# yisol/IDM-VTON

Hardware: AMD Instinct MI355X
Metric: try-on images/sec at 768x1024, 30 DDIM steps, guidance 2.0 (higher is better)
Workload: dtype bf16; 1 GPU; BASELINE.json configs[1]: 768x1024, 30 steps, batch 2/GPU, guidance 2.0, bf16 storage / fp32 accumulate, scheduler ddim, hipGraph on, GarmentNet batched over 6 timesteps, GarmentNet(block b+1)||TryonNet(block b) two-stream overlap on; images_per_call=2, parallelism=dp1 (image shards, one start-up RCCL weight broadcast), rccl_ranks=1

## Files before the change

### idm-vton_amd/csrc/gemm_body.cuh

```cuda
#pragma once
#include <type_traits>
#if !defined(__gfx950__) && !defined(__gfx942__) && defined(__HIP_DEVICE_COMPILE__)
#error "gemm_body.cuh: the counted vmcnt pipeline is written for gfx94x/gfx950 (stores counted in vmcnt)"
#endif
#include "common.cuh"
#include "gemm_common.cuh"

template <typename T, int BN, int BM, int WN, int WM, int ST, bool V1, bool LIN, bool PF, bool TR, bool XA = false>
__device__ __forceinline__ void gemm_body(const GemmParams& p, char* smem, const int m0, const int n0) {
    typedef typename VT<T>::v8 v8;
    typedef typename VT<T>::v4 v4;
    constexpr int NW = WN * WM;
    constexpr int SN = BN / WN, SM = BM / WM;
    constexpr int NI = SN / 32, MI = SM / 32;
    constexpr int WBYTES = BN * 128, XBYTES = BM * 128;
    constexpr int PW_ = BN / 8, PX_ = BM / 8;
    constexpr bool UNEVEN = (PW_ % NW != 0) || (PX_ % NW != 0);
    constexpr int WI = (PW_ + NW - 1) / NW, XI = (PX_ + NW - 1) / NW;
    static_assert(BN % 8 == 0 && BM % 8 == 0 && WN * SN == BN && WM * SM == BM && NI * 32 == SN && MI * 32 == SM, "tile / wave-count mismatch");
    static_assert(!UNEVEN || (V1 && ST == 2), "round-robin piece assignment needs the two-stage ring");
    char* sW = smem;
    char* sX = smem + ST * WBYTES;

    const int lane = threadIdx.x & 63;
    const int wave = uniform(threadIdx.x >> 6);
    const int wn = wave / WM, wm = wave % WM;
    const int u = lane >> 5, l31 = lane & 31;

    const int lrow = lane >> 3, lslot = lane & 7;
    auto wj = [&](int i) { return UNEVEN ? wave + i * NW : wave * WI + i; };
    auto xj = [&](int i) { return UNEVEN ? wave + i * NW : wave * XI + i; };
    uint32_t w_off[WI];
#pragma unroll
    for (int i = 0; i < WI; ++i) {
        const int R = wj(i) * 8 + lrow;
        const int c = lslot ^ ((R >> 1) & 7);
        w_off[i] = ((uint32_t)(n0 + R) * (uint32_t)p.Ktot + c * 8) * 2u;
    }
    int x_pix[XI], x_oy[XI], x_ox[XI], x_c8[XI];
    uint32_t x_off[XI];
    const int HoWo = p.Ho * p.Wo;
    auto kbyte = [&](int t) -> uint32_t { return (uint32_t)t * 128u; };
#pragma unroll
    for (int i = 0; i < XI; ++i) {
        const int R = xj(i) * 8 + lrow;
        const int m = m0 + R;
        x_c8[i] = (lslot ^ ((R >> 1) & 7)) * 8;
        if constexpr (LIN) {
            x_off[i] = m < p.M ? ((uint32_t)m * (uint32_t)p.seg[0].pitch + p.seg[0].coff + x_c8[i]) * 2u : OOB_SENTINEL;
        } else if (m < p.M) {
            const int b = m / HoWo, rem = m - b * HoWo;
            const int oy = rem / p.Wo, ox = rem - oy * p.Wo;
            x_pix[i] = b * p.Hi * p.Wi; x_oy[i] = oy * p.stride; x_ox[i] = ox * p.stride;
        } else {
            x_pix[i] = 0; x_oy[i] = -(1 << 28); x_ox[i] = 0;
        }
    }
    const __amdgpu_buffer_rsrc_t rs_w = make_rsrc(p.w, p.w_bytes);
    const __amdgpu_buffer_rsrc_t rs_x0 = make_rsrc(p.seg[0].ptr, p.seg[0].bytes);
    const int hin = p.ups ? p.Ho : p.Hi, win = p.ups ? p.Wo : p.Wi;

    int si = 0, kseg = 0;
    auto issue = [&](int t, int buf) {
        char* dW = sW + buf * WBYTES;
        char* dX = sX + buf * XBYTES;
#pragma unroll
        for (int i = 0; i < WI; ++i) {
            if (UNEVEN && wj(i) >= PW_) continue;
            dma16(rs_w, dW + wj(i) * 1024, w_off[i] + kbyte(t));
        }
        if constexpr (LIN) {
#pragma unroll
            for (int i = 0; i < XI; ++i) {
                if (UNEVEN && xj(i) >= PX_) continue;
                dma16(rs_x0, dX + xj(i) * 1024, x_off[i] + kbyte(t));
            }
        } else {
            const idmvton_seg sg = p.seg[si];
            const __amdgpu_buffer_rsrc_t rs_x = make_rsrc(sg.ptr, sg.bytes);
#pragma unroll
            for (int i = 0; i < XI; ++i) {
                if (UNEVEN && xj(i) >= PX_) continue;
                int iy = x_oy[i] + sg.dy, ix = x_ox[i] + sg.dx;
                const bool ok = (unsigned)iy < (unsigned)hin && (unsigned)ix < (unsigned)win;
                if (p.ups) { iy >>= 1; ix >>= 1; }
                const uint32_t off = ((uint32_t)(x_pix[i] + iy * p.Wi + ix) * (uint32_t)sg.pitch + sg.coff + kseg + x_c8[i]) * 2u;
                dma16(rs_x, dX + xj(i) * 1024, ok ? off : OOB_SENTINEL);
            }
            kseg += 64;
            if (kseg >= sg.len) { kseg = 0; ++si; }
        }
    };

    idmvton_seg sgc = p.seg[0];
    __amdgpu_buffer_rsrc_t rs_xc = rs_x0;
    auto issue_part = [&](int t, int buf, int s) {
        constexpr int LPT_ = WI + XI;
        char* dW = sW + buf * WBYTES;
        char* dX = sX + buf * XBYTES;
        if constexpr (!LIN) {
            if (s == 0) { sgc = p.seg[si]; rs_xc = make_rsrc(sgc.ptr, sgc.bytes); }
        }
#pragma unroll
        for (int j = 0; j < LPT_; ++j) {
            if ((j & 3) != s) continue;
            if (j < WI) {
                if (UNEVEN && wj(j) >= PW_) continue;
                dma16(rs_w, dW + wj(j) * 1024, w_off[j] + kbyte(t));
            } else {
                const int i = j - WI;
                if (UNEVEN && xj(i) >= PX_) continue;
                if constexpr (LIN) dma16(rs_x0, dX + xj(i) * 1024, x_off[i] + kbyte(t));
                else {
                    int iy = x_oy[i] + sgc.dy, ix = x_ox[i] + sgc.dx;
                    const bool ok = (unsigned)iy < (unsigned)hin && (unsigned)ix < (unsigned)win;
                    if (p.ups) { iy >>= 1; ix >>= 1; }
                    const uint32_t off = ((uint32_t)(x_pix[i] + iy * p.Wi + ix) * (uint32_t)sgc.pitch + sgc.coff + kseg + x_c8[i]) * 2u;
                    dma16(rs_xc, dX + xj(i) * 1024, ok ? off : OOB_SENTINEL);
                }
            }
        }
        if constexpr (!LIN) {
            if (s == 3) { kseg += 64; if (kseg >= sgc.len) { kseg = 0; ++si; } }
        }
    };

    int a_row[NI], a_swz[NI], b_row[MI], b_swz[MI];
#pragma unroll
    for (int ni = 0; ni < NI; ++ni) { const int r = wn * SN + ni * 32 + l31; a_row[ni] = r * 128; a_swz[ni] = (r >> 1) & 7; }
#pragma unroll
    for (int mi = 0; mi < MI; ++mi) { const int r = wm * SM + mi * 32 + l31; b_row[mi] = r * 128; b_swz[mi] = (r >> 1) & 7; }

    f32x16 acc[NI][MI];
#pragma unroll
    for (int ni = 0; ni < NI; ++ni)
#pragma unroll
        for (int mi = 0; mi < MI; ++mi)
#pragma unroll
            for (int r = 0; r < 16; ++r) acc[ni][mi][r] = 0.f;

    auto frag_a = [&](const char* bW, int s, int ni) { return *(const v8*)(bW + a_row[ni] + (((2 * s + u) ^ a_swz[ni]) << 4)); };
    auto frag_b = [&](const char* bX, int s, int mi) { return *(const v8*)(bX + b_row[mi] + (((2 * s + u) ^ b_swz[mi]) << 4)); };
    auto compute = [&](int buf, bool spread = false, int t_next = 0, int buf_next = 0) {
        const char* bW = sW + buf * WBYTES;
        const char* bX = sX + buf * XBYTES;
        if constexpr (!PF) {
#pragma unroll
            for (int s = 0; s < 4; ++s) {
                v8 a[NI], b[MI];
#pragma unroll
                for (int ni = 0; ni < NI; ++ni) a[ni] = frag_a(bW, s, ni);
#pragma unroll
                for (int mi = 0; mi < MI; ++mi) b[mi] = frag_b(bX, s, mi);
                if constexpr (V1) {
                    if (spread) issue_part(t_next, buf_next, s);
                    __builtin_amdgcn_sched_barrier(0);
                }
#pragma unroll
                for (int ni = 0; ni < NI; ++ni)
#pragma unroll
                    for (int mi = 0; mi < MI; ++mi)
                        acc[ni][mi] = TR ? VT<T>::mfma(b[mi], a[ni], acc[ni][mi]) : VT<T>::mfma(a[ni], b[mi], acc[ni][mi]);
            }
        } else {
            v8 a[2][NI], b[2][MI];
#pragma unroll
            for (int ni = 0; ni < NI; ++ni) a[0][ni] = frag_a(bW, 0, ni);
#pragma unroll
            for (int mi = 0; mi < MI; ++mi) b[0][mi] = frag_b(bX, 0, mi);
#pragma unroll
            for (int s = 0; s < 4; ++s) {
                if (s < 3) {
#pragma unroll
                    for (int ni = 0; ni < NI; ++ni) a[(s + 1) & 1][ni] = frag_a(bW, s + 1, ni);
#pragma unroll
                    for (int mi = 0; mi < MI; ++mi) b[(s + 1) & 1][mi] = frag_b(bX, s + 1, mi);
                }
                if (spread) issue_part(t_next, buf_next, s);
                __builtin_amdgcn_sched_barrier(0);
#pragma unroll
                for (int ni = 0; ni < NI; ++ni)
#pragma unroll
                    for (int mi = 0; mi < MI; ++mi)
                        acc[ni][mi] = TR ? VT<T>::mfma(b[s & 1][mi], a[s & 1][ni], acc[ni][mi])
                                         : VT<T>::mfma(a[s & 1][ni], b[s & 1][mi], acc[ni][mi]);
                __builtin_amdgcn_sched_barrier(0);
            }
        }
    };

    v8 xkf[XA ? XA_NK : 1];
    int xa_b = 0, xa_h = 0;
    if constexpr (XA) {
        static_assert(NI == 2 && !TR, "fused cross-attention: one 64-channel head per wave");
        const int mw = m0 + wm * SM;
        xa_b = (mw < p.M ? mw : p.M - 1) / p.xa.tokens;
        xa_h = (n0 + wn * SN) >> 6;
        xattn_load_k<T>(p.xa, xa_b, xa_h, lane, xkf);
    }
    const int nt = p.Ktot >> 6;
    if constexpr (!V1) {
        issue(0, 0);
        for (int t = 0; t < nt; ++t) {
            asm volatile("s_waitcnt vmcnt(0)" ::: "memory");
            __syncthreads();
            if (t + 1 < nt) issue(t + 1, (t + 1) & 1);
            compute(t & 1);
        }
    } else {
        constexpr int LPT = WI + XI;
        static_assert((ST - 2) * LPT < 64, "vmcnt immediate is 6 bits");
#pragma unroll
        for (int s = 0; s < ST - 1; ++s)
            if (s < nt) issue(s, s);
        int cbuf = 0, ibuf = ST - 1;
        for (int t = 0; t < nt; ++t) {
            if (t + ST - 2 < nt) wait_vmcnt<(ST - 2) * LPT>(); else wait_vmcnt<0>();
            __builtin_amdgcn_s_barrier();
            asm volatile("" ::: "memory");
            compute(cbuf, t + ST - 1 < nt, t + ST - 1, ibuf);
            cbuf = cbuf + 1 == ST ? 0 : cbuf + 1;
            ibuf = ibuf + 1 == ST ? 0 : ibuf + 1;
        }
    }

    if constexpr (XA) {
        v8 xvf[XA_NV];
        xattn_load_v<T>(p.xa, xa_b, xa_h, lane, xvf);
        xattn_compute<T, MI>(p.xa, p.M, acc, m0 + wm * SM, lane, xkf, xvf);
    }
    gemm_epilogue<T, NI, MI, SN, SM, TR>(p, acc, m0, n0, wn, wm, lane);
}

template <typename T, int BN, int BM, int WN, int WM, int ST, bool V1, bool LIN, int OCC, bool PFX = false>
__global__ __launch_bounds__(WN * WM * 64, OCC) void gemm_conv_kernel(const GemmParams p) {
    __shared__ __attribute__((aligned(1024))) char smem[ST * (BN + BM) * 128];
    const int wg = xcd_remap(blockIdx.x, p.tiles_m * p.tiles_n);
    int tm, tn;
    if constexpr (!V1) { tm = wg / p.tiles_n; tn = wg - tm * p.tiles_n; }
    else {
        const int GM = p.gm > 0 ? p.gm : 1024 / BM;
        const int width = GM * p.tiles_n;
        const int grp = wg / width, rem = wg - grp * width;
        const int first = grp * GM;
        const int gsz = p.tiles_m - first < GM ? p.tiles_m - first : GM;
        tn = rem / gsz; tm = first + (rem - tn * gsz);
    }
    const int m0 = tm * BM, n0 = tn * BN;
    if constexpr (BN == 320) {
        gemm_body<T, BN, BM, WN, WM, ST, V1, LIN, OCC == 1 || PFX, false>(p, smem, m0, n0);
    } else {
        if (p.vt != nullptr && n0 >= p.vt_n0) gemm_body<T, BN, BM, WN, WM, ST, V1, LIN, OCC == 1 || PFX, true>(p, smem, m0, n0);
        else gemm_body<T, BN, BM, WN, WM, ST, V1, LIN, OCC == 1 || PFX, false>(p, smem, m0, n0);
    }
}

template <typename T, int BN, int BM, int WN, int WM, int ST, int OCC>
__global__ __launch_bounds__(WN * WM * 64, OCC) void gemm_xattn_kernel(const GemmParams p) {
    __shared__ __attribute__((aligned(1024))) char smem[ST * (BN + BM) * 128];
    const int wg = xcd_remap(blockIdx.x, p.tiles_m * p.tiles_n);
    const int GM = p.gm > 0 ? p.gm : 1024 / BM;
    const int width = GM * p.tiles_n;
    const int grp = wg / width, rem = wg - grp * width;
    const int first = grp * GM;
    const int gsz = p.tiles_m - first < GM ? p.tiles_m - first : GM;
    const int tn = rem / gsz, tm = first + (rem - tn * gsz);
    gemm_body<T, BN, BM, WN, WM, ST, true, true, OCC == 1, false, true>(p, smem, tm * BM, tn * BN);
}

template <typename T, int BN, int BM, int WN, int WM, int ST, bool V1, int OCC, bool PFX = false>
static void launch_cfg(const GemmParams& p0, bool lin, hipStream_t st) {
    GemmParams p = p0;
    p.gm = V1 ? idmvton_choose_gm(p.tiles_m, p.tiles_n, BM, BN, p.Ktot) : 0;
    const dim3 grid(p.tiles_n * p.tiles_m), block(WN * WM * 64);
    if constexpr (V1) {
        if (lin) { hipLaunchKernelGGL((gemm_conv_kernel<T, BN, BM, WN, WM, ST, true, true, OCC, PFX>), grid, block, 0, st, p); return; }
    }
    hipLaunchKernelGGL((gemm_conv_kernel<T, BN, BM, WN, WM, ST, V1, false, OCC, PFX>), grid, block, 0, st, p);
}


int gemm_tiles_v0(const GemmParams& p, bool bf16, int bn, int bm, bool lin, hipStream_t st);
int gemm_tiles_v1(const GemmParams& p, bool bf16, int bn, int bm, bool lin, hipStream_t st);
int gemm_tiles_v2(const GemmParams& p, bool bf16, int bn, int bm, bool lin, hipStream_t st);
int gemm_tiles_w8(const GemmParams& p, bool bf16, int bn, int bm, int form, bool lin, hipStream_t st);
int gemm_tiles_xattn(const GemmParams& p, bool bf16, int bn, int bm, int w8, hipStream_t st);
int launch_gemm_lin(const GemmParams& p, bool bf16, int bm, int form, int grid_cap, hipStream_t st);
```

### idm-vton_amd/csrc/gemm_common.cuh

```cuda
#pragma once
#include "common.cuh"
#include "xattn.cuh"

struct GemmParams {
    const void* w; uint32_t w_bytes; int N; int Ktot;
    int nseg; idmvton_seg seg[IDMVTON_MAX_SEG];
    int M, Ho, Wo, Hi, Wi, stride, ups;
    void* out; int ldo;
    const void* bias; const void* rowbias; int rowbias_ld; int rows_per_group;
    const void* res; int ldr;
    int mode;
    void* vt; int vt_n0; int vt_tokens; int vt_perm;
    int colscale_n; float colscale;
    int tiles_m, tiles_n;
    int gm;
    int wide;
    int res32, out32;
    int bias32;
    int out8; float o8_scale, vt8_scale;
    XAttnParams xa;
};

int idmvton_choose_gm(int tiles_m, int tiles_n, int bm, int bn, int K);

template <int N> __device__ __forceinline__ void wait_vmcnt() { asm volatile("s_waitcnt vmcnt(%0)" ::"n"(N) : "memory"); }

__device__ __forceinline__ void swap_cols8(const f32x16& c, const int gp, float (&v)[8]) {
#pragma unroll
    for (int j = 0; j < 4; ++j) {
        const auto r = __builtin_amdgcn_permlane32_swap(__float_as_uint(c[8 * gp + j]), __float_as_uint(c[8 * gp + 4 + j]), false, false);
        v[j] = __uint_as_float(r[0]);
        v[4 + j] = __uint_as_float(r[1]);
    }
}

template <typename T, int NI, int MI, int SN, int SM, bool TR>
__device__ __forceinline__ void gemm_epilogue(const GemmParams& p, f32x16 (&acc)[NI][MI], const int m0, const int n0, const int wn, const int wm,
                                              const int lane) {
    typedef typename VT<T>::v4 v4;
    typedef typename VT<T>::v8 v8;
    const int u = lane >> 5, l31 = lane & 31;
    const T* bias = (const T*)p.bias;
    if constexpr (TR) {
        if (p.out8) {
            uint8_t* vt = (uint8_t*)p.vt;
            const int Cv = p.N - p.vt_n0;
#pragma unroll
            for (int ni = 0; ni < NI; ++ni) {
                const int n = n0 + wn * SN + ni * 32 + l31;
                if (n >= p.N) continue;
                const float bv = bias ? (float)bias[n] : 0.f;
#pragma unroll
                for (int mi = 0; mi < MI; ++mi) {
                    const int m = m0 + wm * SM + mi * 32;
                    if (m >= p.M) continue;
                    const int b = m / p.vt_tokens;
                    const int tok = m - b * p.vt_tokens;
                    int4 o;
                    int w[4];
#pragma unroll
                    for (int g = 0; g < 4; ++g)
                        w[g] = pack4_fp8(clamp448((acc[ni][mi][4 * g] + bv) * p.vt8_scale), clamp448((acc[ni][mi][4 * g + 1] + bv) * p.vt8_scale),
                                         clamp448((acc[ni][mi][4 * g + 2] + bv) * p.vt8_scale), clamp448((acc[ni][mi][4 * g + 3] + bv) * p.vt8_scale));
                    o.x = w[0]; o.y = w[1]; o.z = w[2]; o.w = w[3];
                    *(int4*)(vt + ((size_t)(b * Cv + n - p.vt_n0) * p.vt_tokens + (tok & ~63) + 32 * u + ((tok >> 1) & 16))) = o;
                }
            }
            return;
        }
        if (p.vt_perm) {
            T* vt = (T*)p.vt;
            const int Cv = p.N - p.vt_n0;
#pragma unroll
            for (int ni = 0; ni < NI; ++ni) {
                const int n = n0 + wn * SN + ni * 32 + l31;
                if (n >= p.N) continue;
                const float bv = bias ? (float)bias[n] : 0.f;
#pragma unroll
                for (int mi = 0; mi < MI; ++mi)
#pragma unroll
                    for (int gp = 0; gp < 2; ++gp) {
                        const int m = m0 + wm * SM + mi * 32 + 16 * gp;
                        if (m >= p.M) continue;
                        const int b = m / p.vt_tokens;
                        const int tok = m - b * p.vt_tokens + 8 * u;
                        v8 o;
#pragma unroll
                        for (int j = 0; j < 8; ++j) o[j] = (T)(acc[ni][mi][8 * gp + j] + bv);
                        *(v8*)(vt + ((size_t)(b * Cv + n - p.vt_n0) * p.vt_tokens + tok)) = o;
                    }
            }
            return;
        }
        T* vt = (T*)p.vt;
        const int Cv = p.N - p.vt_n0;
#pragma unroll
        for (int ni = 0; ni < NI; ++ni) {
            const int n = n0 + wn * SN + ni * 32 + l31;
            if (n >= p.N) continue;
            const float bv = bias ? (float)bias[n] : 0.f;
#pragma unroll
            for (int mi = 0; mi < MI; ++mi)
#pragma unroll
                for (int g = 0; g < 4; ++g) {
                    const int m = m0 + wm * SM + mi * 32 + 8 * g + 4 * u;
                    if (m >= p.M) continue;
                    const int b = m / p.vt_tokens;
                    int tok = m - b * p.vt_tokens;
                    if (p.vt_perm) tok = (tok & ~12) | ((tok & 4) << 1) | ((tok & 8) >> 1);
                    v4 o;
#pragma unroll
                    for (int j = 0; j < 4; ++j) o[j] = (T)(acc[ni][mi][4 * g + j] + bv);
                    *(v4*)(vt + ((size_t)(b * Cv + n - p.vt_n0) * p.vt_tokens + tok)) = o;
                }
        }
        return;
    }
    T* out = (T*)p.out;
    const T* res = (const T*)p.res;
    const T* rowbias = (const T*)p.rowbias;
    if (p.wide) {
#pragma unroll
        for (int mi = 0; mi < MI; ++mi) {
            const int m = m0 + wm * SM + mi * 32 + l31;
            if (m >= p.M) continue;
            const T* rb = rowbias ? rowbias + (size_t)(m / p.rows_per_group) * p.rowbias_ld : nullptr;
            if (p.mode == IDMVTON_EPI_GEGLU) {
                if constexpr (NI % 2 == 0) {
#pragma unroll
                    for (int pr = 0; pr < NI / 2; ++pr)
#pragma unroll
                        for (int gp = 0; gp < 2; ++gp) {
                            float h[8], gt[8];
                            swap_cols8(acc[2 * pr][mi], gp, h);
                            swap_cols8(acc[2 * pr + 1][mi], gp, gt);
                            const int nh = n0 + wn * SN + pr * 64 + 16 * gp + 8 * u;
                            if (nh + 32 >= p.N) continue;
                            const int jo = ((n0 + wn * SN + pr * 64) >> 1) + 16 * gp + 8 * u;
                            if (bias) {
                                const v8 bh = *(const v8*)(bias + nh), bg = *(const v8*)(bias + nh + 32);
#pragma unroll
                                for (int j = 0; j < 8; ++j) { h[j] += (float)bh[j]; gt[j] += (float)bg[j]; }
                            }
                            v8 o;
#pragma unroll
                            for (int j = 0; j < 8; ++j) o[j] = (T)(h[j] * gelu_erf(gt[j]));
                            *(v8*)(out + (size_t)m * p.ldo + jo) = o;
                        }
                }
                continue;
            }
#pragma unroll
            for (int ni = 0; ni < NI; ++ni) {
#pragma unroll
                for (int gp = 0; gp < 2; ++gp) {
                    float v[8];
                    swap_cols8(acc[ni][mi], gp, v);
                    const int n = n0 + wn * SN + ni * 32 + 16 * gp + 8 * u;
                    if (n >= p.N) continue;
                    if (bias) {
                        if (p.bias32) {
                            const float4* bp = (const float4*)((const float*)p.bias + n);
                            const float4 b0 = bp[0], b1 = bp[1];
                            v[0] += b0.x; v[1] += b0.y; v[2] += b0.z; v[3] += b0.w;
                            v[4] += b1.x; v[5] += b1.y; v[6] += b1.z; v[7] += b1.w;
                        } else {
                            const v8 bb = *(const v8*)(bias + n);
#pragma unroll
                            for (int j = 0; j < 8; ++j) v[j] += (float)bb[j];
                        }
                    }
                    if (rb) {
                        const v8 bb = *(const v8*)(rb + n);
#pragma unroll
                        for (int j = 0; j < 8; ++j) v[j] += (float)bb[j];
                    }
                    if (n < p.colscale_n) {
#pragma unroll
                        for (int j = 0; j < 8; ++j) v[j] *= p.colscale;
                    }
                    if constexpr (NI * MI <= 8)
                    if (p.out8) {
                        int2 o;
                        o.x = pack4_fp8(clamp448(v[0] * p.o8_scale), clamp448(v[1] * p.o8_scale), clamp448(v[2] * p.o8_scale), clamp448(v[3] * p.o8_scale));
                        o.y = pack4_fp8(clamp448(v[4] * p.o8_scale), clamp448(v[5] * p.o8_scale), clamp448(v[6] * p.o8_scale), clamp448(v[7] * p.o8_scale));
                        *(int2*)((uint8_t*)p.out + (size_t)m * p.ldo + n) = o;
                        continue;
                    }
                    if (p.mode == IDMVTON_EPI_GELU) {
#pragma unroll
                        for (int j = 0; j < 8; ++j) v[j] = gelu_erf(v[j]);
                    } else if (p.mode == IDMVTON_EPI_QUICKGELU) {
#pragma unroll
                        for (int j = 0; j < 8; ++j) v[j] = v[j] / (1.0f + __expf(-1.702f * v[j]));
                    }
                    if (res) {
                        if (p.res32) {
                            const float4* rp = (const float4*)((const float*)p.res + (size_t)m * p.ldr + n);
                            const float4 r0 = rp[0], r1 = rp[1];
                            v[0] += r0.x; v[1] += r0.y; v[2] += r0.z; v[3] += r0.w;
                            v[4] += r1.x; v[5] += r1.y; v[6] += r1.z; v[7] += r1.w;
                        } else {
                            const v8 rr = *(const v8*)(res + (size_t)m * p.ldr + n);
#pragma unroll
                            for (int j = 0; j < 8; ++j) v[j] += (float)rr[j];
                        }
                    }
                    if (p.out32) {
                        float4* op = (float4*)((float*)p.out + (size_t)m * p.ldo + n);
                        op[0] = make_float4(v[0], v[1], v[2], v[3]);
                        op[1] = make_float4(v[4], v[5], v[6], v[7]);
                    } else {
                        v8 o;
#pragma unroll
                        for (int j = 0; j < 8; ++j) o[j] = (T)v[j];
                        *(v8*)(out + (size_t)m * p.ldo + n) = o;
                    }
                }
            }
        }
        return;
    }
    if constexpr (NI * MI <= 8)
#pragma unroll
    for (int mi = 0; mi < MI; ++mi) {
        const int m = m0 + wm * SM + mi * 32 + l31;
        if (m >= p.M) continue;
        const T* rb = rowbias ? rowbias + (size_t)(m / p.rows_per_group) * p.rowbias_ld : nullptr;
        if (p.mode == IDMVTON_EPI_GEGLU) {
            if constexpr (NI % 2 == 0) {
#pragma unroll
                for (int pr = 0; pr < NI / 2; ++pr)
#pragma unroll
                    for (int g = 0; g < 4; ++g) {
                        const int nh = n0 + wn * SN + pr * 64 + 8 * g + 4 * u;
                        if (nh + 32 >= p.N) continue;
                        const int jo = ((n0 + wn * SN + pr * 64) >> 1) + 8 * g + 4 * u;
                        v4 o;
#pragma unroll
                        for (int j = 0; j < 4; ++j) {
                            float h = acc[2 * pr][mi][4 * g + j], gt = acc[2 * pr + 1][mi][4 * g + j];
                            if (bias) { h += (float)bias[nh + j]; gt += (float)bias[nh + 32 + j]; }
                            o[j] = (T)(h * gelu_erf(gt));
                        }
                        *(v4*)(out + (size_t)m * p.ldo + jo) = o;
                    }
            }
            continue;
        }
#pragma unroll
        for (int ni = 0; ni < NI; ++ni)
#pragma unroll
            for (int g = 0; g < 4; ++g) {
                const int n = n0 + wn * SN + ni * 32 + 8 * g + 4 * u;
                if (n >= p.N) continue;
                float v[4];
#pragma unroll
                for (int j = 0; j < 4; ++j) v[j] = acc[ni][mi][4 * g + j];
                if (bias) {
                    const v4 bb = *(const v4*)(bias + n);
#pragma unroll
                    for (int j = 0; j < 4; ++j) v[j] += (float)bb[j];
                }
                if (rb) {
                    const v4 bb = *(const v4*)(rb + n);
#pragma unroll
                    for (int j = 0; j < 4; ++j) v[j] += (float)bb[j];
                }
                if (n < p.colscale_n) {
#pragma unroll
                    for (int j = 0; j < 4; ++j) v[j] *= p.colscale;
                }
                if (p.mode == IDMVTON_EPI_GELU) {
#pragma unroll
                    for (int j = 0; j < 4; ++j) v[j] = gelu_erf(v[j]);
                } else if (p.mode == IDMVTON_EPI_QUICKGELU) {
#pragma unroll
                    for (int j = 0; j < 4; ++j) v[j] = v[j] / (1.0f + __expf(-1.702f * v[j]));
                }
                if (res) {
                    const v4 rr = *(const v4*)(res + (size_t)m * p.ldr + n);
#pragma unroll
                    for (int j = 0; j < 4; ++j) v[j] += (float)rr[j];
                }
                v4 o;
#pragma unroll
                for (int j = 0; j < 4; ++j) o[j] = (T)v[j];
                *(v4*)(out + (size_t)m * p.ldo + n) = o;
            }
    }
}
```

### idm-vton_amd/csrc/gemm_conv.hip

```cpp
#include <cstdlib>
#include <cstring>
#include <vector>
#include "gemm_body.cuh"

int launch_gemm_lin(const GemmParams& p, bool bf16, int bm, int form, int grid_cap, hipStream_t st);

#include <map>
#include <mutex>
#include <tuple>
int idmvton_choose_gm(int tiles_m, int tiles_n, int bm, int bn, int K) {
    static const char* env = getenv("IDMVTON_GM");
    if (env) return atoi(env);
    static const bool model = getenv("IDMVTON_GM_MODEL") && atoi(getenv("IDMVTON_GM_MODEL")) != 0;
    if (!model) return 0;
    static std::mutex mu;
    static std::map<std::tuple<int, int, int, int, int>, int> cache;
    const auto key = std::make_tuple(tiles_m, tiles_n, bm, bn, K);
    std::lock_guard<std::mutex> lk(mu);
    auto it = cache.find(key);
    if (it != cache.end()) return it->second;
    const int T = tiles_m * tiles_n, q = T / 8, r = T % 8;
    static const long cap = getenv("IDMVTON_GM_CAP_KB") ? atol(getenv("IDMVTON_GM_CAP_KB")) << 10 : (2l << 20);
    long best = -1; int best_gm = 0;
    for (int gm = 1; gm <= tiles_m; ++gm) {
        if (gm > 1 && (long)gm * bm * K * 2 > cap) break;
        long cost = 0;
        for (int x = 0; x < 8; ++x) {
            const int lo = x < r ? x * (q + 1) : r * (q + 1) + (x - r) * q, n = x < r ? q + 1 : q;
            int m_lo = tiles_m, m_hi = -1;
            std::vector<char> ms(tiles_m, 0), ns(tiles_n, 0);
            int cm = 0, cn = 0;
            for (int wg = lo; wg < lo + n; ++wg) {
                const int width = gm * tiles_n, grp = wg / width, rem = wg - grp * width, first = grp * gm;
                const int gsz = tiles_m - first < gm ? tiles_m - first : gm;
                const int tn = rem / gsz, tm = first + (rem - tn * gsz);
                if (!ms[tm]) { ms[tm] = 1; ++cm; }
                if (!ns[tn]) { ns[tn] = 1; ++cn; }
            }
            (void)m_lo; (void)m_hi;
            cost += (long)cm * bm + (long)cn * bn;
        }
        if (best < 0 || cost < best) { best = cost; best_gm = gm; }
    }
    cache[key] = best_gm;
    return best_gm;
}

static int launch_gemm(const GemmParams& p0, bool bf16, int variant, int bn, int bm, bool lin, hipStream_t st) {
    GemmParams p = p0;
    int form = 0;
    int grid_cap = 0;
    if (variant == 5) { form = bm & 15; grid_cap = (bm & 0x4000) ? 5 : 0; bm &= ~(15 | 0x4000); }
    p.tiles_n = (p.N + bn - 1) / bn;
    p.tiles_m = (p.M + bm - 1) / bm;
    int rc = 1;
    if (p.mode == IDMVTON_EPI_XATTN) {
        if (bm != 64 && p.xa.tokens % 64 != 0) {
            bm = 64;
            p.tiles_m = (p.M + bm - 1) / bm;
        }
        if (gemm_tiles_xattn(p, bf16, bn, bm, variant == 6 && bn == 128 && bm == 128, st))
            return idmvton_set_error(IDMVTON_E_ARG, "gemm_conv: IDMVTON_EPI_XATTN runs on the 128x64, 128x128 and 128x256 tiles (got %dx%d)", bn, bm);
        CHECK_LAUNCH("gemm_conv");
        return IDMVTON_OK;
    }
    if (variant == 0) rc = gemm_tiles_v0(p, bf16, bn, bm, lin, st);
    else if (variant == 1) rc = gemm_tiles_v1(p, bf16, bn, bm, lin, st);
    else if (variant == 2) rc = gemm_tiles_v2(p, bf16, bn, bm, lin, st);
    else if (variant == 5) {
        if (!(bn == 256 && (bm == 256 || bm == 192))) return idmvton_set_error(IDMVTON_E_ARG, "gemm_conv: variant 5 is the 256x256 / 256x192 tile");
        if (lin) rc = launch_gemm_lin(p, bf16, bm, form, grid_cap, st);
        else if (bm == 256) rc = gemm_tiles_v1(p, bf16, 256, 256, lin, st);
        else {
            p.tiles_n = (p.N + 127) / 128; p.tiles_m = (p.M + 255) / 256;
            rc = gemm_tiles_v1(p, bf16, 128, 256, lin, st);
        }
    } else if (variant == 6) {
        const int form6 = bm & 15;
        bm &= ~15;
        p.tiles_m = (p.M + bm - 1) / bm;
        if (bn == 320 && (p.vt || !p.wide || p.out8 || p.mode == IDMVTON_EPI_GEGLU)) {
            const int fbn = bn == 320 ? 128 : bn, fbm = bn == 320 ? 256 : bm;
            p.tiles_n = (p.N + fbn - 1) / fbn;
            p.tiles_m = (p.M + fbm - 1) / fbm;
            rc = gemm_tiles_v1(p, bf16, fbn, fbm, lin, st);
        } else rc = gemm_tiles_w8(p, bf16, bn, bm, form6, lin, st);
    } else return idmvton_set_error(IDMVTON_E_ARG, "gemm_conv: unknown variant %d", variant);
    if (rc) return idmvton_set_error(IDMVTON_E_ARG, "gemm_conv: variant %d has no %dx%d tile", variant, bn, bm);
    CHECK_LAUNCH("gemm_conv");
    return IDMVTON_OK;
}

extern "C" int idmvton_gemm_conv(const idmvton_gemm_conv_args* a, void* stream) {
    CHECK_ARG(a != nullptr, IDMVTON_E_ARG, "gemm_conv: null args");
    CHECK_ARG(a->dtype == IDMVTON_F16 || a->dtype == IDMVTON_BF16, IDMVTON_E_DTYPE, "gemm_conv: dtype %d", a->dtype);
    CHECK_ARG(a->M > 0 && a->N > 0 && a->Ktot > 0, IDMVTON_E_SHAPE, "gemm_conv: M=%d N=%d K=%d", a->M, a->N, a->Ktot);
    CHECK_ARG(a->Ktot % 64 == 0, IDMVTON_E_SHAPE, "gemm_conv: Ktot=%d must be a multiple of 64", a->Ktot);
    CHECK_ARG(a->N % 4 == 0, IDMVTON_E_SHAPE, "gemm_conv: N=%d must be a multiple of 4", a->N);
    CHECK_ARG(a->nseg >= 1 && a->nseg <= IDMVTON_MAX_SEG, IDMVTON_E_SHAPE, "gemm_conv: nseg=%d", a->nseg);
    int ksum = 0;
    for (int s = 0; s < a->nseg; ++s) {
        const idmvton_seg& g = a->seg[s];
        CHECK_ARG(g.ptr && g.len > 0 && g.len % 64 == 0, IDMVTON_E_SHAPE, "gemm_conv: seg %d len=%d", s, g.len);
        CHECK_ARG(g.pitch % 8 == 0 && g.coff % 8 == 0, IDMVTON_E_ALIGN, "gemm_conv: seg %d pitch=%d coff=%d", s, g.pitch, g.coff);
        CHECK_ARG(g.bytes < 0x80000000u, IDMVTON_E_SHAPE, "gemm_conv: seg %d tensor >= 2 GiB", s);
        CHECK_ARG(((uintptr_t)g.ptr & 15) == 0, IDMVTON_E_ALIGN, "gemm_conv: seg %d pointer not 16-byte aligned", s);
        ksum += g.len;
    }
    CHECK_ARG(ksum == a->Ktot, IDMVTON_E_SHAPE, "gemm_conv: segment lengths sum to %d, Ktot=%d", ksum, a->Ktot);
    CHECK_ARG(a->Ho > 0 && a->Wo > 0 && a->Hi > 0 && a->Wi > 0 && a->stride > 0 && a->M % (a->Ho * a->Wo) == 0,
              IDMVTON_E_SHAPE, "gemm_conv: geometry M=%d Ho=%d Wo=%d", a->M, a->Ho, a->Wo);
    if (a->ups) CHECK_ARG(a->stride == 1 && a->Ho <= 2 * a->Hi && a->Ho >= 2 * a->Hi - 1 && a->Wo <= 2 * a->Wi && a->Wo >= 2 * a->Wi - 1, IDMVTON_E_SHAPE,
                          "gemm_conv: ups=1 needs stride 1 and an output grid of 2Hi x 2Wi or one short of it (Ho=%d Hi=%d Wo=%d Wi=%d)", a->Ho, a->Hi, a->Wo, a->Wi);
    CHECK_ARG(a->w && ((uintptr_t)a->w & 15) == 0, IDMVTON_E_ALIGN, "gemm_conv: weight pointer");
    const uint64_t wbytes = (uint64_t)a->N * a->Ktot * 2;
    CHECK_ARG(wbytes + (uint64_t)128 * a->Ktot * 2 < 0xFFFFFFFFull, IDMVTON_E_SHAPE, "gemm_conv: weight too large");
    const bool geglu = a->mode == IDMVTON_EPI_GEGLU, xattn = a->mode == IDMVTON_EPI_XATTN;
    CHECK_ARG(a->mode == IDMVTON_EPI_NONE || a->mode == IDMVTON_EPI_GELU || a->mode == IDMVTON_EPI_QUICKGELU || geglu || xattn, IDMVTON_E_ARG, "gemm_conv: mode %d", a->mode);
    CHECK_ARG(a->colscale_n >= 0 && a->colscale_n % 4 == 0 && !(geglu && a->colscale_n), IDMVTON_E_ARG, "gemm_conv: colscale_n=%d", a->colscale_n);
    if (geglu) CHECK_ARG(a->N % 64 == 0 && !a->res && !a->rowbias && !a->vt, IDMVTON_E_ARG, "gemm_conv: GEGLU needs N%%64==0, no res/rowbias/vt");
    CHECK_ARG(a->out || (a->vt && a->vt_n0 == 0), IDMVTON_E_ARG, "gemm_conv: null out");
    if (a->out) CHECK_ARG(a->ldo % 4 == 0 && ((uintptr_t)a->out & 7) == 0, IDMVTON_E_ALIGN, "gemm_conv: out alignment");
    if (a->res) CHECK_ARG(a->ldr % 4 == 0 && ((uintptr_t)a->res & 7) == 0, IDMVTON_E_ALIGN, "gemm_conv: res alignment");
    if (a->bias) CHECK_ARG(((uintptr_t)a->bias & 7) == 0, IDMVTON_E_ALIGN, "gemm_conv: bias alignment");
    if (a->rowbias) CHECK_ARG(a->rowbias_ld % 4 == 0 && a->rows_per_group > 0 && ((uintptr_t)a->rowbias & 7) == 0,
                              IDMVTON_E_ALIGN, "gemm_conv: rowbias");
    if (a->vt && a->vt_perm) CHECK_ARG(((uintptr_t)a->vt & 15) == 0, IDMVTON_E_ALIGN, "gemm_conv: vt pointer not 16-byte aligned");
    if (a->vt && a->vt_perm) CHECK_ARG(a->vt_tokens % 16 == 0, IDMVTON_E_ARG, "gemm_conv: vt_perm needs vt_tokens %% 16 == 0 (got %d)", a->vt_tokens);
    if (a->vt) CHECK_ARG(a->vt_tokens > 0 && a->vt_tokens % 4 == 0 && a->M % a->vt_tokens == 0 && a->vt_n0 % 64 == 0 &&
                         a->vt_n0 >= 0 && a->vt_n0 < a->N && ((uintptr_t)a->vt & 7) == 0,
                         IDMVTON_E_ARG, "gemm_conv: vt_tokens=%d vt_n0=%d", a->vt_tokens, a->vt_n0);

    GemmParams p;
    memset(&p.xa, 0, sizeof(p.xa));
    if (xattn) {
        const idmvton_xattn* x = a->xattn;
        CHECK_ARG(x != nullptr && (x->nseg == 1 || x->nseg == 2), IDMVTON_E_ARG, "gemm_conv: IDMVTON_EPI_XATTN needs `xattn` with 1 or 2 key segments");
        CHECK_ARG(a->N % 64 == 0 && !a->bias && !a->res && !a->rowbias && !a->vt && !a->colscale_n && !a->io_flags &&
                  a->nseg == 1 && a->Ho == 1 && a->Hi == 1 && a->Wo == a->M && a->Wi == a->M && a->out && a->ldo % 8 == 0 && ((uintptr_t)a->out & 15) == 0,
                  IDMVTON_E_ARG, "gemm_conv: IDMVTON_EPI_XATTN is a plain Linear with N %% 64 == 0 and nothing else in its epilogue");
        CHECK_ARG(x->tokens > 0 && x->tokens % 32 == 0 && a->M % x->tokens == 0, IDMVTON_E_SHAPE, "gemm_conv: xattn.tokens=%d (rows per batch element, a multiple of 32 dividing M=%d)", x->tokens, a->M);
        for (int s = 0; s < x->nseg; ++s) {
            const int nk_max = s == 0 ? 96 : 32;
            CHECK_ARG(x->k[s] && x->vt[s] && x->nk[s] > 0 && x->nk[s] <= nk_max && x->k_rows[s] >= ((x->nk[s] + 31) & ~31) && x->ldk[s] >= a->N && x->ldk[s] % 8 == 0 &&
                      x->ldvt[s] >= ((x->nk[s] + 15) & ~15) && x->ldvt[s] % 8 == 0 && (((uintptr_t)x->k[s] | (uintptr_t)x->vt[s]) & 15) == 0, IDMVTON_E_SHAPE,
                      "gemm_conv: xattn segment %d: nk=%d (<= %d) k_rows=%d (>= round32(nk)) ldk=%d ldvt=%d (>= round16(nk))", s, x->nk[s], nk_max, x->k_rows[s], x->ldk[s], x->ldvt[s]);
            p.xa.k[s] = x->k[s]; p.xa.vt[s] = x->vt[s]; p.xa.ldk[s] = x->ldk[s]; p.xa.ldvt[s] = x->ldvt[s]; p.xa.nk[s] = x->nk[s]; p.xa.krows[s] = x->k_rows[s];
        }
        p.xa.nseg = x->nseg; p.xa.tokens = x->tokens; p.xa.vchan = a->N; p.xa.ip_scale = x->ip_scale;
    } else CHECK_ARG(a->xattn == nullptr, IDMVTON_E_ARG, "gemm_conv: `xattn` without mode IDMVTON_EPI_XATTN");
    p.w = a->w; p.w_bytes = (uint32_t)wbytes; p.N = a->N; p.Ktot = a->Ktot;
    p.nseg = a->nseg;
    for (int s = 0; s < IDMVTON_MAX_SEG; ++s) p.seg[s] = a->seg[s < a->nseg ? s : a->nseg - 1];
    p.M = a->M; p.Ho = a->Ho; p.Wo = a->Wo; p.Hi = a->Hi; p.Wi = a->Wi; p.stride = a->stride; p.ups = a->ups ? 1 : 0;
    p.out = a->out; p.ldo = a->ldo; p.bias = a->bias; p.rowbias = a->rowbias; p.rowbias_ld = a->rowbias_ld;
    p.rows_per_group = a->rows_per_group > 0 ? a->rows_per_group : 1; p.res = a->res; p.ldr = a->ldr; p.mode = a->mode;
    p.vt = a->vt; p.vt_n0 = a->vt_n0; p.vt_tokens = a->vt_tokens > 0 ? a->vt_tokens : 4; p.vt_perm = a->vt_perm ? 1 : 0;
    p.colscale_n = a->colscale_n; p.colscale = a->colscale;
    p.tiles_m = p.tiles_n = 0; p.gm = 0;
    {
        auto a16 = [](const void* q) { return ((uintptr_t)q & 15) == 0; };
        const int n_out = geglu ? a->N / 2 : a->N;
        p.wide = n_out % 8 == 0 && a->N % 8 == 0 && a->colscale_n % 8 == 0 && (!a->out || (a->ldo % 8 == 0 && a16(a->out))) &&
                 (!a->res || (a->ldr % 8 == 0 && a16(a->res))) && (!a->bias || a16(a->bias)) &&
                 (!a->rowbias || (a->rowbias_ld % 8 == 0 && a16(a->rowbias))) && (!a->vt || a->vt_n0 % 8 == 0);
    }

    int variant = 1, bn = 64, bm = 64;
    static const bool env_narrow = getenv("IDMVTON_EPILOGUE_8B") != nullptr;
    if ((a->tile_hint & 0x8000) || env_narrow) p.wide = 0;
    p.res32 = (a->io_flags & IDMVTON_IO_RES_F32) ? 1 : 0;
    p.out32 = (a->io_flags & IDMVTON_IO_OUT_F32) ? 1 : 0;
    p.bias32 = (a->io_flags & IDMVTON_IO_BIAS_F32) ? 1 : 0;
    if (p.bias32) CHECK_ARG(a->bias && p.wide && !geglu && !a->vt && ((uintptr_t)a->bias & 15) == 0, IDMVTON_E_ARG,
                            "gemm_conv: IDMVTON_IO_BIAS_F32 needs a 16-byte aligned bias and the plain 16-byte epilogue (no GEGLU, no vt)");
    CHECK_ARG((a->io_flags & ~15) == 0, IDMVTON_E_ARG, "gemm_conv: io_flags=%d", a->io_flags);
    p.out8 = (a->io_flags & IDMVTON_IO_OUT_F8) ? 1 : 0;
    p.o8_scale = a->f8_out_scale; p.vt8_scale = a->f8_vt_scale;
    if (p.out8) {
        CHECK_ARG(a->io_flags == IDMVTON_IO_OUT_F8 && a->mode == IDMVTON_EPI_NONE && !a->res && !a->rowbias && p.wide,
                  IDMVTON_E_ARG, "gemm_conv: IDMVTON_IO_OUT_F8 needs the plain 16-byte epilogue (no activation / residual / rowbias / fp32 IO)");
        CHECK_ARG((!a->out || a->f8_out_scale > 0.f) && (!a->vt || (a->f8_vt_scale > 0.f && a->vt_tokens % 64 == 0 && ((uintptr_t)a->vt & 15) == 0)),
                  IDMVTON_E_ARG, "gemm_conv: IDMVTON_IO_OUT_F8: scales > 0, vt_tokens %% 64 == 0 (got %d), 16-byte aligned vt", a->vt_tokens);
    }
    if (p.res32 || p.out32) {
        CHECK_ARG((a->io_flags & ~7) == 0 && !geglu && !a->vt, IDMVTON_E_ARG, "gemm_conv: io_flags=%d (fp32 res / out: no GEGLU, no vt)", a->io_flags);
        CHECK_ARG(!p.res32 || a->res, IDMVTON_E_ARG, "gemm_conv: IDMVTON_IO_RES_F32 without res");
        CHECK_ARG(p.wide, IDMVTON_E_ALIGN, "gemm_conv: the fp32 residual stream needs the 16-byte epilogue (N, ldo, ldr multiples of 8, 16-byte aligned pointers)");
    }
    if (a->tile_hint) { variant = (a->tile_hint >> 28) & 0xf; bn = (a->tile_hint >> 16) & 0xfff; bm = a->tile_hint & 0x7fff; }
    else {
        static const int cand[5][2] = {{256, 256}, {128, 256}, {128, 128}, {128, 64}, {64, 64}};
        for (int i = 0; i < 5; ++i) {
            const int n_ = cand[i][0], m_ = cand[i][1];
            if (geglu && n_ < 128) continue;
            if (xattn && (n_ != 128)) continue;
            if (a->vt && a->vt_n0 % n_ != 0) continue;
            if (i < 4 && (n_ > ((a->N + 63) & ~63) || m_ > ((a->M + 63) & ~63))) continue;
            bn = n_; bm = m_;
            if ((long)((a->N + n_ - 1) / n_) * ((a->M + m_ - 1) / m_) >= 200) break;
        }
    }
    if (geglu) CHECK_ARG(bn >= 128, IDMVTON_E_ARG, "gemm_conv: GEGLU needs BN >= 128 (64-row wave tiles)");
    if (a->vt) CHECK_ARG(a->vt_n0 % bn == 0, IDMVTON_E_ARG, "gemm_conv: vt_n0 %% BN != 0");
    const idmvton_seg& s0 = a->seg[0];
    const bool lin = a->nseg == 1 && a->Ho == 1 && a->Hi == 1 && a->Wo == a->M && a->Wi == a->M && a->stride == 1 &&
                     !a->ups && s0.dy == 0 && s0.dx == 0 && (uint64_t)a->M * s0.pitch * 2 < 0x80000000ull;
    if (!a->tile_hint && bn == 256 && bm == 256 && lin) { variant = 5; bm = 257; }
    else if (!a->tile_hint && !xattn) {
        if (bn == 256 && bm == 256) variant = 6;
        else if (bn == 128 && bm == 128) variant = 6;
        if (a->N > 256 && a->N <= 320 && p.wide && !a->vt && !geglu && !p.out8 && (a->M + 191) / 192 >= 200) { variant = 6; bn = 320; bm = 192; }
    }
    hipStream_t st = (hipStream_t)stream;
    return launch_gemm(p, a->dtype == IDMVTON_BF16, variant, bn, bm, lin, st);
}
```

### idm-vton_amd/csrc/gemm_lin.hip

```cpp
#include "gemm_common.cuh"
#include <type_traits>

template <typename T, int BM, int WN, int WM, int DMA_SPLIT, int WAIT_AT>
__device__ __forceinline__ void gemm_lin_persistent(const GemmParams& p, char* smem) {
    typedef typename VT<T>::v8 v8;
    constexpr int BN = 256, NW = WN * WM;
    constexpr int SN = BN / WN, SM = BM / WM, NI = SN / 32, MI = SM / 32;
    constexpr int PWW = BN / (8 * NW), PWX = BM / (8 * NW);
    static_assert(PWW * 8 * NW == BN && PWX * 8 * NW == BM && NI * 32 * WN == BN && MI * 32 * WM == BM, "tile / wave-count mismatch");
    constexpr int OPW = BN * 128;
    constexpr int BUF = (BN + BM) * 128;

    const int lane = threadIdx.x & 63;
    const int wave = uniform(threadIdx.x >> 6);
    const int wn = wave / WM, wm = wave % WM;
    const int u = lane >> 5, l31 = lane & 31;

    const int ntiles = p.tiles_m * p.tiles_n, G = gridDim.x;
    auto coords = [&](int idx, int& m0, int& n0) {
        const int wg = xcd_remap(idx, ntiles);
        const int GM = p.gm > 0 ? p.gm : 1024 / BM;
        const int width = GM * p.tiles_n;
        const int grp = wg / width, rem = wg - grp * width;
        const int first = grp * GM;
        const int gsz = p.tiles_m - first < GM ? p.tiles_m - first : GM;
        const int tn = rem / gsz;
        m0 = (first + (rem - tn * gsz)) * BM;
        n0 = tn * BN;
    };

    const int lrow = lane >> 3, lslot = lane & 7;
    uint32_t w_off[PWW], x_off[PWX];
    auto set_offsets = [&](int m0, int n0) {
#pragma unroll
        for (int i = 0; i < PWW; ++i) {
            const int R = (wave * PWW + i) * 8 + lrow;
            w_off[i] = ((uint32_t)(n0 + R) * (uint32_t)p.Ktot + (lslot ^ ((R >> 1) & 7)) * 8) * 2u;
        }
#pragma unroll
        for (int i = 0; i < PWX; ++i) {
            const int R = (wave * PWX + i) * 8 + lrow;
            const int m = m0 + R;
            x_off[i] = m < p.M ? ((uint32_t)m * (uint32_t)p.seg[0].pitch + p.seg[0].coff + (lslot ^ ((R >> 1) & 7)) * 8) * 2u : OOB_SENTINEL;
        }
    };
    const __amdgpu_buffer_rsrc_t rs_w = make_rsrc(p.w, p.w_bytes);
    const __amdgpu_buffer_rsrc_t rs_x = make_rsrc(p.seg[0].ptr, p.seg[0].bytes);
    char* const dW = smem + wave * (PWW * 1024);
    char* const dX = smem + OPW + wave * (PWX * 1024);
    auto dma_w = [&](int i, int buf_off, uint32_t koff) {
        __builtin_amdgcn_raw_ptr_buffer_load_lds(rs_w, LDS_PTR(dW + buf_off + i * 1024), 16, w_off[i], koff, 0, 0);
    };
    auto dma_x = [&](int i, int buf_off, uint32_t koff) {
        __builtin_amdgcn_raw_ptr_buffer_load_lds(rs_x, LDS_PTR(dX + buf_off + i * 1024), 16, x_off[i], koff, 0, 0);
    };
    auto dma_first = [&](int buf_off) {
#pragma unroll
        for (int i = 0; i < PWW; ++i) dma_w(i, buf_off, 0u);
#pragma unroll
        for (int i = 0; i < PWX; ++i) dma_x(i, buf_off, 0u);
    };

    const int swz = (l31 >> 1) & 7;
    int fa_off[4], fb_off[4];
#pragma unroll
    for (int s = 0; s < 4; ++s) {
        const int ch = ((2 * s + u) ^ swz) << 4;
        fa_off[s] = (wn * SN + l31) * 128 + ch;
        fb_off[s] = OPW + (wm * SM + l31) * 128 + ch;
    }
    v8 fa[2][NI], fb[2][MI];
    f32x16 acc[NI][MI];

    auto read_all = [&](int set, int s, int buf_off) {
#pragma unroll
        for (int ni = 0; ni < NI; ++ni) fa[set][ni] = *(const v8*)(smem + buf_off + fa_off[s] + ni * 4096);
#pragma unroll
        for (int mi = 0; mi < MI; ++mi) fb[set][mi] = *(const v8*)(smem + buf_off + fb_off[s] + mi * 4096);
    };
    constexpr int NMF = NI * MI;
    constexpr int NRD = NI + MI;
    auto pin = [&](int nrd, int nv) {
#pragma unroll
        for (int i = 0; i < NMF; ++i) {
            __builtin_amdgcn_sched_group_barrier(0x008, 1, 0);
            if (i < nrd) __builtin_amdgcn_sched_group_barrier(0x100, 1, 0);
            if (i >= NMF - nv) __builtin_amdgcn_sched_group_barrier(0x010, 1, 0);
            if (i < nv - NMF) __builtin_amdgcn_sched_group_barrier(0x010, 1, 0);
        }
    };

    const int nt = p.Ktot >> 6;
    int idx = blockIdx.x, m0, n0, nm0 = 0, nn0 = 0;
    bool has_next = false;
    int cur = 0;

    auto run_tile = [&](auto trc) {
        constexpr bool TR = decltype(trc)::value;
        auto mfma_range = [&](int set, int i0, int i1) {
#pragma unroll
            for (int k = i0; k < i1; ++k) {
                const int ni = k / MI, mi = k % MI;
                acc[ni][mi] = TR ? VT<T>::mfma(fb[set][mi], fa[set][ni], acc[ni][mi]) : VT<T>::mfma(fa[set][ni], fb[set][mi], acc[ni][mi]);
            }
        };
#pragma unroll
        for (int ni = 0; ni < NI; ++ni)
#pragma unroll
            for (int mi = 0; mi < MI; ++mi)
#pragma unroll
                for (int r = 0; r < 16; ++r) acc[ni][mi][r] = 0.f;
        __builtin_amdgcn_s_barrier();
        asm volatile("" ::: "memory");
        read_all(0, 0, cur);
        for (int t = 0; t + 1 < nt; ++t) {
            const int nxt = cur ^ BUF;
            const uint32_t koff = (uint32_t)(t + 1) * 128u;
            read_all(1, 1, cur);
#pragma unroll
            for (int i = 0; i < PWW; ++i) dma_w(i, nxt, koff);
            if constexpr (DMA_SPLIT == 1) {
#pragma unroll
                for (int i = 0; i < PWX; ++i) dma_x(i, nxt, koff);
            }
            mfma_range(0, 0, NMF);
            pin(NRD, DMA_SPLIT == 0 ? PWW : PWW + PWX);
            __builtin_amdgcn_sched_barrier(0);
            read_all(0, 2, cur);
            if constexpr (DMA_SPLIT == 0) {
#pragma unroll
                for (int i = 0; i < PWX; ++i) dma_x(i, nxt, koff);
            }
            mfma_range(1, 0, NMF);
            pin(NRD, DMA_SPLIT == 0 ? PWX : 0);
            __builtin_amdgcn_sched_barrier(0);
            read_all(1, 3, cur);
            mfma_range(0, 0, NMF);
            pin(NRD, 0);
            __builtin_amdgcn_sched_barrier(0);
            mfma_range(1, 0, WAIT_AT);
            __builtin_amdgcn_sched_barrier(0);
            asm volatile("s_waitcnt vmcnt(0) lgkmcnt(0)" ::: "memory");
            __builtin_amdgcn_s_barrier();
            asm volatile("" ::: "memory");
            __builtin_amdgcn_sched_barrier(0);
            read_all(0, 0, nxt);
            mfma_range(1, WAIT_AT, NMF);
#pragma unroll
            for (int i = 0; i < NMF - WAIT_AT; ++i) {
                __builtin_amdgcn_sched_group_barrier(0x008, 1, 0);
                if (i < NRD) __builtin_amdgcn_sched_group_barrier(0x100, 1, 0);
                if (i == NMF - WAIT_AT - 1 && NRD > NMF - WAIT_AT) __builtin_amdgcn_sched_group_barrier(0x100, NRD - (NMF - WAIT_AT), 0);
            }
            __builtin_amdgcn_sched_barrier(0);
            cur = nxt;
        }
        if (has_next) {
            set_offsets(nm0, nn0);
            dma_first(cur ^ BUF);
        }
        read_all(1, 1, cur);
        mfma_range(0, 0, NMF);
        pin(NRD, 0);
        __builtin_amdgcn_sched_barrier(0);
        read_all(0, 2, cur);
        mfma_range(1, 0, NMF);
        pin(NRD, 0);
        __builtin_amdgcn_sched_barrier(0);
        read_all(1, 3, cur);
        mfma_range(0, 0, NMF);
        pin(NRD, 0);
        __builtin_amdgcn_sched_barrier(0);
        mfma_range(1, 0, NMF);
        if (has_next) asm volatile("s_waitcnt vmcnt(0)" ::: "memory");
        gemm_epilogue<T, NI, MI, SN, SM, TR>(p, acc, m0, n0, wn, wm, lane);
    };

    coords(idx, m0, n0);
    set_offsets(m0, n0);
    dma_first(0);
    asm volatile("s_waitcnt vmcnt(0)" ::: "memory");
    for (;;) {
        const int nidx = idx + G;
        has_next = nidx < ntiles;
        if (has_next) coords(nidx, nm0, nn0);
        if (p.vt != nullptr && n0 >= p.vt_n0) run_tile(std::true_type{});
        else run_tile(std::false_type{});
        if (!has_next) break;
        cur ^= BUF; idx = nidx; m0 = nm0; n0 = nn0;
    }
}

template <typename T, int BM, int WN, int WM, int DMA_SPLIT, int WAIT_AT>
__global__ __launch_bounds__(512, 2) void gemm_lin_kernel(const GemmParams p) {
    __shared__ __attribute__((aligned(1024))) char smem[2 * (256 + BM) * 128];
    gemm_lin_persistent<T, BM, WN, WM, DMA_SPLIT, WAIT_AT>(p, smem);
}

static int persistent_grid(int ntiles, int grid_cap) {
    static int cus = 0;
    if (!cus) {
        int dev = 0, n = 0;
        if (hipGetDevice(&dev) != hipSuccess || hipDeviceGetAttribute(&n, hipDeviceAttributeMultiprocessorCount, dev) != hipSuccess || n < 8) n = 256;
        cus = n & ~7;
    }
    const int cap = grid_cap > 0 ? grid_cap : cus;
    return ntiles < cap ? ntiles : cap;
}
template <typename T>
static int launch_lin(const GemmParams& p0, int bm, int form, int grid_cap, hipStream_t st) {
    GemmParams p = p0;
    p.gm = idmvton_choose_gm(p.tiles_m, p.tiles_n, bm, 256, p.Ktot);
    const dim3 grid(persistent_grid(p.tiles_n * p.tiles_m, grid_cap)), block(512);
    if (bm == 192) hipLaunchKernelGGL((gemm_lin_kernel<T, 192, 4, 2, 0, 2>), grid, block, 0, st, p);
    else if (form == 0) hipLaunchKernelGGL((gemm_lin_kernel<T, 256, 2, 4, 0, 2>), grid, block, 0, st, p);
    else hipLaunchKernelGGL((gemm_lin_kernel<T, 256, 2, 4, 1, 2>), grid, block, 0, st, p);
    return 0;
}
int launch_gemm_lin(const GemmParams& p, bool bf16, int bm, int form, int grid_cap, hipStream_t st) {
    return bf16 ? launch_lin<bf16_t>(p, bm, form, grid_cap, st) : launch_lin<f16_t>(p, bm, form, grid_cap, st);
}
```

### idm-vton_amd/csrc/gemm_tiles_v1.hip

```cpp
#include "gemm_body.cuh"

template <typename T>
static int run(const GemmParams& p, int bn, int bm, bool lin, hipStream_t st) {
    if (bn == 256 && bm == 256) launch_cfg<T, 256, 256, 2, 4, 2, true, 2>(p, lin, st);
    else if (bn == 128 && bm == 256) launch_cfg<T, 128, 256, 2, 4, 3, true, 2>(p, lin, st);
    else if (bn == 128 && bm == 128) launch_cfg<T, 128, 128, 2, 2, 3, true, 1>(p, lin, st);
    else if (bn == 128 && bm == 64) launch_cfg<T, 128, 64, 2, 2, 3, true, 2>(p, lin, st);
    else if (bn == 64 && bm == 64) launch_cfg<T, 64, 64, 2, 2, 4, true, 2>(p, lin, st);
    else return 1;
    return 0;
}
int gemm_tiles_v1(const GemmParams& p, bool bf16, int bn, int bm, bool lin, hipStream_t st) {
    return bf16 ? run<bf16_t>(p, bn, bm, lin, st) : run<f16_t>(p, bn, bm, lin, st);
}
```

### idm-vton_amd/ffi.py

```python
import ctypes as C
import os

_HERE = os.path.dirname(os.path.abspath(__file__))
LIB_PATH = os.environ.get("IDMVTON_HIP_LIB") or os.path.join(_HERE, "libidmvton_hip.so")

F16, BF16, F32, F8E4M3 = 0, 1, 2, 3
EPI_NONE, EPI_GEGLU, EPI_GELU, EPI_QUICKGELU, EPI_XATTN = 0, 1, 2, 3, 4
ATTN_SELF, ATTN_CROSS = 0, 1
IO_RES_F32, IO_OUT_F32, IO_BIAS_F32, IO_OUT_F8 = 1, 2, 4, 8
GN_X_F32, GN_Y_SPLIT, GN_AFFINE_F32 = 1, 2, 4
LAYOUT_SPLIT, LAYOUT_NHWC_F32 = 1, 2
SPLIT_ACT, SPLIT_W3, SPLIT_W3T = 0, 1, 2
KVS_WIDEN_E4M3, KVS_COPY = 0, 1
MAX_SEG = 24
ABI_VERSION = 9

i32, u32, f32, vp = C.c_int32, C.c_uint32, C.c_float, C.c_void_p


class Seg(C.Structure):
    _fields_ = [("ptr", vp), ("bytes", u32), ("pitch", i32), ("coff", i32), ("len", i32), ("dy", i32), ("dx", i32)]


class XAttn(C.Structure):
    _fields_ = [("nseg", i32), ("k", vp * 2), ("ldk", i32 * 2), ("k_rows", i32 * 2), ("vt", vp * 2), ("ldvt", i32 * 2), ("nk", i32 * 2),
                ("tokens", i32), ("ip_scale", f32)]


class GemmConvArgs(C.Structure):
    _fields_ = [("dtype", i32), ("w", vp), ("N", i32), ("Ktot", i32), ("nseg", i32), ("seg", Seg * MAX_SEG),
                ("M", i32), ("Ho", i32), ("Wo", i32), ("Hi", i32), ("Wi", i32), ("stride", i32), ("ups", i32),
                ("out", vp), ("ldo", i32), ("bias", vp), ("rowbias", vp), ("rowbias_ld", i32),
                ("rows_per_group", i32), ("res", vp), ("ldr", i32), ("mode", i32), ("vt", vp), ("vt_n0", i32),
                ("vt_tokens", i32), ("tile_hint", i32), ("vt_perm", i32), ("io_flags", i32), ("xattn", C.POINTER(XAttn)),
                ("colscale_n", i32), ("colscale", f32), ("f8_out_scale", f32), ("f8_vt_scale", f32)]


class AttnArgs(C.Structure):
    _fields_ = [("dtype", i32), ("mode", i32), ("B", i32), ("heads", i32), ("Nq", i32), ("q", vp), ("ldq", i32),
                ("out", vp), ("ldo", i32), ("nseg", i32), ("k", vp * 2), ("ldk", i32 * 2), ("vt", vp * 2),
                ("ldvt", i32 * 2), ("nk", i32 * 2), ("k_rows", i32 * 2), ("seg_b0", i32 * 2), ("ip_scale", f32), ("tune", i32), ("q_prescaled", i32)]


class LayerNormArgs(C.Structure):
    _fields_ = [("dtype", i32), ("rows", i32), ("C", i32), ("x", vp), ("ldx", i32), ("gamma", vp), ("beta", vp),
                ("eps", f32), ("y", vp), ("ldy", i32), ("y2", vp), ("ldy2", i32), ("x_f32", i32)]


class GroupNormArgs(C.Structure):
    _fields_ = [("dtype", i32), ("B", i32), ("HW", i32), ("C", i32), ("groups", i32), ("x", vp), ("C1", i32),
                ("x2", vp), ("gamma", vp), ("beta", vp), ("eps", f32), ("silu", i32), ("y", vp), ("stats", vp), ("stats_doubles", i32),
                ("flags", i32)]


class PackInputArgs(C.Structure):
    _fields_ = [("dtype", i32), ("B", i32), ("hw", i32), ("cpad", i32), ("latents", vp), ("cond", vp), ("out", vp)]


class CfgStepArgs(C.Structure):
    _fields_ = [("dtype", i32), ("B", i32), ("hw", i32), ("ldc", i32), ("eps_nhwc", vp), ("latents", vp),
                ("noise", vp), ("coef", vp)]


class LayoutArgs(C.Structure):
    _fields_ = [("dtype", i32), ("B", i32), ("C", i32), ("HW", i32), ("cpad", i32), ("to_nhwc", i32), ("src", vp),
                ("dst", vp), ("scale", f32), ("shift", f32), ("flags", i32)]


class VaeSampleArgs(C.Structure):
    _fields_ = [("dtype", i32), ("B", i32), ("hw", i32), ("ldm", i32), ("moments", vp), ("noise", vp), ("z", vp),
                ("scale", f32)]


class AttnSmallArgs(C.Structure):
    _fields_ = [("dtype", i32), ("B", i32), ("heads", i32), ("Lq", i32), ("Lk", i32), ("d", i32), ("q", vp), ("ldq", i32),
                ("k", vp), ("ldk", i32), ("v", vp), ("ldv", i32), ("out", vp), ("ldo", i32), ("scale", f32), ("causal", i32)]


class AttnF8Args(C.Structure):
    _fields_ = [("out_dtype", i32), ("B", i32), ("heads", i32), ("Nq", i32), ("q8", vp), ("ldq", i32), ("out", vp), ("ldo", i32),
                ("nseg", i32), ("k8", vp * 2), ("ldk", i32 * 2), ("vt8", vp * 2), ("ldvt", i32 * 2), ("nk", i32 * 2), ("k_rows", i32 * 2),
                ("seg_b0", i32 * 2), ("qk_scale_exp", i32), ("v_scale_exp", i32)]


class QuantF8Args(C.Structure):
    _fields_ = [("dtype", i32), ("mode", i32), ("rows", i32), ("cols", i32), ("src", vp), ("lds", i32), ("dst", vp), ("ldd", i32), ("scale", f32)]


class SoftmaxArgs(C.Structure):
    _fields_ = [("dtype", i32), ("rows", i32), ("n", i32), ("ld", i32), ("x", vp), ("scale", f32), ("y_split", vp), ("ldy", i32), ("n_valid", i32)]


class SplitArgs(C.Structure):
    _fields_ = [("dtype", i32), ("mode", i32), ("rows", i32), ("cols", i32), ("src", vp), ("lds", i32), ("dst", vp), ("ldd", i32)]


class KvUnpackDesc(C.Structure):
    _fields_ = [("src", vp), ("dst", vp), ("exp", vp), ("rows", i32), ("cols", i32), ("lds", i32), ("ldd", i32)]


class KvUnpackArgs(C.Structure):
    _fields_ = [("dtype", i32), ("n", i32), ("desc", vp), ("max_chunks", i32)]


class KvStreamDesc(KvUnpackDesc):
    pass


class KvStreamArgs(C.Structure):
    _fields_ = [("dtype", i32), ("mode", i32), ("n", i32), ("workgroups", i32), ("desc", vp), ("first", vp)]


STRUCTS = {"idmvton_seg": Seg, "idmvton_gemm_conv_args": GemmConvArgs, "idmvton_attn_args": AttnArgs,
           "idmvton_layernorm_args": LayerNormArgs, "idmvton_groupnorm_args": GroupNormArgs,
           "idmvton_pack_input_args": PackInputArgs, "idmvton_cfg_step_args": CfgStepArgs,
           "idmvton_layout_args": LayoutArgs, "idmvton_vae_sample_args": VaeSampleArgs, "idmvton_softmax_args": SoftmaxArgs,
           "idmvton_attn_small_args": AttnSmallArgs, "idmvton_attn_f8_args": AttnF8Args, "idmvton_quant_f8_args": QuantF8Args,
           "idmvton_split_args": SplitArgs, "idmvton_xattn": XAttn, "idmvton_kv_unpack_desc": KvUnpackDesc,
           "idmvton_kv_unpack_args": KvUnpackArgs, "idmvton_kv_stream_desc": KvStreamDesc, "idmvton_kv_stream_args": KvStreamArgs}

SYMBOLS = ["idmvton_last_error", "idmvton_abi_version", "idmvton_sizeof", "idmvton_gemm_conv", "idmvton_attn_fwd",
           "idmvton_layernorm", "idmvton_groupnorm", "idmvton_pack_input", "idmvton_cfg_step", "idmvton_layout",
           "idmvton_vae_sample", "idmvton_softmax_rows", "idmvton_probe_mfma", "idmvton_groupnorm_stats_doubles",
           "idmvton_attn_small", "idmvton_rccl_unique_id", "idmvton_rccl_comm_init", "idmvton_rccl_bcast_arena",
           "idmvton_rccl_comm_destroy", "idmvton_attn_f8", "idmvton_quant_f8", "idmvton_split", "idmvton_attn_fwd_shared",
           "idmvton_attn_f8_shared", "idmvton_attn_fwd_indexed", "idmvton_attn_f8_indexed",
           "idmvton_attn_fwd_ragged", "idmvton_attn_f8_ragged", "idmvton_kv_unpack", "idmvton_kv_stream",
           "idmvton_host_device_ptr", "idmvton_kv_fill"]

_lib = None


class HipLibraryMissing(RuntimeError):
    pass


def lib():
    global _lib
    if _lib is not None:
        return _lib
    if not os.path.exists(LIB_PATH):
        raise HipLibraryMissing(f"{LIB_PATH} not built: run `make -C {os.path.join(_HERE, 'csrc')}` "
                                "(or __graft_entry__.build()); there is no CPU fallback")
    L = C.CDLL(LIB_PATH)
    for s in SYMBOLS:
        if not hasattr(L, s):
            raise HipLibraryMissing(f"{LIB_PATH} does not export {s}")
    L.idmvton_last_error.restype = C.c_char_p
    L.idmvton_sizeof.argtypes = [C.c_char_p]
    L.idmvton_abi_version.restype = C.c_int
    v = L.idmvton_abi_version()
    if v != ABI_VERSION:
        raise HipLibraryMissing(f"{LIB_PATH} implements C ABI version {v}, this binding needs {ABI_VERSION}: rebuild it "
                                f"(`make -C {os.path.join(_HERE, 'csrc')}`)")
    for name, st in STRUCTS.items():
        n = L.idmvton_sizeof(name.encode())
        if n != C.sizeof(st):
            raise HipLibraryMissing(f"ABI drift: sizeof({name}) is {n} in the library, {C.sizeof(st)} in ffi.py")
    for s in ("idmvton_gemm_conv", "idmvton_attn_fwd", "idmvton_layernorm", "idmvton_groupnorm",
              "idmvton_pack_input", "idmvton_cfg_step", "idmvton_layout", "idmvton_vae_sample", "idmvton_softmax_rows",
              "idmvton_attn_small", "idmvton_attn_f8", "idmvton_quant_f8", "idmvton_split"):
        getattr(L, s).argtypes = [vp, vp]
        getattr(L, s).restype = C.c_int
    for s in ("idmvton_attn_fwd_shared", "idmvton_attn_f8_shared"):
        getattr(L, s).argtypes = [vp, C.POINTER(i32), vp]
        getattr(L, s).restype = C.c_int
    for s in ("idmvton_attn_fwd_indexed", "idmvton_attn_f8_indexed"):
        getattr(L, s).argtypes = [vp, C.POINTER(i32), C.POINTER(vp), vp]
        getattr(L, s).restype = C.c_int
    for s in ("idmvton_attn_fwd_ragged", "idmvton_attn_f8_ragged"):
        getattr(L, s).argtypes = [vp, C.POINTER(i32), C.POINTER(vp), C.POINTER(vp), vp]
        getattr(L, s).restype = C.c_int
    L.idmvton_kv_unpack.argtypes = [vp, vp, vp]
    L.idmvton_kv_unpack.restype = C.c_int
    L.idmvton_kv_stream.argtypes = [vp, vp, vp, vp]
    L.idmvton_kv_stream.restype = C.c_int
    L.idmvton_kv_fill.argtypes = [vp, vp, vp, vp]
    L.idmvton_kv_fill.restype = C.c_int
    L.idmvton_host_device_ptr.argtypes = [vp, C.POINTER(vp)]
    L.idmvton_host_device_ptr.restype = C.c_int
    L.idmvton_probe_mfma.argtypes = [C.c_int, vp, vp, vp, vp]
    L.idmvton_groupnorm_stats_doubles.argtypes = [C.c_int] * 4
    L.idmvton_groupnorm_stats_doubles.restype = C.c_int
    L.idmvton_rccl_unique_id.argtypes = [vp]
    L.idmvton_rccl_comm_init.argtypes = [vp, C.c_int, C.c_int, C.POINTER(vp)]
    L.idmvton_rccl_bcast_arena.argtypes = [vp, vp, C.c_uint64, C.c_int, C.c_uint64, vp]
    L.idmvton_rccl_comm_destroy.argtypes = [vp]
    for s in ("idmvton_rccl_unique_id", "idmvton_rccl_comm_init", "idmvton_rccl_bcast_arena", "idmvton_rccl_comm_destroy"):
        getattr(L, s).restype = C.c_int
    _lib = L
    return L


def call(fn_name, args, stream):
    L = lib()
    rc = getattr(L, fn_name)(C.byref(args), C.c_void_p(stream))
    if rc != 0:
        raise RuntimeError(f"{fn_name} failed ({rc}): {L.idmvton_last_error().decode()}")


def call_shared(fn_name, args, seg_nb, stream):
    L = lib()
    nb = (i32 * 2)(*seg_nb)
    rc = getattr(L, fn_name)(C.byref(args), nb, C.c_void_p(stream))
    if rc != 0:
        raise RuntimeError(f"{fn_name} failed ({rc}): {L.idmvton_last_error().decode()}")


def call_indexed(fn_name, args, seg_nb, seg_index, stream):
    L = lib()
    nb = (i32 * 2)(*seg_nb)
    ix = (vp * 2)(*[int(x) if x else None for x in seg_index])
    rc = getattr(L, fn_name)(C.byref(args), nb, ix, C.c_void_p(stream))
    if rc != 0:
        raise RuntimeError(f"{fn_name} failed ({rc}): {L.idmvton_last_error().decode()}")


def call_ragged(fn_name, args, seg_nb, seg_index, seg_nk, stream):
    L = lib()
    nb = (i32 * 2)(*seg_nb)
    ix = (vp * 2)(*[int(x) if x else None for x in (seg_index or (0, 0))])
    nk = (vp * 2)(*[int(x) if x else None for x in seg_nk])
    rc = getattr(L, fn_name)(C.byref(args), nb, ix, nk, C.c_void_p(stream))
    if rc != 0:
        raise RuntimeError(f"{fn_name} failed ({rc}): {L.idmvton_last_error().decode()}")


def call_kv_unpack(args, host_desc, stream):
    L = lib()
    rc = L.idmvton_kv_unpack(C.byref(args), host_desc if isinstance(host_desc, int) else C.cast(host_desc, vp), C.c_void_p(stream))
    if rc != 0:
        raise RuntimeError(f"idmvton_kv_unpack failed ({rc}): {L.idmvton_last_error().decode()}")


def call_kv_stream(args, host_desc, host_first, stream):
    L = lib()
    p = lambda x: x if isinstance(x, int) else C.cast(x, vp)
    rc = L.idmvton_kv_stream(C.byref(args), p(host_desc), p(host_first), C.c_void_p(stream))
    if rc != 0:
        raise RuntimeError(f"idmvton_kv_stream failed ({rc}): {L.idmvton_last_error().decode()}")


def call_kv_fill(args, host_desc, host_first, stream):
    L = lib()
    p = lambda x: x if isinstance(x, int) else C.cast(x, vp)
    rc = L.idmvton_kv_fill(C.byref(args), p(host_desc), p(host_first), C.c_void_p(stream))
    if rc != 0:
        raise RuntimeError(f"idmvton_kv_fill failed ({rc}): {L.idmvton_last_error().decode()}")


def host_device_ptr(host):
    L = lib()
    dev = vp()
    rc = L.idmvton_host_device_ptr(C.c_void_p(host), C.byref(dev))
    if rc != 0:
        raise RuntimeError(f"idmvton_host_device_ptr failed ({rc}): {L.idmvton_last_error().decode()}")
    return int(dev.value)
```

### idm-vton_amd/ops.py

```python
import ctypes as C
import json
import os

import torch

from . import ffi

_DT = {torch.float16: ffi.F16, torch.bfloat16: ffi.BF16}


def _dt(t):
    try:
        return _DT[t.dtype]
    except KeyError:
        raise TypeError(f"idm_vton_amd ops take float16/bfloat16 tensors, got {t.dtype}") from None


def _stream():
    return torch.cuda.current_stream().cuda_stream


PROFILE = None


def _call(fn_name, args, flops=0.0, bytes_=0.0, seg_nb=None, seg_index=None, seg_nk=None):
    if seg_nk is not None:
        launch = lambda: ffi.call_ragged(fn_name, args, seg_nb, seg_index, seg_nk, _stream())
    elif seg_index is not None:
        launch = lambda: ffi.call_indexed(fn_name, args, seg_nb, seg_index, _stream())
    elif seg_nb is not None:
        launch = lambda: ffi.call_shared(fn_name, args, seg_nb, _stream())
    else:
        launch = lambda: ffi.call(fn_name, args, _stream())
    if PROFILE is None:
        launch()
        return
    e0, e1 = torch.cuda.Event(enable_timing=True), torch.cuda.Event(enable_timing=True)
    e0.record()
    launch()
    e1.record()
    PROFILE.append((fn_name, e0, e1, flops, bytes_))


TUNE_PATH = os.environ.get("IDMVTON_TUNE_TABLE") or os.path.join(os.path.dirname(os.path.abspath(__file__)), "tune_gfx950.json")
_TUNE = {"gemm": {}, "attn": {}}
RECORD = None


def load_tune(path=TUNE_PATH):
    global _TUNE
    _TUNE = {"gemm": {}, "attn": {}}
    if path and os.path.exists(path):
        with open(path) as f:
            t = json.load(f)
        _TUNE = {"gemm": dict(t.get("gemm", {})), "attn": dict(t.get("attn", {}))}
        for kind in ("gemm", "attn") if os.environ.get("IDMVTON_TUNE_NO_MIRROR") != "1" else ():
            for k, v in list(_TUNE[kind].items()):
                d, rest = k.split(",", 1)
                if d in ("0", "1"):
                    _TUNE[kind].setdefault(("1" if d == "0" else "0") + "," + rest, v)
    return _TUNE


def gemm_key(a):
    return "%d,%d,%d,%d,%d,%d,%d,%d,%d,%d" % (a.dtype, a.M, a.N, a.Ktot, a.nseg, a.Wo, a.stride, a.ups, a.mode, 1 if a.vt else 0)


def attn_key(a):
    return "%d,%d,%d,%d,%d,%d,%d,%d,%d" % (a.dtype, a.mode, a.B, a.heads, a.Nq, a.nseg, a.nk[0], a.nk[1] if a.nseg > 1 else 0,
                                          a.seg_b0[1] if a.nseg > 1 else 0)


def _dev(t):
    if not t.is_cuda:
        raise RuntimeError("idm_vton_amd ops run on the GPU only (tensor is on %s); there is no CPU fallback" % t.device)
    return t


def _ptr(t):
    return None if t is None else _dev(t).data_ptr()


class SegSpec:
    __slots__ = ("t", "coff", "len", "dy", "dx")

    def __init__(self, t, coff, length, dy=0, dx=0):
        self.t, self.coff, self.len, self.dy, self.dx = t, coff, length, dy, dx


def gemm_conv(segs, w, M, *, Ho=1, Wo=None, Hi=1, Wi=None, stride=1, ups=False, out=None, ldo=None, bias=None,
              rowbias=None, rowbias_ld=0, rows_per_group=1, res=None, ldr=None, geglu=False, gelu=False, quick_gelu=False, vt=None,
              vt_n0=0, vt_tokens=0, vt_perm=True, colscale_n=0, colscale=1.0, tile_hint=0, out_f32=False, xattn=None, f8=None):
    if f8 is not None:
        if res is not None or rowbias is not None or geglu or gelu or quick_gelu or (bias is not None and bias.dtype == torch.float32):
            raise ValueError("gemm_conv(f8=...): no residual / rowbias / activation, and the bias in the storage dtype (not fp32)")
        if vt is not None and vt_tokens % 64 != 0:
            raise ValueError(f"gemm_conv(f8=...): vt_tokens must be a multiple of 64 (got {vt_tokens})")
    a = ffi.GemmConvArgs()
    a.dtype = _dt(w)
    N, Ktot = w.shape
    a.w, a.N, a.Ktot = _ptr(w), N, Ktot
    a.nseg = len(segs)
    for i, s in enumerate(segs):
        t = _dev(s.t)
        g = a.seg[i]
        pitch = t.shape[-1]
        for d in range(t.dim() - 2, -1, -1):
            if t.shape[d] > 1:
                pitch = t.stride(d)
                break
        extent = 1 + sum((n - 1) * st for n, st in zip(t.shape, t.stride()))
        g.ptr, g.bytes, g.pitch = t.data_ptr(), extent * t.element_size(), pitch
        g.coff, g.len, g.dy, g.dx = s.coff, s.len, s.dy, s.dx
    Wo = M if Wo is None else Wo
    Wi = M if Wi is None else Wi
    a.M, a.Ho, a.Wo, a.Hi, a.Wi, a.stride, a.ups = M, Ho, Wo, Hi, Wi, stride, int(bool(ups))
    n_out = N // 2 if geglu else (vt_n0 if vt is not None else N)
    if out is None and n_out > 0:
        out = torch.empty((M, n_out), dtype=torch.uint8 if f8 is not None else (torch.float32 if out_f32 else w.dtype), device=w.device)
    if f8 is not None:
        if (out is not None and out.dtype != torch.uint8) or (vt is not None and vt.dtype != torch.uint8):
            raise TypeError("gemm_conv(f8=...): out / vt must be uint8 (e4m3 bytes)")
        a.f8_out_scale, a.f8_vt_scale = float(f8[0]), float(f8[1])
    a.io_flags = ffi.IO_OUT_F8 if f8 is not None else (
        (ffi.IO_RES_F32 if res is not None and res.dtype == torch.float32 else 0) |
        (ffi.IO_OUT_F32 if out is not None and out.dtype == torch.float32 else 0) |
        (ffi.IO_BIAS_F32 if bias is not None and bias.dtype == torch.float32 else 0))
    a.out = _ptr(out)
    a.ldo = (ldo if ldo is not None else (out.stride(-2) if out is not None else 0))
    a.bias = _ptr(bias)
    a.rowbias, a.rowbias_ld, a.rows_per_group = _ptr(rowbias), rowbias_ld, rows_per_group
    a.res = _ptr(res)
    a.ldr = (ldr if ldr is not None else (res.stride(-2) if res is not None else 0))
    a.mode = ffi.EPI_GEGLU if geglu else (ffi.EPI_GELU if gelu else (ffi.EPI_QUICKGELU if quick_gelu else ffi.EPI_NONE))
    xa, xflops = None, 0.0
    if xattn is not None:
        xa = ffi.XAttn()
        xa.nseg, xa.tokens, xa.ip_scale = len(xattn["segs"]), xattn["tokens"], xattn.get("ip_scale", 1.0)
        for i, sg in enumerate(xattn["segs"]):
            xa.k[i], xa.vt[i], xa.ldk[i], xa.ldvt[i], xa.nk[i], xa.k_rows[i] = _ptr(sg["k"]), _ptr(sg["vt"]), sg["ldk"], sg["ldvt"], sg["nk"], sg["k_rows"]
            xflops += 4.0 * M * N * sg["nk"]
        a.mode, a.xattn = ffi.EPI_XATTN, C.pointer(xa)
    a.vt, a.vt_n0, a.vt_tokens = _ptr(vt), vt_n0, vt_tokens
    a.vt_perm = int(bool(vt_perm)) if vt is not None else 0
    a.colscale_n, a.colscale = colscale_n, colscale
    a.tile_hint = tile_hint if tile_hint else _TUNE["gemm"].get(gemm_key(a), 0)
    if RECORD is not None:
        RECORD.append(("gemm", gemm_key(a), type(a).from_buffer_copy(a), (segs, w, out, bias, rowbias, res, vt, xa, xattn)))
    seen, xbytes = set(), 0
    for sg in segs:
        if sg.t.data_ptr() not in seen:
            seen.add(sg.t.data_ptr())
            xbytes += sg.t.numel() * sg.t.element_size()
    esz = w.element_size()
    obytes = (M * (N // 2 if geglu else N)) * (out.element_size() if out is not None else esz) + (M * N * res.element_size() if res is not None else 0)
    _call("idmvton_gemm_conv", a, flops=2.0 * M * N * Ktot + xflops, bytes_=float(xbytes + N * Ktot * esz + obytes))
    return out


def xattn_q_weight(w):
    return w.index_select(0, key_order_index(w.shape[0], w.device)).contiguous()


def key_order_index(n, device=None):
    if n % 16:
        raise ValueError("key order needs a multiple of 16 keys, got %d" % n)
    i = torch.arange(n, device=device)
    return (i & ~12) | ((i & 4) << 1) | ((i & 8) >> 1)


def key_order(vt):
    return vt.index_select(-1, key_order_index(vt.shape[-1], vt.device)).contiguous()


def round16(n):
    return (n + 15) // 16 * 16


def linear(x, w, **kw):
    M, K = x.shape
    return gemm_conv([SegSpec(x, 0, K)], w, M, **kw)


def conv_segs(x, k, pad, coff=0, length=None):
    length = x.shape[-1] if length is None else length
    return [SegSpec(x, coff, length, ky - pad, kx - pad) for ky in range(k) for kx in range(k)]


QSCALE = 0.125 * 1.4426950408889634


def attention(q, out, segs, heads, *, mode=ffi.ATTN_SELF, ip_scale=1.0, B=None, Nq=None, ldq=None, ldo=None, tune=0, q_prescaled=False):
    a = ffi.AttnArgs()
    a.dtype, a.mode = _dt(q), mode
    a.B = q.shape[0] if B is None else B
    a.Nq = q.shape[1] if Nq is None else Nq
    a.heads = heads
    a.q, a.ldq = _ptr(q), (q.stride(-2) if ldq is None else ldq)
    a.out, a.ldo = _ptr(out), (out.stride(-2) if ldo is None else ldo)
    a.nseg = len(segs)
    for i, s in enumerate(segs):
        a.k[i], a.vt[i] = _ptr(s["k"]), _ptr(s["vt"])
        a.ldk[i], a.ldvt[i] = s["ldk"], s["ldvt"]
        a.nk[i], a.k_rows[i], a.seg_b0[i] = s["nk"], s.get("k_rows", 0), s.get("b0", 0)
    a.ip_scale = ip_scale
    a.q_prescaled = int(bool(q_prescaled))
    a.tune = tune
    if not tune:
        t = _TUNE["attn"].get(attn_key(a), 0)
        a.tune = t if (q_prescaled or ((t >> 16) & 0xff) not in (7, 8, 16)) else 0
    if RECORD is not None:
        RECORD.append(("attn", attn_key(a), type(a).from_buffer_copy(a), (q, out, segs)))
    fl = 0.0
    for s in segs:
        fl += 4.0 * (a.B - s.get("b0", 0)) * heads * a.Nq * s["nk"] * 64
    nb, ix, nkt = _seg_nb(segs), _seg_index(segs, a.B), _seg_nk(segs, a.B)
    _call("idmvton_attn_fwd_ragged" if nkt else "idmvton_attn_fwd_indexed" if ix else "idmvton_attn_fwd_shared" if nb else "idmvton_attn_fwd", a, flops=fl,
          bytes_=2.0 * a.B * a.Nq * heads * 64 * q.element_size(), seg_nb=nb or ([0, 0] if ix or nkt else None), seg_index=ix, seg_nk=nkt)
    return out


def _seg_nb(segs):
    nb = [int(s.get("nb", 0) or 0) for s in segs] + [0] * (2 - len(segs))
    return nb if any(nb) else None


def _seg_index(segs, B):
    ix = []
    for s in segs:
        t = s.get("index")
        if t is not None:
            if not (isinstance(t, torch.Tensor) and t.dtype == torch.int32 and t.is_cuda and t.is_contiguous() and t.numel() == B - s.get("b0", 0)):
                raise ValueError(f"attention: a segment's index must be a contiguous int32 device tensor of B - b0 = {B - s.get('b0', 0)} entries")
            if int(s.get("nb", 0) or 0) < 1:
                raise ValueError("attention: a segment with index= needs nb= (the number of elements it holds)")
        ix.append(0 if t is None else t.data_ptr())
    ix += [0] * (2 - len(ix))
    return ix if any(ix) else None


def _seg_nk(segs, B):
    nk = []
    for s in segs:
        t = s.get("nk_table")
        if t is not None and not (isinstance(t, torch.Tensor) and t.dtype == torch.int32 and t.is_cuda and t.is_contiguous() and t.numel() == B):
            raise ValueError(f"attention: a segment's nk_table must be a contiguous int32 device tensor of B = {B} entries")
        nk.append(0 if t is None else t.data_ptr())
    nk += [0] * (2 - len(nk))
    return nk if any(nk) else None


def quant_f8(src, scale, mode=0, out=None):
    rows, cols = src.shape
    ldd = cols if mode == 0 else (cols + 63) // 64 * 64
    if out is None:
        out = torch.empty((rows, ldd), dtype=torch.uint8, device=src.device)
    a = ffi.QuantF8Args()
    a.dtype, a.mode, a.rows, a.cols = _dt(src), mode, rows, cols
    a.src, a.lds, a.dst, a.ldd, a.scale = _ptr(src), src.stride(0), _ptr(out), out.stride(0), scale
    _call("idmvton_quant_f8", a, bytes_=float(rows * cols * (src.element_size() + 1)))
    return out


KV_UNPACK_CHUNK = 1024
KV_UNPACK_MAX_N = 65534


class KvUnpackTable:

    def __init__(self, host, device):
        self.host = host.contiguous()
        self.n = self.host.shape[0]
        lo = lambda c: self.host[:, c] & 0xffffffff
        self.items = lo(3) * ((self.host[:, 3] >> 32) >> 4)
        self.dev = self.host.to(device)

    def launch(self, dtype, first=0, count=None):
        count = self.n - first if count is None else count
        if first % 2 or first < 0 or count < 1 or first + count > self.n:
            raise ValueError(f"kv_unpack: descriptors [{first}, {first + count}) of {self.n} (an even first index, at least one descriptor)")
        for f0 in range(first, first + count, KV_UNPACK_MAX_N):
            c = min(KV_UNPACK_MAX_N, first + count - f0)
            a = ffi.KvUnpackArgs()
            a.dtype, a.n, a.desc = _DT[dtype], c, self.dev.data_ptr() + 40 * f0
            a.max_chunks = (int(self.items[f0:f0 + c].max()) + KV_UNPACK_CHUNK - 1) // KV_UNPACK_CHUNK
            launch = lambda: ffi.call_kv_unpack(a, self.host.data_ptr() + 40 * f0, _stream())
            if PROFILE is None:
                launch()
                continue
            e0, e1 = torch.cuda.Event(enable_timing=True), torch.cuda.Event(enable_timing=True)
            e0.record()
            launch()
            e1.record()
            PROFILE.append(("idmvton_kv_unpack", e0, e1, 0.0, 48.0 * float(self.items[f0:f0 + c].sum())))


def kv_unpack_rows(src, dst, exp, rows, cols, lds, ldd):
    t = lambda v: v if isinstance(v, torch.Tensor) else torch.tensor(v, dtype=torch.int64)
    src, dst, exp, rows, cols, lds, ldd = torch.broadcast_tensors(*[t(v) for v in (src, dst, exp, rows, cols, lds, ldd)])
    return torch.stack([src, dst, exp, rows | (cols << 32), lds | (ldd << 32)], dim=-1)


def kv_unpack(descs, dtype, device=None):
    if not isinstance(descs, KvUnpackTable):
        rec = []
        for src, dst, exp in descs:
            if src.dtype != torch.uint8 or dst.dtype != dtype or exp.dtype != torch.int32 or exp.numel() != 1 or src.dim() != 2 or src.shape != dst.shape or \
                    src.stride(1) != 1 or dst.stride(1) != 1:
                raise ValueError("kv_unpack: a run is (uint8 [rows][cols], %s [rows][cols], one int32), rows contiguous" % dtype)
            rows, cols = src.shape
            rec.append((_ptr(src), _ptr(dst), _ptr(exp), rows | (cols << 32), src.stride(0) | (dst.stride(0) << 32)))
        device = descs[0][0].device if device is None else device
        descs = KvUnpackTable(torch.tensor(rec, dtype=torch.int64).reshape(-1, 5), device)
    descs.launch(dtype)
    return descs


KV_STREAM_CHUNK = 1024
KV_STREAM_MAX_N = 1 << 20
KV_STREAM_WORKGROUPS = 16


def stream_address(t):
    if t.is_cuda:
        return t.data_ptr()
    if not t.is_pinned():
        raise ValueError("kv_stream: a host tensor that a kernel reads must be page-locked (pin_memory=True); this one is pageable")
    return ffi.host_device_ptr(t.data_ptr())


def kv_stream_first(items):
    chunks = (items + KV_STREAM_CHUNK - 1) // KV_STREAM_CHUNK
    return torch.cat([torch.zeros(1, dtype=torch.int64), torch.cumsum(chunks, 0)]).to(torch.int32)


class KvStreamTable:
    ENTRY = "kv_stream"

    def __init__(self, host, device, mode=ffi.KVS_WIDEN_E4M3, slices=None):
        self.host, self.mode = host.contiguous(), mode
        self.n = self.host.shape[0]
        self.slices = [(0, self.n)] if slices is None else [(int(f), int(c)) for f, c in slices]
        for f, c in self.slices:
            if f % 2 or f < 0 or c < 1 or c > KV_STREAM_MAX_N or f + c > self.n:
                raise ValueError(f"kv_stream: descriptors [{f}, {f + c}) of {self.n} (an even first index, 1 to {KV_STREAM_MAX_N} descriptors)")
        self.items = (self.host[:, 3] & 0xffffffff) * ((self.host[:, 3] >> 32) >> 4)
        firsts = [kv_stream_first(self.items[f:f + c]) for f, c in self.slices]
        self.first_at, at = [], 0
        for t in firsts:
            self.first_at.append(at)
            at += t.numel()
        self.first_host = torch.cat(firsts).contiguous()
        self.dev, self.first_dev = self.host.to(device), self.first_host.to(device)

    def launch(self, dtype, which=0, workgroups=None):
        f0, c = self.slices[which]
        a = ffi.KvStreamArgs()
        a.dtype, a.mode, a.n, a.workgroups = _DT[dtype], self.mode, c, KV_STREAM_WORKGROUPS if workgroups is None else workgroups
        a.desc, a.first = self.dev.data_ptr() + 40 * f0, self.first_dev.data_ptr() + 4 * self.first_at[which]
        call = getattr(ffi, "call_" + self.ENTRY)
        launch = lambda: call(a, self.host.data_ptr() + 40 * f0, self.first_host.data_ptr() + 4 * self.first_at[which], _stream())
        if PROFILE is None:
            return launch()
        e0, e1 = torch.cuda.Event(enable_timing=True), torch.cuda.Event(enable_timing=True)
        e0.record()
        launch()
        e1.record()
        PROFILE.append(("idmvton_" + self.ENTRY, e0, e1, 0.0, self.bytes_moved(f0, c)))

    def bytes_moved(self, f0, c):
        return (48.0 if self.mode == ffi.KVS_WIDEN_E4M3 else 32.0) * float(self.items[f0:f0 + c].sum())


class KvFillTable(KvStreamTable):
    ENTRY = "kv_fill"

    def link_bytes(self, f0=0, c=None):
        c = self.n - f0 if c is None else c
        return 16.0 * float(self.items[f0:f0 + c][self.host[f0:f0 + c, 0] != 0].sum())

    def bytes_moved(self, f0, c):
        return self.link_bytes(f0, c) + (32.0 if self.mode == ffi.KVS_WIDEN_E4M3 else 16.0) * float(self.items[f0:f0 + c].sum())


def kv_pad_even(rec):
    if rec.shape[0] % 2 == 0:
        return rec
    items = (rec[:, 3] & 0xffffffff) * ((rec[:, 3] >> 32) >> 4)
    return torch.cat([rec, rec[int(items.argmin())].view(1, 5)])


def kv_stream(descs, dtype, mode=ffi.KVS_WIDEN_E4M3, workgroups=None, device=None):
    if not isinstance(descs, KvStreamTable):
        widen = mode == ffi.KVS_WIDEN_E4M3
        rec = []
        for src, dst, exp in descs:
            ok = src.dim() == 2 and src.shape == dst.shape and src.stride(1) == 1 and dst.stride(1) == 1 and dst.is_cuda
            if widen:
                ok = ok and src.dtype == torch.uint8 and dst.dtype == dtype and exp is not None and exp.dtype == torch.int32 and exp.numel() == 1
            else:
                ok = ok and src.dtype == dst.dtype
            if not ok:
                raise ValueError("kv_stream: a run is (uint8 [rows][cols], %s [rows][cols], one int32) when widening, (x [rows][cols], x [rows][cols], None) "
                                 "when copying; rows contiguous, the destination on the device" % dtype)
            rows, cols = src.shape
            sz = 1 if widen else src.element_size()
            rec.append((stream_address(src), _ptr(dst), stream_address(exp) if widen else 0, rows | ((cols * sz) << 32),
                        (src.stride(0) * sz) | ((dst.stride(0) * sz) << 32)))
        device = descs[0][1].device if device is None else device
        descs = KvStreamTable(torch.tensor(rec, dtype=torch.int64).reshape(-1, 5), device, mode)
    descs.launch(dtype, 0, workgroups)
    return descs


def kv_fill(descs, dtype, mode=ffi.KVS_WIDEN_E4M3, workgroups=None, device=None):
    if not isinstance(descs, KvStreamTable):
        widen = mode == ffi.KVS_WIDEN_E4M3
        rec = []
        for src, dst, exp in descs:
            ok = dst.dim() == 2 and dst.stride(1) == 1 and dst.is_cuda and (not widen or dst.dtype == dtype)
            if src is not None:
                ok = ok and src.dim() == 2 and src.shape == dst.shape and src.stride(1) == 1
                if widen:
                    ok = ok and src.dtype == torch.uint8 and exp is not None and exp.dtype == torch.int32 and exp.numel() == 1
                else:
                    ok = ok and src.dtype == dst.dtype
            if not ok:
                raise ValueError("kv_fill: a run is (uint8 [rows][cols], %s [rows][cols], one int32) when widening, (x [rows][cols], x [rows][cols], None) "
                                 "when copying, (None, dst [rows][cols], None) for a zero run; rows contiguous, the destination on the device" % dtype)
            rows, cols = dst.shape
            sz = 1 if widen else dst.element_size()
            if src is None:
                rec.append((0, _ptr(dst), 0, rows | ((cols * sz) << 32), (cols * sz) | ((dst.stride(0) * sz) << 32)))
            else:
                rec.append((stream_address(src), _ptr(dst), stream_address(exp) if widen else 0, rows | ((cols * sz) << 32),
                            (src.stride(0) * sz) | ((dst.stride(0) * sz) << 32)))
        device = descs[0][1].device if device is None else device
        descs = KvFillTable(torch.tensor(rec, dtype=torch.int64).reshape(-1, 5), device, mode)
    descs.launch(dtype, 0, workgroups)
    return descs


def attention_f8(q8, out, segs, heads, *, qk_scale_exp, v_scale_exp, B, Nq, ldq=None, ldo=None):
    a = ffi.AttnF8Args()
    a.out_dtype, a.B, a.heads, a.Nq = _dt(out), B, heads, Nq
    a.q8, a.ldq = _ptr(q8), (q8.stride(-2) if ldq is None else ldq)
    a.out, a.ldo = _ptr(out), (out.stride(-2) if ldo is None else ldo)
    a.nseg = len(segs)
    fl = 0.0
    for i, s in enumerate(segs):
        a.k8[i], a.vt8[i] = _ptr(s["k8"]), _ptr(s["vt8"])
        a.ldk[i], a.ldvt[i] = s["ldk"], s["ldvt"]
        a.nk[i], a.k_rows[i], a.seg_b0[i] = s["nk"], s.get("k_rows", 0), s.get("b0", 0)
        fl += 4.0 * (B - s.get("b0", 0)) * heads * Nq * s["nk"] * 64
    a.qk_scale_exp, a.v_scale_exp = qk_scale_exp, v_scale_exp
    nb, ix, nkt = _seg_nb(segs), _seg_index(segs, B), _seg_nk(segs, B)
    _call("idmvton_attn_f8_ragged" if nkt else "idmvton_attn_f8_indexed" if ix else "idmvton_attn_f8_shared" if nb else "idmvton_attn_f8", a, flops=fl,
          bytes_=float(B * Nq * heads * 64 * (1 + out.element_size())), seg_nb=nb or ([0, 0] if ix or nkt else None), seg_index=ix, seg_nk=nkt)
    return out


def attention_small(q, k, v, out, heads, d, *, scale, causal=False, B=None, Lq=None, Lk=None, ldq=None, ldk=None, ldv=None, ldo=None):
    a = ffi.AttnSmallArgs()
    a.dtype = _dt(q)
    a.B = q.shape[0] if B is None else B
    a.heads, a.d = heads, d
    a.Lq = q.shape[1] if Lq is None else Lq
    a.Lk = k.shape[1] if Lk is None else Lk
    a.q, a.ldq = _ptr(q), (q.stride(-2) if ldq is None else ldq)
    a.k, a.ldk = _ptr(k), (k.stride(-2) if ldk is None else ldk)
    a.v, a.ldv = _ptr(v), (v.stride(-2) if ldv is None else ldv)
    a.out, a.ldo = _ptr(out), (out.stride(-2) if ldo is None else ldo)
    a.scale, a.causal = scale, int(bool(causal))
    _call("idmvton_attn_small", a, flops=4.0 * a.B * heads * a.Lq * a.Lk * d)
    return out


def layernorm(x, gamma, beta, eps=1e-5, out=None, out2=None):
    rows, Cc = x.shape
    if out is None:
        out = torch.empty((rows, Cc), dtype=gamma.dtype, device=x.device)
    a = ffi.LayerNormArgs()
    a.dtype, a.rows, a.C = _dt(gamma), rows, Cc
    a.x_f32 = int(x.dtype == torch.float32)
    a.x, a.ldx = _ptr(x), x.stride(0)
    a.gamma, a.beta, a.eps = _ptr(gamma), _ptr(beta), eps
    a.y, a.ldy = _ptr(out), out.stride(0)
    a.y2, a.ldy2 = _ptr(out2), (out2.stride(0) if out2 is not None else 0)
    _call("idmvton_layernorm", a, bytes_=(x.element_size() + (1.0 + (out2 is not None)) * out.element_size()) * rows * Cc)
    return out


def groupnorm(x, gamma, beta, groups, eps, silu, stats, x2=None, out=None, split_dtype=None):
    B, HW, C1 = x.shape
    Cc = C1 + (x2.shape[-1] if x2 is not None else 0)
    prec = split_dtype is not None
    if prec and not (x.dtype == gamma.dtype == beta.dtype == torch.float32 and (x2 is None or x2.dtype == torch.float32)):
        raise TypeError("groupnorm(split_dtype=...): x, gamma and beta must be float32")
    if out is None:
        out = torch.empty((B, HW, 2 * Cc if prec else Cc), dtype=split_dtype if prec else x.dtype, device=x.device)
    a = ffi.GroupNormArgs()
    a.dtype, a.B, a.HW, a.C, a.groups = _dt(out), B, HW, Cc, groups
    a.flags = (ffi.GN_X_F32 | ffi.GN_Y_SPLIT | ffi.GN_AFFINE_F32) if prec else 0
    a.x, a.C1, a.x2 = _ptr(x), C1, _ptr(x2)
    a.gamma, a.beta, a.eps, a.silu = _ptr(gamma), _ptr(beta), eps, int(bool(silu))
    a.y, a.stats, a.stats_doubles = _ptr(out), _ptr(stats), stats.numel()
    _call("idmvton_groupnorm", a, bytes_=(2.0 * x.element_size() + (2 if prec else 1) * out.element_size()) * B * HW * Cc)
    return out


GN_STATS_DOUBLES = 2 * 32 * (2048 + 2 * 64 + 64)


def gn_stats_doubles(B, HW, C, groups):
    return ffi.lib().idmvton_groupnorm_stats_doubles(B, HW, C, groups)


def pack_input(latents, cond, out):
    a = ffi.PackInputArgs()
    B, hw = latents.shape[0], latents.shape[2] * latents.shape[3] if latents.dim() == 4 else latents.shape[2]
    a.dtype, a.B, a.hw, a.cpad = _dt(out), B, hw, out.shape[-1]
    a.latents, a.cond, a.out = _ptr(latents), _ptr(cond), _ptr(out)
    _call("idmvton_pack_input", a)
    return out


def cfg_step(eps_nhwc, latents, noise, coef):
    a = ffi.CfgStepArgs()
    B = latents.shape[0]
    hw = latents.numel() // (B * 4)
    a.dtype, a.B, a.hw, a.ldc = _dt(eps_nhwc), B, hw, eps_nhwc.shape[-1]
    a.eps_nhwc, a.latents, a.noise, a.coef = _ptr(eps_nhwc), _ptr(latents), _ptr(noise), _ptr(coef)
    _call("idmvton_cfg_step", a)
    return latents


def to_nhwc(src_nchw_f32, dtype, cpad=None, scale=1.0, shift=0.0, out=None, split=False):
    B, Cc = src_nchw_f32.shape[:2]
    HW = src_nchw_f32.numel() // (B * Cc)
    cpad = Cc if cpad is None else cpad
    if out is None:
        out = torch.empty((B, HW, 2 * cpad if split else cpad), dtype=dtype, device=src_nchw_f32.device)
    a = ffi.LayoutArgs()
    a.flags = ffi.LAYOUT_SPLIT if split else 0
    a.dtype, a.B, a.C, a.HW, a.cpad, a.to_nhwc = _dt(out), B, Cc, HW, cpad, 1
    a.src, a.dst, a.scale, a.shift = _ptr(src_nchw_f32), _ptr(out), scale, shift
    _call("idmvton_layout", a)
    return out


def to_nchw(src_nhwc, Cc, shape_hw, scale=1.0, shift=0.0, out=None):
    B, HW, cpad = src_nhwc.shape
    if out is None:
        out = torch.empty((B, Cc) + tuple(shape_hw), dtype=torch.float32, device=src_nhwc.device)
    a = ffi.LayoutArgs()
    f32 = src_nhwc.dtype == torch.float32
    a.flags = ffi.LAYOUT_NHWC_F32 if f32 else 0
    a.dtype, a.B, a.C, a.HW, a.cpad, a.to_nhwc = (ffi.BF16 if f32 else _dt(src_nhwc)), B, Cc, HW, cpad, 0
    a.src, a.dst, a.scale, a.shift = _ptr(src_nhwc), _ptr(out), scale, shift
    _call("idmvton_layout", a)
    return out


def vae_sample(moments_nhwc, noise, scale, out=None):
    B, hw, ldm = moments_nhwc.shape
    if out is None:
        out = torch.empty_like(noise)
    a = ffi.VaeSampleArgs()
    a.dtype, a.B, a.hw, a.ldm = _dt(moments_nhwc), B, hw, ldm
    a.moments, a.noise, a.z, a.scale = _ptr(moments_nhwc), _ptr(noise), _ptr(out), scale
    _call("idmvton_vae_sample", a)
    return out


def softmax_rows(x, scale, n_valid=0):
    a = ffi.SoftmaxArgs()
    a.dtype, a.rows, a.n, a.ld = _dt(x), x.shape[0], x.shape[1], x.stride(0)
    a.x, a.scale, a.n_valid = _ptr(x), scale, n_valid
    _call("idmvton_softmax_rows", a)
    return x


def softmax_rows_split(x, scale, dtype, n_valid=0, out=None):
    rows, n = x.shape
    if out is None:
        out = torch.empty((rows, 2 * n), dtype=dtype, device=x.device)
    elif tuple(out.shape) != (rows, 2 * n) or out.dtype != dtype:
        raise ValueError(f"softmax_rows_split(out=...): needs shape {(rows, 2 * n)} of {dtype}, got {tuple(out.shape)} of {out.dtype}")
    a = ffi.SoftmaxArgs()
    a.n_valid = n_valid
    a.dtype, a.rows, a.n, a.ld = _dt(out), rows, n, x.stride(0)
    a.x, a.scale, a.y_split, a.ldy = _ptr(x), scale, _ptr(out), out.stride(0)
    _call("idmvton_softmax_rows", a, bytes_=float(rows * n * (3 * 4 + 2 * out.element_size())))
    return out


def split(x, dtype, mode=ffi.SPLIT_ACT, out=None):
    rows, cols = x.shape
    shape = {ffi.SPLIT_ACT: (rows, 2 * cols), ffi.SPLIT_W3: (rows, 3 * cols), ffi.SPLIT_W3T: (cols, 3 * rows)}[mode]
    if out is None:
        out = torch.empty(shape, dtype=dtype, device=x.device)
    elif tuple(out.shape) != shape or out.dtype != dtype:
        raise ValueError(f"split(out=...): needs shape {shape} of {dtype}, got {tuple(out.shape)} of {out.dtype}")
    a = ffi.SplitArgs()
    a.dtype, a.mode, a.rows, a.cols = _dt(out), mode, rows, cols
    a.src, a.lds, a.dst, a.ldd = _ptr(x), x.stride(0), _ptr(out), out.stride(0)
    _call("idmvton_split", a, bytes_=float(rows * cols * 4 + out.numel() * out.element_size()))
    return out


def probe_mfma(which, a, b):
    c = torch.empty((64, 16), dtype=torch.float32, device=a.device)
    rc = ffi.lib().idmvton_probe_mfma(which, C.c_void_p(a.data_ptr()), C.c_void_p(b.data_ptr()),
                                      C.c_void_p(c.data_ptr()), C.c_void_p(_stream()))
    if rc != 0:
        raise RuntimeError(ffi.lib().idmvton_last_error().decode())
    return c


load_tune()
```

### idm-vton_amd/pipeline.py

```python
import torch

from . import ops
from .garment_cache import (GarmentCache, PackedGarmentCache, ShelvedGarmentCache, alloc_kv, fill_records, index_runs, kv_shapes, shelf_records,
                            slot_run, timestep_run)
from .scheduler import StepScheduler


def drive_blocks(blocks, garment, tryon, main=None, side=None, ready=None, free=None):
    if side is None:
        for bi in range(len(blocks)):
            garment(bi, 0)
            if tryon(bi, 0):
                return
        return
    garment(0, 0)
    side.wait_stream(main)
    for bi in range(len(blocks)):
        cur, nxt = bi & 1, (bi + 1) & 1
        if bi + 1 < len(blocks):
            with torch.cuda.stream(side):
                if bi >= 1:
                    side.wait_event(free[nxt])
                garment(bi + 1, nxt)
                ready[nxt].record(side)
        if bi >= 1:
            main.wait_event(ready[cur])
        tryon(bi, cur)
        free[cur].record(main)
    main.wait_stream(side)


def _copy_state(G, st):
    for name in ("latents", "cond", "cloth_k", "gix", "gnk"):
        if G.get(name) is not None:
            G[name].copy_(st[name])
    for name in ("ctx_t", "ctx_gk"):
        if name in G:
            for p, ent in st[name]["kv"].items():
                for kind, t in ent.items():
                    G[name]["kv"][p][kind].copy_(t)


def _is_attn1_kv(key):
    return ".attn1.to_k." in key or ".attn1.to_v." in key


class TryonEngine:
    def __init__(self, unet, unet_encoder, vae, resampler=None, dtype=torch.bfloat16, device="cuda"):
        self.unet, self.unet_encoder, self.vae, self.resampler = unet, unet_encoder, vae, resampler
        self.dtype, self.device = dtype, torch.device(device)
        self._graphs = {}
        self._set_shapes = {}
        self._side = None
        self.garment_steps = 6
        self.ramp = True
        self.stats = dict(garment_batches=0, garment_set_copies=0, garment_stream_launches=0)
        self._streaming = []
        self._weights_id = None

    @staticmethod
    def _timesteps(scheduler, num_inference_steps, strength):
        sched = StepScheduler(scheduler)
        timesteps = sched.set_timesteps(num_inference_steps)
        init_t = min(int(num_inference_steps * strength), num_inference_steps)
        timesteps = timesteps[max(num_inference_steps - init_t, 0):]
        if len(timesteps) < 1:
            raise ValueError(f"After adjusting the num_inference_steps by strength parameter: {strength}, the number of pipeline"
                             f"steps is {len(timesteps)} which is < 1 and not appropriate for this pipeline.")
        return sched, timesteps

    def _block_schedule(self, n):
        k = max(1, min(self.garment_steps, n))
        sizes, s0 = [], 0
        for c in (1, 2, 4):
            if c < k and s0 + c <= n and self.ramp:
                sizes.append(c); s0 += c
        while s0 < n:
            sizes.append(min(k, n - s0)); s0 += sizes[-1]
        blocks, s0 = [], 0
        for c in sizes:
            blocks.append((s0, c)); s0 += c
        return k, blocks

    def _garment_inputs(self, cloth_lat, text_embeds_cloth, timesteps, B):
        dev, dt = self.device, self.dtype
        cloth_nhwc = ops.to_nhwc(cloth_lat, dt, cpad=self.unet_encoder.cin_pad)
        ctx_g = self.unet_encoder.encode_context(text_embeds_cloth.to(dev))
        temb_g = self.unet_encoder.time_embeddings(timesteps, B)
        n = len(timesteps)
        k, blocks = self._block_schedule(n)
        tidx = torch.tensor([[min(s0 + j, n - 1) for j in range(k)] for s0, _ in blocks], device=dev)
        temb_gk = temb_g[tidx].reshape(len(blocks), k * B, -1).contiguous()
        cloth_k = cloth_nhwc.repeat(k, 1, 1).contiguous()
        ctx_gk = ctx_g if k == 1 else self.unet_encoder.encode_context(text_embeds_cloth.to(dev).repeat(k, 1, 1))
        return dict(cloth=cloth_nhwc, ctx_g=ctx_g, temb_g=temb_g, k=k, blocks=blocks, temb_gk=temb_gk, cloth_k=cloth_k, ctx_gk=ctx_gk)

    @staticmethod
    def _garment_latent_size(cloth):
        Hg, Wg = cloth.shape[-2:]
        if Hg % 8 or Wg % 8:
            raise ValueError(f"`cloth` height and width have to be divisible by 8 but are {Hg} and {Wg}.")
        return Hg // 8, Wg // 8

    @staticmethod
    def _set_key(st):
        return (st["B"], st["gh"], st["gw"], st["k"])

    @staticmethod
    def _graph_key(st, live):
        if live:
            return (st["B"], st["h"], st["w"], st["gh"], st["gw"], st["k"], st["steps_noise"] is not None)
        return (st["B"], st["h"], st["w"], st["gh"], st["gw"], st["k"], st["steps_noise"] is not None, "cached",
                "indexed" if st.get("gindex") is not None else st["gcache"].G) + (("ragged",) if st.get("gnk") is not None else ())

    def weights_identity(self):
        if self._weights_id is None:
            self._weights_id = self.unet_encoder.weights_id() + ":" + self.unet.weights_id(_is_attn1_kv)
        return self._weights_id

    @torch.no_grad()
    def encode_garment(self, *, cloth, text_embeds_cloth, noise_cloth, num_inference_steps, scheduler="ddpm", strength=1.0,
                       height=None, width=None, storage="native"):
        dev = self.device
        f32 = lambda t: t.to(dev, torch.float32).contiguous()
        cloth, nz = f32(cloth), f32(noise_cloth)
        G = cloth.shape[0]
        Hg, Wg = cloth.shape[-2:]
        H = height or Hg
        W = width or Wg
        if H % 8 or W % 8:
            raise ValueError(f"`height` and `width` have to be divisible by 8 but are {H} and {W}.")
        gh, gw = self._garment_latent_size(cloth)
        h, w = H // 8, W // 8
        _, timesteps = self._timesteps(scheduler, num_inference_steps, strength)
        if (Hg, Wg) == (H, W):
            cloth_lat = self.vae.encode_sample(torch.cat([cloth, cloth, cloth]), torch.cat([nz, nz, nz]))[2 * G:]
        else:
            cloth_lat = self.vae.encode_sample(cloth, nz)
        gs = dict(B=G, gh=gh, gw=gw, **self._garment_inputs(cloth_lat, text_embeds_cloth, timesteps, G))
        n, k = len(timesteps), gs["k"]
        fs, ks = self._discover_set_shapes(gs)
        feats = [torch.empty(sh, dtype=self.dtype, device=dev) for sh in fs]
        if storage == "e4m3":
            return self._encode_packed(gs, feats, ks, timesteps, h, w)
        if storage != "native":
            raise ValueError(f"encode_garment: storage={storage!r} (\"native\" or \"e4m3\")")
        kv = alloc_kv(ks, k, n, dev)
        for bi, (s0, c) in enumerate(gs["blocks"]):
            self._garment_side(gs, gs["temb_gk"][bi], dict(feats=feats, kv=timestep_run(kv, n, G, s0, c)), c)
        return GarmentCache(G=G, timesteps=timesteps, h=h, w=w, gh=gh, gw=gw, dtype=self.dtype, attn_fp8=self.unet.attn_fp8, f8_exp=self.unet.f8_exp,
                            weights_id=self.weights_identity(), kv=kv)

    def _encode_packed(self, gs, feats, ks, timesteps, h, w):
        if self.unet.attn_fp8:
            raise ValueError("encode_garment(storage=\"e4m3\"): an attn_fp8 engine's cache cannot be packed (its features already are e4m3 operands)")
        G, n, k, dev = gs["B"], len(timesteps), gs["k"], self.device
        blk = alloc_kv(ks, k, k, dev)
        meta = dict(G=G, timesteps=timesteps, h=h, w=w, gh=gs["gh"], gw=gs["gw"], dtype=self.dtype, attn_fp8=False, f8_exp=self.unet.f8_exp,
                    weights_id=self.weights_identity())
        amax = None
        for bi, (s0, c) in enumerate(gs["blocks"]):
            self._garment_side(gs, gs["temb_gk"][bi], dict(feats=feats, kv=timestep_run(blk, k, G, 0, c)), c)
            m = torch.stack([torch.stack([t.reshape(c, G, -1).abs().amax(dim=(0, 2)).float() for t in kvf], dim=-1)
                             for kvf in timestep_run(blk, k, G, 0, c)], dim=1)
            amax = m if amax is None else torch.maximum(amax, m)
        from .garment_cache import pack_exponent
        exps = pack_exponent(amax)
        kv = alloc_kv([(a, b, torch.uint8) for a, b, _ in ks], k, n, dev)
        for bi, (s0, c) in enumerate(gs["blocks"]):
            views = timestep_run(blk, k, G, 0, c)
            self._garment_side(gs, gs["temb_gk"][bi], dict(feats=feats, kv=views), c)
            part = GarmentCache(**{**meta, "timesteps": timesteps[s0:s0 + c], "kv": views}).pack(exps)
            for (dk, dv), (sk, sv) in zip(timestep_run(kv, n, G, s0, c), part.kv):
                dk.copy_(sk)
                dv.copy_(sv)
        self.stats["garment_batches"] -= len(gs["blocks"])
        return PackedGarmentCache(exps=exps, kv=kv, **meta)

    def empty_garment_cache(self, G, garment_height, garment_width, num_inference_steps, scheduler="ddpm", strength=1.0, height=None, width=None):
        if garment_height % 8 or garment_width % 8:
            raise ValueError(f"`garment_height` and `garment_width` have to be divisible by 8 but are {garment_height} and {garment_width}.")
        H, W = height or garment_height, width or garment_width
        if H % 8 or W % 8:
            raise ValueError(f"`height` and `width` have to be divisible by 8 but are {H} and {W}.")
        if G < 1:
            raise ValueError(f"empty_garment_cache: G = {G} < 1")
        gh, gw = garment_height // 8, garment_width // 8
        _, timesteps = self._timesteps(scheduler, num_inference_steps, strength)
        n = len(timesteps)
        kv = []
        for blk, tokens in zip(self.unet.block_order, self.unet.feature_tokens(gh, gw)):
            C, N = blk["qkv"].shape[1], ops.round16(tokens)
            kv.append((torch.empty(n * G * N, C, dtype=self.dtype, device=self.device), torch.empty(n * G, C, N, dtype=self.dtype, device=self.device)))
        return GarmentCache(G=G, timesteps=timesteps, h=H // 8, w=W // 8, gh=gh, gw=gw, dtype=self.dtype, attn_fp8=self.unet.attn_fp8,
                            f8_exp=self.unet.f8_exp, weights_id=self.weights_identity(), kv=kv, sizes=[(gh, gw)] * G)

    @torch.no_grad()
    def prepare(self, *, image, mask_image, pose_img, cloth, prompt_embeds, negative_prompt_embeds, pooled_prompt_embeds,
                negative_pooled_prompt_embeds, text_embeds_cloth, noise, num_inference_steps, guidance_scale,
                ip_hidden_states=None, image_embeds=None, scheduler="ddpm", height=None, width=None, strength=1.0,
                image_dtype=None, garment_index=None):
        dev, dt = self.device, self.dtype
        self._release_streamed()
        f32 = lambda t: t.to(dev, torch.float32).contiguous()
        gcache = cloth if isinstance(cloth, GarmentCache) else None
        if garment_index is not None and gcache is None:
            raise ValueError("garment_index names garments of a GarmentCache: pass one as `cloth=` (a live call encodes one garment per person)")
        gindex = None
        if gcache is not None and gcache.sizes is not None and garment_index is None:
            raise ValueError("a GarmentCache with `sizes` holds garments of several sizes: pass garment_index (person i wears garment "
                             "garment_index[i]; the i % G rule of a plain cache does not apply)")
        if gcache is not None:
            gidx = gcache.check(timesteps=self._timesteps(scheduler, num_inference_steps, strength)[1],
                                h=(height or image.shape[-2]) // 8, w=(width or image.shape[-1]) // 8, dtype=dt, attn_fp8=self.unet.attn_fp8,
                                f8_exp=self.unet.f8_exp, weights_id=self.weights_identity(), persons=image.shape[0], garment_index=garment_index)
            if garment_index is not None:
                gidx, gindex = gidx
            if gcache.host_resident:
                self._check_host_cache(gcache)
        image, mask_image, pose_img = f32(image), f32(mask_image), f32(pose_img)
        cloth = f32(cloth) if gcache is None else None
        B = image.shape[0]
        H = height or image.shape[-2]
        W = width or image.shape[-1]
        h, w = H // 8, W // 8
        gh, gw = self._garment_latent_size(cloth) if gcache is None else (gcache.gh, gcache.gw)
        if H % 8 or W % 8:
            raise ValueError(f"`height` and `width` have to be divisible by 8 but are {H} and {W}.")
        start_is_given = bool(noise.get("latents_given"))
        if strength < 1.0 and noise.get("image") is None and not start_is_given:
            raise ValueError("strength < 1 starts from add_noise(encode(image)): pass the posterior draw of the init-image encode as "
                             "noise['image'] (the reference's first random draw, tryon_pipeline.py:883-889), or set noise['latents_given'] "
                             "when noise['latents'] already is the start (the reference's `latents=` argument)")
        sched, timesteps = self._timesteps(scheduler, num_inference_steps, strength)
        if guidance_scale <= 1:
            guidance_scale = 1.0
            if negative_prompt_embeds is None:
                negative_prompt_embeds = torch.zeros_like(prompt_embeds)
            if negative_pooled_prompt_embeds is None:
                negative_pooled_prompt_embeds = torch.zeros_like(pooled_prompt_embeds)
            if ip_hidden_states is not None and ip_hidden_states.shape[0] == B:
                ip_hidden_states = torch.cat([torch.zeros_like(ip_hidden_states), ip_hidden_states])
            if image_embeds is not None and image_embeds.shape[0] == B:
                image_embeds = torch.cat([torch.zeros_like(image_embeds), image_embeds])

        init_image = 2.0 * image - 1.0
        mask = (mask_image >= 0.5).float()
        masked_image = init_image * (mask < 0.5)
        if strength == 1.0 or start_is_given:
            latents = f32(noise["latents"]) * sched.init_noise_sigma
        else:
            src = init_image if image_dtype is None else init_image.to(image_dtype).float()
            ab = float(sched.alphas_cumprod[int(timesteps[0])])
            latents = ab ** 0.5 * self.vae.encode_sample(src, f32(noise["image"])) + (1.0 - ab) ** 0.5 * f32(noise["latents"])
        mask_l = torch.nn.functional.interpolate(mask, size=(h, w))
        if gcache is None and tuple(cloth.shape[-2:]) == (H, W):
            enc = self.vae.encode_sample(torch.cat([masked_image, pose_img, cloth]),
                                         torch.cat([f32(noise["masked"]), f32(noise["pose"]), f32(noise["cloth"])]))
            masked_lat, pose_lat, cloth_lat = enc[:B], enc[B:2 * B], enc[2 * B:]
        else:
            enc = self.vae.encode_sample(torch.cat([masked_image, pose_img]), torch.cat([f32(noise["masked"]), f32(noise["pose"])]))
            masked_lat, pose_lat, cloth_lat = enc[:B], enc[B:], None
            if gcache is None:
                cloth_lat = self.vae.encode_sample(cloth, f32(noise["cloth"]))
        cond = torch.cat([mask_l, masked_lat, pose_lat], dim=1).permute(0, 2, 3, 1).reshape(B, h * w, 9)
        cond = torch.cat([cond, cond], dim=0).to(dt).contiguous()

        pe = torch.cat([negative_prompt_embeds, prompt_embeds], dim=0).to(dev)
        add_text = torch.cat([negative_pooled_prompt_embeds, pooled_prompt_embeds], dim=0).to(dev)
        time_ids = torch.tensor([[H, W, 0, 0, H, W]], dtype=torch.float32, device=dev).repeat(2 * B, 1)
        if image_embeds is None:
            image_embeds = self.resampler(ip_hidden_states.to(dev))
        ctx_t = self.unet.encode_context(pe, image_embeds)
        temb_t = self.unet.time_embeddings(timesteps, 2 * B, dict(text_embeds=add_text, time_ids=time_ids))
        if gcache is None:
            garm = dict(self._garment_inputs(cloth_lat, text_embeds_cloth, timesteps, B), gcache=None, gidx=None, garment_persons=None,
                        gindex=None, gix=None, gnk=None)
        else:
            k, blocks = self._block_schedule(len(timesteps))
            if gcache.sizes is not None:
                per = [self.unet.feature_tokens(*sz) for sz in gcache.garment_sizes(gindex)]
                gnk = torch.tensor([[p[f] for p in per] * 2 for f in range(len(per[0]))], dtype=torch.int32, device=dev)
            garm = dict(cloth=None, ctx_g=None, temb_g=None, k=k, blocks=blocks, temb_gk=None, cloth_k=None, ctx_gk=None,
                        gcache=gcache, gidx=gidx, garment_persons=B, gindex=gindex,
                        gix=torch.tensor(gindex, dtype=torch.int32, device=dev) if gindex is not None else None,
                        gnk=gnk if gcache.sizes is not None else None)
        coef = torch.tensor([list(sched.coeffs(t)) + [guidance_scale] for t in timesteps], dtype=torch.float32, device=dev)
        steps_noise = f32(noise["steps"]) if noise.get("steps") is not None and scheduler == "ddpm" else None
        return dict(B=B, h=h, w=w, gh=gh, gw=gw, timesteps=timesteps, latents=latents.contiguous(), cond=cond,
                    ctx_t=ctx_t, temb_t=temb_t, coef=coef, steps_noise=steps_noise, **garm,
                    x_in=torch.empty(2 * B, h * w, self.unet.cin_pad, dtype=dt, device=dev),
                    trace=dict(masked_lat=masked_lat, pose_lat=pose_lat, cloth_lat=cloth_lat, image_embeds=image_embeds))

    def _garment_side(self, st, temb_gk, fset, c=None):
        B, h, w = st["B"], st["gh"], st["gw"]
        c = st["k"] if c is None else c
        self.stats["garment_batches"] += 1
        _, feats = self.unet_encoder.forward(st["cloth_k"][:c * B], temb_gk[:c * B], st["ctx_gk"], c * B, h, w, feats_buf=fset["feats"])
        self.unet.project_garment_kv(feats, out=fset["kv"])

    def _tryon_main(self, st, temb_t, coef, noise, kv_j):
        B, h, w = st["B"], st["h"], st["w"]
        ops.pack_input(st["latents"], st["cond"], st["x_in"])
        eps, _ = self.unet.forward(st["x_in"], temb_t, st["ctx_t"], 2 * B, h, w, garment_kv=kv_j, garment_persons=st["garment_persons"],
                                   garment_hw=(st["gh"], st["gw"]), garment_index=st.get("gix"), garment_nk=st.get("gnk"))
        ops.cfg_step(eps, st["latents"], noise, coef)
        return eps

    def _discover_set_shapes(self, st):
        B, h, w, k = st["B"], st["gh"], st["gw"], st["k"]
        key = self._set_key(st)
        if key not in self._set_shapes:
            _, feats = self.unet_encoder.forward(st["cloth_k"], st["temb_gk"][0], st["ctx_gk"], k * B, h, w)
            kv = self.unet.project_garment_kv(feats)
            self._set_shapes[key] = ([tuple(f.shape) for f in feats], kv_shapes(kv))
        return self._set_shapes[key]

    def _alloc_set(self, feat_shapes, shapes, n, k, G):
        kv = alloc_kv(shapes, n, k, self.device)
        return dict(feats=[torch.empty(sh, dtype=self.dtype, device=self.device) for sh in feat_shapes], kv=kv,
                    step=[timestep_run(kv, k, G, j) for j in range(k)])

    def _new_set(self, st):
        fs, ks = self._discover_set_shapes(st)
        return self._alloc_set(fs, ks, st["k"], st["k"], st["B"])

    def _fill_set(self, st, fset, s0, c):
        gc, idx = st["gcache"], st["gidx"][s0:s0 + c]
        self.stats["garment_set_copies"] += 1
        if st["gindex"] is not None:
            n, P = len(gc.timesteps), st["B"]
            runs = index_runs(list(dict.fromkeys(st["gindex"])))
            for j, i in enumerate(idx):
                for d0, g0, cc in runs:
                    for (dk, dv), (sk, sv) in zip(slot_run(fset["kv"], st["k"], P, j, d0, cc), slot_run(gc.kv, n, gc.G, i, g0, cc)):
                        dk.copy_(sk)
                        dv.copy_(sv)
            return
        runs = [(0, idx[0], c)] if idx == list(range(idx[0], idx[0] + c)) else [(j, i, 1) for j, i in enumerate(idx)]
        for j0, i0, cc in runs:
            for (dk, dv), (sk, sv) in zip(timestep_run(fset["kv"], st["k"], gc.G, j0, cc), gc.run(i0, cc)):
                dk.copy_(sk)
                dv.copy_(sv)

    @staticmethod
    def _cache_set_shapes(st):
        gc = st["gcache"]
        slots = gc.G if st["gindex"] is None else st["B"]
        if isinstance(gc, ShelvedGarmentCache):
            n = len(gc.timesteps)
            return slots, [((n * slots * a[0], a[1]), (n * slots, b[0], b[1]), gc.dtype) for a, b in gc.slot_shapes]
        dt = lambda d: gc.dtype if gc.packed else d
        return slots, [((a[0] // gc.G * slots,) + a[1:], (b[0] // gc.G * slots,) + b[1:], dt(d)) for a, b, d in kv_shapes(gc.kv)]

    def _check_host_cache(self, gc):
        if self.unet.attn_fp8:
            raise ValueError("host-resident GarmentCache attn_fp8 mismatch: an attn_fp8 engine does not stream a cache from host memory "
                             "(move it with .to(device))")
        if isinstance(gc, ShelvedGarmentCache):
            for part in gc.parts:
                self._check_host_cache(part)
            return
        if gc.sizes is not None:
            raise ValueError("host-resident GarmentCache sizes mismatch: a cache with `sizes` (slotted / mixed_sizes) is not streamed from host "
                             "memory (move it with .to(device))")
        if not all(k.is_pinned() and vt.is_pinned() for k, vt in gc.kv):
            raise ValueError("host-resident GarmentCache kv mismatch: the tensors are pageable host memory; the device reads page-locked memory "
                             "only -- make the cache with .to(\"cpu\", pin_memory=True) or GarmentPool(resident=\"host\")")
        if gc.packed and not gc.exps.is_pinned():
            raise ValueError("host-resident GarmentCache exps mismatch: the exponents are pageable host memory; the device reads page-locked "
                             "memory only -- make the cache with .to(\"cpu\", pin_memory=True) or GarmentPool(resident=\"host\")")

    def _release_streamed(self):
        self._streaming = [h for h in self._streaming if not h[1].query()]

    def _stream_fill(self, st, sets, blocks=None):
        gc, k = st["gcache"], st["k"]
        if isinstance(gc, ShelvedGarmentCache):
            return self._shelf_fill(st, sets, blocks)
        n = len(gc.timesteps)
        garments = list(range(gc.G)) if st["gindex"] is None else list(dict.fromkeys(st["gindex"]))
        S = gc.G if st["gindex"] is None else st["B"]
        built = [bi for bi in range(len(st["blocks"])) if blocks is None or bi in blocks]
        steps = [(st["blocks"][bi][0] + j, j) for bi in built for j in range(st["blocks"][bi][1])]
        first = {i: at for at, (i, _) in enumerate(steps)}
        per = len(garments) * len(gc.kv) * 2
        addr = {}

        def address(t):
            if t.data_ptr() not in addr:
                addr[t.data_ptr()] = ops.stream_address(t)
            return addr[t.data_ptr()]
        rec = torch.cat([fill_records(gc.kv, n, gc.G, fs["kv"], k, S, gc.exps if gc.packed else None, [st["gidx"][i] for i, _ in steps],
                                      [j for _, j in steps], garments, list(range(len(garments))), address=address) for fs in sets])
        which = {(p, bi): at for at, (p, bi) in enumerate((p, bi) for p in range(len(sets)) for bi in built)}
        table = ops.KvStreamTable(rec, self.device, ops.ffi.KVS_WIDEN_E4M3 if gc.packed else ops.ffi.KVS_COPY,
                                  [((p * len(steps) + first[st["blocks"][bi][0]]) * per, st["blocks"][bi][1] * per) for p, bi in which])
        self._release_streamed()
        hold = [gc, torch.cuda.Event()]
        self._streaming.append(hold)

        def garment(bi, p):
            self.stats["garment_stream_launches"] += 1
            table.launch(self.dtype, which[(p, bi)])
            hold[1].record()
        return garment

    def _shelf_fill(self, st, sets, blocks=None):
        gc, k = st["gcache"], st["k"]
        garments = list(dict.fromkeys(st["gindex"]))
        S = st["B"]
        built = [bi for bi in range(len(st["blocks"])) if blocks is None or bi in blocks]
        steps = [(st["blocks"][bi][0] + j, j) for bi in built for j in range(st["blocks"][bi][1])]
        first = {i: at for at, (i, _) in enumerate(steps)}
        addr = {}

        def address(t):
            if t.data_ptr() not in addr:
                addr[t.data_ptr()] = ops.stream_address(t)
            return addr[t.data_ptr()]
        parts = [gc.parts[g] for g in garments]
        recs = [shelf_records(parts, gc.packed, fs["kv"], k, S, [st["gidx"][i] for i, _ in steps], [j for _, j in steps],
                              list(range(len(garments))), address=address) for fs in sets]
        per = recs[0][1]
        which = {(p, bi): at for at, (p, bi) in enumerate((p, bi) for p in range(len(sets)) for bi in built)}
        table = ops.KvFillTable(torch.cat([r for r, _ in recs]), self.device, ops.ffi.KVS_WIDEN_E4M3 if gc.packed else ops.ffi.KVS_COPY,
                                [((p * len(steps) + first[st["blocks"][bi][0]]) * per, st["blocks"][bi][1] * per) for p, bi in which])
        self._release_streamed()
        hold = [gc, torch.cuda.Event()]
        self._streaming.append(hold)

        def garment(bi, p):
            self.stats["garment_stream_launches"] += 1
            table.launch(self.dtype, which[(p, bi)])
            hold[1].record()
        return garment

    def _packed_fill(self, st, sets, blocks=None):
        gc, k = st["gcache"], st["k"]
        n = len(gc.timesteps)
        garments = list(range(gc.G)) if st["gindex"] is None else list(dict.fromkeys(st["gindex"]))
        S = gc.G if st["gindex"] is None else st["B"]
        steps = [(s0 + j, j) for bi, (s0, c) in enumerate(st["blocks"]) if blocks is None or bi in blocks for j in range(c)]
        first = {i: at for at, (i, _) in enumerate(steps)}
        per = len(garments) * len(gc.kv) * 2
        rec = torch.cat([fill_records(gc.kv, n, gc.G, fs["kv"], k, S, gc.exps, [st["gidx"][i] for i, _ in steps], [j for _, j in steps], garments,
                                      list(range(len(garments)))) for fs in sets])
        table = ops.KvUnpackTable(rec, self.device)

        def garment(bi, p):
            s0, c = st["blocks"][bi]
            self.stats["garment_set_copies"] += 1
            table.launch(self.dtype, (p * len(steps) + first[s0]) * per, c * per)
        return garment

    def _slot_table(self, st):
        if st["gindex"] is None:
            return None
        slot = {g: u for u, g in enumerate(dict.fromkeys(st["gindex"]))}
        return torch.tensor([slot[g] for g in st["gindex"]], dtype=torch.int32, device=self.device)

    def _noise(self, st, i):
        return st["steps_noise"][i] if st["steps_noise"] is not None else None

    def _eager_form(self, st, live, overlap):
        blocks = st["blocks"]
        if live:
            sets = [self._new_set(st) for _ in range(2 if overlap else 1)]
            garment = lambda bi, p: self._garment_side(st, st["temb_gk"][bi], sets[p], blocks[bi][1])
            kv = lambda i, j, p: sets[p]["step"][j]
        elif st["gcache"].packed or st["gcache"].host_resident:
            slots, shapes = self._cache_set_shapes(st)
            sets = [self._alloc_set((), shapes, len(st["gcache"].timesteps), st["k"], slots) for _ in range(2 if overlap else 1)]
            garment = (self._stream_fill if st["gcache"].host_resident else self._packed_fill)(st, sets)
            st = dict(st, gix=self._slot_table(st))
            kv = lambda i, j, p: sets[p]["step"][j]
        else:
            overlap = False
            garment = lambda bi, p: None
            kv = lambda i, j, p: st["gcache"].step(st["gidx"][i])
        step = lambda i, j, p: self._tryon_main(st, st["temb_t"][i], st["coef"][i], self._noise(st, i), kv(i, j, p))
        if not overlap:
            return garment, step, st["latents"], None
        if self._side is None:
            self._side = torch.cuda.Stream()
        ready, free = [torch.cuda.Event(), torch.cuda.Event()], [torch.cuda.Event(), torch.cuda.Event()]
        return garment, step, st["latents"], (self._side, ready, free)

    def _graph_state(self, st, live):
        has_noise = st["steps_noise"] is not None
        key = self._graph_key(st, live)
        if key in self._graphs:
            return self._graphs[key]
        G = {name: st[name] for name in ("B", "h", "w", "gh", "gw", "k", "garment_persons", "latents", "cond", "x_in", "ctx_t")}
        G["gix"] = self._slot_table(st)
        G["gnk"] = st["gnk"].clone() if st.get("gnk") is not None else None
        G.update(tt=st["temb_t"][0].clone(), cf=st["coef"][0].clone(), nz=st["steps_noise"][0].clone() if has_noise else None, graphs={},
                 side=torch.cuda.Stream(), ready=[torch.cuda.Event(), torch.cuda.Event()], free=[torch.cuda.Event(), torch.cuda.Event()],
                 pools=dict(tryon=torch.cuda.graph_pool_handle(), garm=torch.cuda.graph_pool_handle()))
        saved = st["latents"].clone()
        warm = torch.cuda.Stream()
        warm.wait_stream(torch.cuda.current_stream())
        with torch.cuda.stream(warm):
            if live:
                G.update(cloth_k=st["cloth_k"], ctx_gk=st["ctx_gk"], tgk=st["temb_gk"][0].clone())
                G["sets"] = [self._new_set(st), self._new_set(st)]
                self._garment_side(G, G["tgk"], G["sets"][0])
            else:
                gc = st["gcache"]
                slots, shapes = self._cache_set_shapes(st)
                G["sets"] = [self._alloc_set((), shapes, len(gc.timesteps), st["k"], slots) for _ in range(2)]
                if gc.host_resident:
                    self._stream_fill(st, G["sets"][:1], blocks=(0,))(0, 0)
                elif gc.packed:
                    self._packed_fill(st, G["sets"][:1], blocks=(0,))(0, 0)
                else:
                    self._fill_set(st, G["sets"][0], *st["blocks"][0])
            self._tryon_main(G, G["tt"], G["cf"], G["nz"], G["sets"][0]["step"][0])
        torch.cuda.current_stream().wait_stream(warm)
        torch.cuda.synchronize()
        self._release_streamed()
        st["latents"].copy_(saved)
        self._graphs[key] = G
        return G

    def _graph(self, G, kind, par, j=0):
        gk = (kind, par, j)
        if gk in G["graphs"]:
            return G["graphs"][gk]
        keep = G["latents"].clone()
        torch.cuda.synchronize()
        g = torch.cuda.CUDAGraph()
        with torch.cuda.graph(g, pool=G["pools"][kind], capture_error_mode="thread_local"):
            if kind == "garm":
                self._garment_side(G, G["tgk"], G["sets"][par], j)
                self.stats["garment_batches"] -= 1
            else:
                self._tryon_main(G, G["tt"], G["cf"], G["nz"], G["sets"][par]["step"][j])
        G["latents"].copy_(keep)
        G["graphs"][gk] = g
        return g

    def _graph_form(self, st, live, overlap):
        G = self._graph_state(st, live)
        if G["latents"] is not st["latents"]:
            _copy_state(G, dict(st, gix=self._slot_table(st)))
        blocks, graphs = st["blocks"], G["graphs"]
        for p in ((0, 1) if overlap and len(blocks) > 1 else (0,)):
            for j in range(st["k"]):
                self._graph(G, "tryon", p, j)
        if live:
            for bi, (_, c) in enumerate(blocks):
                self._graph(G, "garm", (bi & 1) if overlap else 0, c)

            def garment(bi, p):
                G["tgk"].copy_(st["temb_gk"][bi])
                self.stats["garment_batches"] += 1
                graphs[("garm", p, blocks[bi][1])].replay()
        elif st["gcache"].host_resident:
            garment = self._stream_fill(st, G["sets"])
        elif st["gcache"].packed:
            garment = self._packed_fill(st, G["sets"])
        else:
            garment = lambda bi, p: self._fill_set(st, G["sets"][p], *blocks[bi])
        tt, cf, nz = G["tt"], G["cf"], G["nz"]

        def step(i, j, p):
            tt.copy_(st["temb_t"][i]); cf.copy_(st["coef"][i])
            if nz is not None:
                nz.copy_(st["steps_noise"][i])
            graphs[("tryon", p, j)].replay()

        return garment, step, G["latents"], (G["side"], G["ready"], G["free"]) if overlap else None

    @torch.no_grad()
    def denoise(self, st, use_graph=False, trace=None, overlap=False, on_step=None):
        if on_step is not None:
            use_graph = overlap = False
        live = st["gcache"] is None
        garment, step, latents, sync = (self._graph_form if use_graph else self._eager_form)(st, live, overlap)
        blocks = st["blocks"]

        def tryon(bi, p):
            s0, c = blocks[bi]
            for j in range(c):
                i = s0 + j
                step(i, j, p)
                if trace is not None:
                    trace.setdefault("step_latents", []).append(latents.clone())
                if on_step is not None and on_step(i, int(st["timesteps"][i]), latents):
                    return True

        if sync is None:
            drive_blocks(blocks, garment, tryon)
        else:
            drive_blocks(blocks, garment, tryon, torch.cuda.current_stream(), *sync)
        return latents

    @torch.no_grad()
    def decode(self, latents):
        self._release_streamed()
        img = self.vae.decode(latents / self.vae.cfg.scaling_factor)
        return (img / 2 + 0.5).clamp(0, 1)

    @torch.no_grad()
    def __call__(self, *, return_latents=False, use_graph=False, overlap=False, timing=None, on_step=None, **kw):
        ev = [torch.cuda.Event(enable_timing=True) for _ in range(4)] if timing is not None else None
        if ev:
            ev[0].record()
        st = self.prepare(**kw)
        if ev:
            ev[1].record()
        lat = self.denoise(st, use_graph=use_graph, overlap=overlap, on_step=on_step)
        if ev:
            ev[2].record()
        out = lat if return_latents else self.decode(lat)
        if ev:
            ev[3].record()
            timing.append(tuple(ev))
        return out
```

### idm-vton_amd/unet.py

```python
import math
import os

import torch

from . import ffi, ops
from .config import UNetConfig, unet_topology
from .weights import conv_weight_nhwc, conv_weight_nhwc_padded, interleave_geglu


def _pad64(c):
    return (c + 63) // 64 * 64


class _Conv:

    def __init__(self, sd, name, cin_pad=None, shortcut=None, pad_out_to=None):
        w = sd[name + ".weight"]
        b = sd[name + ".bias"]
        self.k = w.shape[-1]
        self.cin = w.shape[1]
        self.cin_pad = cin_pad or self.cin
        wk = conv_weight_nhwc_padded(w, self.cin_pad) if self.cin_pad != self.cin else conv_weight_nhwc(w)
        if shortcut is not None:
            ws = sd[shortcut + ".weight"]
            wk = torch.cat([wk, ws.reshape(ws.shape[0], ws.shape[1])], dim=1)
            b = (b.float() + sd[shortcut + ".bias"].float()).to(b.dtype)
        self.cout = w.shape[0]
        if pad_out_to and pad_out_to > self.cout:
            wk = torch.cat([wk, torch.zeros(pad_out_to - self.cout, wk.shape[1], dtype=wk.dtype, device=wk.device)])
            b = torch.cat([b, torch.zeros(pad_out_to - self.cout, dtype=b.dtype, device=b.device)])
        self.w = wk.contiguous()
        self.b = b.contiguous()
        self.n = self.w.shape[0]


class HipUNet:
    def __init__(self, cfg: UNetConfig, state_dict, dtype=torch.bfloat16, device="cuda", stream_f32=False, attn_fp8=False, fuse_xattn=True):
        self.cfg, self.dtype, self.device = cfg, dtype, torch.device(device)
        self.stream_f32 = bool(stream_f32)
        self.attn_fp8 = bool(attn_fp8)
        self.fuse_xattn = bool(fuse_xattn) and os.environ.get("IDMVTON_FUSE_XATTN", "1") != "0"
        self.f8_exp = (2, 2, 2)
        self.f8_fused = os.environ.get("IDMVTON_F8_FUSED", "1") != "0"
        self.topo = unet_topology(cfg)
        sd = {k: v.to(device=self.device, dtype=dtype) for k, v in state_dict.items() if not k.startswith("encoder_hid_proj.")}
        self.sd = sd
        for h, c in zip(cfg.num_attention_heads, cfg.block_out_channels):
            assert c % 64 == 0 and (c // h == 64), "HIP attention kernels are specialised for head_dim 64"
        self.tryon = cfg.mode == "tryon"
        self.ip_scale = 1.0
        self.cin_pad = _pad64(cfg.in_channels)
        self._prep()
        self._gn_stats = torch.empty(ops.GN_STATS_DOUBLES, dtype=torch.float64, device=self.device)
        self._ctx = None

    def _prep(self):
        sd, cfg = self.sd, self.cfg
        self.conv_in = _Conv(sd, "conv_in", cin_pad=self.cin_pad)
        self.res = {}
        self.tf = {}
        temb_w, temb_b, self.temb_slices, off = [], [], {}, 0

        def prep_res(p, cin, cout):
            sc = p + ".conv_shortcut" if cin != cout else None
            self.res[p] = dict(conv1=_Conv(sd, p + ".conv1"), conv2=_Conv(sd, p + ".conv2", shortcut=sc), cin=cin, cout=cout)
            nonlocal off
            temb_w.append(sd[p + ".time_emb_proj.weight"])
            temb_b.append(sd[p + ".time_emb_proj.bias"])
            self.temb_slices[p] = (off, cout)
            off += cout

        def prep_tf(p, ch, n_tf, heads, level):
            blocks = []
            for k in range(n_tf):
                b = f"{p}.transformer_blocks.{k}"
                d = dict(heads=heads)
                d["qkv"] = torch.cat([sd[f"{b}.attn1.to_q.weight"], sd[f"{b}.attn1.to_k.weight"], sd[f"{b}.attn1.to_v.weight"]]).contiguous()
                d["kv_text"] = torch.cat([sd[f"{b}.attn2.to_k.weight"], sd[f"{b}.attn2.to_v.weight"]]).contiguous()
                if self.tryon:
                    d["kv_ip"] = torch.cat([sd[f"{b}.attn2.processor.to_k_ip.weight"], sd[f"{b}.attn2.processor.to_v_ip.weight"]]).contiguous()
                d["ff1_w"], d["ff1_b"] = interleave_geglu(sd[f"{b}.ff.net.0.proj.weight"], sd[f"{b}.ff.net.0.proj.bias"])
                d["p"] = b
                blocks.append(d)
            self.tf[p] = dict(blocks=blocks, ch=ch, heads=heads, level=level)

        level = 0
        for i, blk in enumerate(self.topo["down"]):
            for j, (ci, co) in enumerate(blk["resnets"]):
                prep_res(f"down_blocks.{i}.resnets.{j}", ci, co)
                if blk["attn"]:
                    prep_tf(f"down_blocks.{i}.attentions.{j}", blk["ch"], blk["n_tf"], blk["heads"], level)
            if blk["down"]:
                self.res[f"down_blocks.{i}.downsamplers.0.conv"] = _Conv(sd, f"down_blocks.{i}.downsamplers.0.conv")
                level += 1
        m = self.topo["mid"]
        prep_res("mid_block.resnets.0", m["ch"], m["ch"])
        prep_tf("mid_block.attentions.0", m["ch"], m["n_tf"], m["heads"], level)
        prep_res("mid_block.resnets.1", m["ch"], m["ch"])
        for i, blk in enumerate(self.topo["up"]):
            if self.tryon or blk["attn"]:
                for j, (rin, skip, co) in enumerate(blk["resnets"]):
                    prep_res(f"up_blocks.{i}.resnets.{j}", rin + skip, co)
                    if blk["attn"]:
                        prep_tf(f"up_blocks.{i}.attentions.{j}", blk["ch"], blk["n_tf"], blk["heads"], level)
                if blk["up"]:
                    self.res[f"up_blocks.{i}.upsamplers.0.conv"] = _Conv(sd, f"up_blocks.{i}.upsamplers.0.conv")
            if blk["up"]:
                level -= 1
        self.block_order = [blk for tf in self.tf.values() for blk in tf["blocks"]]
        self.temb_w = torch.cat(temb_w).contiguous()
        self.temb_b = torch.cat(temb_b).contiguous()
        if self.tryon:
            self.conv_out = _Conv(sd, "conv_out", pad_out_to=_pad64(cfg.out_channels) if cfg.out_channels % 4 else None)

    def time_embeddings(self, timesteps, batch, added_cond=None):
        cfg, sd, dt = self.cfg, self.sd, self.dtype
        ts = torch.as_tensor(timesteps, dtype=torch.float32, device=self.device).reshape(-1)
        half = cfg.block_out_channels[0] // 2
        freq = torch.exp(-math.log(10000.0) * torch.arange(half, dtype=torch.float32, device=self.device) / half)
        ang = ts[:, None] * freq[None, :]
        t_emb = torch.cat([torch.cos(ang), torch.sin(ang)], dim=-1).to(dt)
        S = ts.numel()
        mp = max(S, 1)
        e = ops.linear(t_emb.contiguous(), sd["time_embedding.linear_1.weight"], bias=sd["time_embedding.linear_1.bias"])
        e = ops.linear(torch.nn.functional.silu(e.float()).to(dt), sd["time_embedding.linear_2.weight"], bias=sd["time_embedding.linear_2.bias"])
        emb = e[:, None, :].expand(S, batch, -1)
        if cfg.addition_embed_type == "text_time":
            text_embeds, time_ids = added_cond["text_embeds"], added_cond["time_ids"]
            h2 = cfg.addition_time_embed_dim // 2
            f2 = torch.exp(-math.log(10000.0) * torch.arange(h2, dtype=torch.float32, device=self.device) / h2)
            a2 = time_ids.to(self.device).float().flatten()[:, None] * f2[None, :]
            te = torch.cat([torch.cos(a2), torch.sin(a2)], dim=-1).reshape(batch, -1)
            add = torch.cat([text_embeds.to(self.device).float(), te], dim=-1).to(dt).contiguous()
            a = ops.linear(add, sd["add_embedding.linear_1.weight"], bias=sd["add_embedding.linear_1.bias"])
            a = ops.linear(torch.nn.functional.silu(a.float()).to(dt), sd["add_embedding.linear_2.weight"], bias=sd["add_embedding.linear_2.bias"])
            emb = (emb.float() + a.float()[None]).to(dt)
        x = torch.nn.functional.silu(emb.float()).to(dt).reshape(S * batch, -1).contiguous()
        out = ops.linear(x, self.temb_w, bias=self.temb_b)
        return out.reshape(S, batch, -1)

    def encode_context(self, text, ip=None):
        dt, dev = self.dtype, self.device
        B, nt, xd = text.shape
        rt = (nt + 31) // 32 * 32
        tpad = torch.zeros(B, rt, xd, dtype=dt, device=dev)
        tpad[:, :nt] = text.to(dev, dt)
        ctx = dict(B=B, nt=nt, rt=rt, kv={})
        if ip is not None:
            ni = ip.shape[1]
            ri = (ni + 31) // 32 * 32
            ipad = torch.zeros(B, ri, xd, dtype=dt, device=dev)
            ipad[:, :ni] = ip.to(dev, dt)
            ctx.update(ni=ni, ri=ri)
        for p, tf in self.tf.items():
            C = tf["ch"]
            for blk in tf["blocks"]:
                kt = torch.empty(B * rt, C, dtype=dt, device=dev)
                vtt = torch.empty(B, C, rt, dtype=dt, device=dev)
                ops.linear(tpad.reshape(B * rt, xd), blk["kv_text"], out=kt, vt=vtt, vt_n0=C, vt_tokens=rt)
                ent = dict(kt=kt, vtt=vtt)
                if ip is not None:
                    ki = torch.empty(B * ri, C, dtype=dt, device=dev)
                    vti = torch.empty(B, C, ri, dtype=dt, device=dev)
                    ops.linear(ipad.reshape(B * ri, xd), blk["kv_ip"], out=ki, vt=vti, vt_n0=C, vt_tokens=ri)
                    ent.update(ki=ki, vti=vti)
                ctx["kv"][blk["p"]] = ent
        return ctx

    def _gn(self, xa, xb, name, eps, silu):
        sd = self.sd
        return ops.groupnorm(xa, sd[name + ".weight"], sd[name + ".bias"], self.cfg.norm_num_groups, eps, silu,
                             self._gn_stats, x2=xb)

    def _conv3(self, x, cv, B, H, W, stride=1, ups=False, extra_segs=(), out_hw=None, **kw):
        Ho, Wo = (out_hw or (H * 2, W * 2)) if ups else ((H + 2 - 3) // stride + 1, (W + 2 - 3) // stride + 1)
        segs = ops.conv_segs(x, 3, 1, length=cv.cin_pad) + list(extra_segs)
        out = ops.gemm_conv(segs, cv.w, B * Ho * Wo, Ho=Ho, Wo=Wo, Hi=H, Wi=W, stride=stride, ups=ups, bias=cv.b, **kw)
        return out.view(B, Ho * Wo, cv.n), Ho, Wo

    def _resnet(self, p, xa, xb, temb, B, H, W):
        r = self.res[p]
        eps = self.cfg.norm_eps
        g1 = self._gn(xa, xb, p + ".norm1", eps, True)
        off, co = self.temb_slices[p]
        h, _, _ = self._conv3(g1, r["conv1"], B, H, W, rowbias=temb[:, off:off + co], rowbias_ld=temb.stride(0),
                              rows_per_group=H * W)
        g2 = self._gn(h, None, p + ".norm2", eps, True)
        if r["cin"] != r["cout"]:
            extra = [ops.SegSpec(xa, 0, xa.shape[-1])] + ([ops.SegSpec(xb, 0, xb.shape[-1])] if xb is not None else [])
            out, _, _ = self._conv3(g2, r["conv2"], B, H, W, extra_segs=extra)
        else:
            out, _, _ = self._conv3(g2, r["conv2"], B, H, W, res=xa.reshape(B * H * W, -1))
        return out

    def _block(self, blk, hs, B, N, C, ctx, garment, feats_out, stop=None, last=False, nk=None):
        sd, p, heads = self.sd, blk["p"], blk["heads"]
        dt, dev = self.dtype, self.device
        M = B * N
        nk = N if nk is None else nk
        feat = None
        if not self.tryon:
            fb = garment.get("feats_buf") if garment else None
            feat = fb[len(feats_out)][:B].view(M, C) if fb is not None else torch.empty(M, C, dtype=dt, device=dev)
        f8 = self._f8_fused(N)
        eq, ek, ev = self.f8_exp
        f8kw = dict(f8=(2.0 ** ek, 2.0 ** ev)) if f8 else {}
        qk = torch.empty(M, 2 * C, dtype=torch.uint8 if f8 else dt, device=dev)
        vt = torch.empty(B, C, N, dtype=torch.uint8 if f8 else dt, device=dev)
        qcs = ops.QSCALE * (2.0 ** (eq - ek) if f8 else 1.0)
        n1 = ops.layernorm(hs, sd[p + ".norm1.weight"], sd[p + ".norm1.bias"], 1e-5, out2=feat)
        if feat is not None:
            feats_out.append(feat.view(B, N, C))
            if stop is not None and len(feats_out) >= stop:
                return None
        ops.linear(n1, blk["qkv"], out=qk, vt=vt, vt_n0=2 * C, vt_tokens=N, colscale_n=C, colscale=qcs, **f8kw)
        segs = [dict(k=qk[:, C:], vt=vt, nk=nk, ldk=2 * C, ldvt=N, k_rows=N)]
        if self.tryon:
            gnk = garment["nk"][garment["idx"]] if garment.get("nk") is not None else None
            if garment.get("kv") is not None:
                kg, vtg = garment["kv"][garment["idx"]]
                Bg, Ng = vtg.shape[0], vtg.shape[2]
                if gnk is None:
                    if Ng != N:
                        raise ValueError(f"garment K / V^T of {Ng} token rows against {N} own rows: pass garment_hw (the garment's latent size)")
                    gnk = nk
            else:
                g = garment["feats"][garment["idx"]]
                Bg = g.shape[0]
                if gnk is None:
                    gnk = nk if g.shape[1] == N else g.shape[1]
                Ng = ops.round16(gnk)
                if g.shape[1] != Ng:
                    gp = torch.zeros(Bg, Ng, C, dtype=dt, device=dev)
                    gp[:, :g.shape[1]] = g
                    g = gp
                f8g = self._f8_fused(Ng)
                kg = torch.empty(Bg * Ng, C, dtype=torch.uint8 if f8g else dt, device=dev)
                vtg = torch.empty(Bg, C, Ng, dtype=torch.uint8 if f8g else dt, device=dev)
                ops.linear(g.reshape(Bg * Ng, C), blk["qkv"][C:], out=kg, vt=vtg, vt_n0=C, vt_tokens=Ng,
                           **(dict(f8=(2.0 ** ek, 2.0 ** ev)) if f8g else {}))
            garment["idx"] += 1
            gix = garment.get("index")
            P = gix.numel() if gix is not None else garment.get("persons") or Bg
            gseg = dict(k=kg, vt=vtg, nk=gnk, ldk=C, ldvt=Ng, k_rows=Ng, b0=B - P)
            if gix is not None:
                gseg.update(nb=Bg, index=gix)
            elif Bg < P:
                gseg["nb"] = Bg
            if garment.get("nk_table") is not None:
                gseg["nk_table"] = garment["nk_table"][garment["idx"] - 1]
            segs.append(gseg)
        att = torch.empty(M, C, dtype=dt, device=dev)
        if self.attn_fp8:
            segs8 = []
            for sg in segs:
                Bs, Ns = sg["vt"].shape[0], sg["k_rows"]
                if sg["k"].dtype == torch.uint8:
                    segs8.append(dict(k8=sg["k"], vt8=sg["vt"], nk=sg["nk"], ldk=sg["ldk"], ldvt=sg["ldvt"], k_rows=Ns, b0=sg.get("b0", 0), nb=sg.get("nb", 0),
                                      index=sg.get("index"), nk_table=sg.get("nk_table")))
                    continue
                k8 = ops.quant_f8(sg["k"], 2.0 ** ek)
                vt8 = ops.quant_f8(sg["vt"].reshape(Bs * C, Ns), 2.0 ** ev, mode=1)
                segs8.append(dict(k8=k8, vt8=vt8, nk=sg["nk"], ldk=C, ldvt=vt8.shape[1], k_rows=Ns, b0=sg.get("b0", 0), nb=sg.get("nb", 0), index=sg.get("index"),
                                  nk_table=sg.get("nk_table")))
            if f8:
                q8, ldq8 = qk, 2 * C
            else:
                q8, ldq8 = ops.quant_f8(qk[:, :C], 2.0 ** eq), C
            ops.attention_f8(q8, att, segs8, heads, qk_scale_exp=-(eq + ek), v_scale_exp=-ev, B=B, Nq=N, ldq=ldq8, ldo=C)
        else:
            ops.attention(qk, att, segs, heads, B=B, Nq=N, ldq=2 * C, ldo=C, q_prescaled=True)
        f32 = hs.dtype == torch.float32
        hs = ops.linear(att, sd[p + ".attn1.to_out.0.weight"], bias=sd[p + ".attn1.to_out.0.bias"], res=hs, out_f32=f32)
        kv = ctx["kv"][p]
        seg_t = dict(k=kv["kt"], vt=kv["vtt"], nk=ctx["nt"], ldk=C, ldvt=ctx["rt"], k_rows=ctx["rt"])
        xsegs = [seg_t] + ([dict(k=kv["ki"], vt=kv["vti"], nk=ctx["ni"], ldk=C, ldvt=ctx["ri"], k_rows=ctx["ri"])] if self.tryon else [])
        if self.fuse_xattn and N % 32 == 0 and not (C >= 1280 and M >= 8192) and \
                all(sg["nk"] <= (96, 32)[i] and sg["k_rows"] >= (sg["nk"] + 31) // 32 * 32 for i, sg in enumerate(xsegs)):
            if "q2_xw" not in blk:
                blk["q2_xw"] = ops.xattn_q_weight(sd[p + ".attn2.to_q.weight"])
            n2 = ops.layernorm(hs, sd[p + ".norm2.weight"], sd[p + ".norm2.bias"], 1e-5)
            att2 = ops.linear(n2, blk["q2_xw"], xattn=dict(segs=xsegs, tokens=N, ip_scale=self.ip_scale))
        else:
            n2 = ops.layernorm(hs, sd[p + ".norm2.weight"], sd[p + ".norm2.bias"], 1e-5)
            q2 = ops.linear(n2, sd[p + ".attn2.to_q.weight"])
            att2 = torch.empty(M, C, dtype=dt, device=dev)
            if self.tryon:
                ops.attention(q2, att2, xsegs, heads, mode=ffi.ATTN_CROSS, ip_scale=self.ip_scale, B=B, Nq=N, ldq=C, ldo=C)
            else:
                ops.attention(q2, att2, xsegs, heads, B=B, Nq=N, ldq=C, ldo=C)
        hs = ops.linear(att2, sd[p + ".attn2.to_out.0.weight"], bias=sd[p + ".attn2.to_out.0.bias"], res=hs, out_f32=f32)
        n3 = ops.layernorm(hs, sd[p + ".norm3.weight"], sd[p + ".norm3.bias"], 1e-5)
        gg = ops.linear(n3, blk["ff1_w"], bias=blk["ff1_b"], geglu=True)
        hs = ops.linear(gg, sd[p + ".ff.net.2.weight"], bias=sd[p + ".ff.net.2.bias"], res=hs, out_f32=f32 and not last)
        return hs

    def _transformer(self, p, x, B, H, W, ctx, garment, feats_out, stop_after_feats=None):
        sd, tf = self.sd, self.tf[p]
        C, N = tf["ch"], H * W
        Np = ops.round16(N)
        g = self._gn(x, None, p + ".norm", 1e-6, False)
        if Np == N:
            hs = ops.linear(g.reshape(B * N, C), sd[p + ".proj_in.weight"], bias=sd[p + ".proj_in.bias"], out_f32=self.stream_f32)
        else:
            hs = ops.gemm_conv([ops.SegSpec(g, 0, C)], sd[p + ".proj_in.weight"], B * Np, Ho=1, Wo=Np, Hi=1, Wi=N, bias=sd[p + ".proj_in.bias"],
                               out_f32=self.stream_f32)
        for blk in tf["blocks"]:
            hs = self._block(blk, hs, B, Np, C, ctx, garment, feats_out, stop_after_feats, last=blk is tf["blocks"][-1], nk=N)
            if hs is None:
                return None
        if Np == N:
            out = ops.linear(hs, sd[p + ".proj_out.weight"], bias=sd[p + ".proj_out.bias"], res=x.reshape(B * N, C))
        else:
            out = ops.gemm_conv([ops.SegSpec(hs.view(B, Np, C), 0, C)], sd[p + ".proj_out.weight"], B * N, Ho=1, Wo=N, Hi=1, Wi=Np,
                                bias=sd[p + ".proj_out.bias"], res=x.reshape(B * N, C))
        return out.view(B, N, C)

    def feature_tokens(self, h, w):
        lv = [(h, w)]
        for _ in range(len(self.cfg.block_out_channels) - 1):
            lv.append(((lv[-1][0] + 1) // 2, (lv[-1][1] + 1) // 2))
        return [lv[tf["level"]][0] * lv[tf["level"]][1] for tf in self.tf.values() for _ in tf["blocks"]]

    def num_features(self):
        return sum(len(t["blocks"]) for t in self.tf.values())

    def _f8_fused(self, N):
        return self.attn_fp8 and self.f8_fused and N % 64 == 0

    def project_garment_kv(self, feats, out=None):
        assert self.tryon and len(feats) == len(self.block_order)
        res = []
        for i, (blk, g) in enumerate(zip(self.block_order, feats)):
            Bg, N, C = g.shape
            f8 = self._f8_fused(N)
            if out is not None:
                kg, vtg = out[i][0][:Bg * N], out[i][1][:Bg]
            else:
                kg = torch.empty(Bg * N, C, dtype=torch.uint8 if f8 else self.dtype, device=self.device)
                vtg = torch.empty(Bg, C, N, dtype=torch.uint8 if f8 else self.dtype, device=self.device)
            f8kw = dict(f8=(2.0 ** self.f8_exp[1], 2.0 ** self.f8_exp[2])) if f8 else {}
            ops.linear(g.reshape(Bg * N, C), blk["qkv"][C:], out=kg, vt=vtg, vt_n0=C, vt_tokens=N, **f8kw)
            res.append((kg, vtg))
        return res

    def weights_id(self, select=None):
        from .garment_cache import weights_fingerprint
        ids = self.__dict__.setdefault("_weights_ids", {})
        key = getattr(select, "__name__", None) if select is not None else "all"
        if key not in ids:
            ids[key] = weights_fingerprint({k: v for k, v in self.sd.items() if select is None or select(k)})
        return ids[key]

    def forward(self, x, temb, ctx, B, H, W, garment_feats=None, garment_kv=None, feats_buf=None, garment_persons=None, garment_hw=None,
                garment_index=None, garment_nk=None):
        topo = self.topo
        garment = dict(feats=garment_feats, kv=garment_kv, feats_buf=feats_buf, idx=0, persons=garment_persons, index=garment_index, nk_table=garment_nk,
                       nk=self.feature_tokens(*garment_hw) if garment_hw is not None and self.tryon else None)
        feats = []
        stop = None if self.tryon else self.num_features()
        h, _, _ = self._conv3(x, self.conv_in, B, H, W)
        skips = [(h, H, W)]
        for i, blk in enumerate(topo["down"]):
            for j in range(len(blk["resnets"])):
                h = self._resnet(f"down_blocks.{i}.resnets.{j}", h, None, temb, B, H, W)
                if blk["attn"]:
                    h = self._transformer(f"down_blocks.{i}.attentions.{j}", h, B, H, W, ctx, garment, feats)
                skips.append((h, H, W))
            if blk["down"]:
                h, H, W = self._conv3(h, self.res[f"down_blocks.{i}.downsamplers.0.conv"], B, H, W, stride=2)
                skips.append((h, H, W))
        h = self._resnet("mid_block.resnets.0", h, None, temb, B, H, W)
        h = self._transformer("mid_block.attentions.0", h, B, H, W, ctx, garment, feats)
        h = self._resnet("mid_block.resnets.1", h, None, temb, B, H, W)
        for i, blk in enumerate(topo["up"]):
            if not self.tryon and not blk["attn"]:
                continue
            for j in range(len(blk["resnets"])):
                s, sh, sw = skips.pop()
                assert (sh, sw) == (H, W), "skip / upsample size mismatch"
                h = self._resnet(f"up_blocks.{i}.resnets.{j}", h, s, temb, B, H, W)
                if blk["attn"]:
                    h = self._transformer(f"up_blocks.{i}.attentions.{j}", h, B, H, W, ctx, garment, feats, stop)
                    if h is None:
                        return None, feats
            if blk["up"]:
                tgt = (skips[-1][1], skips[-1][2]) if skips else (2 * H, 2 * W)
                h, H, W = self._conv3(h, self.res[f"up_blocks.{i}.upsamplers.0.conv"], B, H, W, ups=True, out_hw=tgt)
        if not self.tryon:
            return None, feats
        g = self._gn(h, None, "conv_norm_out", self.cfg.norm_eps, True)
        out, _, _ = self._conv3(g, self.conv_out, B, H, W)
        return out, feats
```

### include/idmvton_hip.h

```cpp
#ifndef IDMVTON_HIP_H
#define IDMVTON_HIP_H
#include <stddef.h>
#include <stdint.h>

#ifdef __cplusplus
extern "C" {
#endif

enum { IDMVTON_OK = 0, IDMVTON_E_SHAPE = -1, IDMVTON_E_DTYPE = -2, IDMVTON_E_ALIGN = -3, IDMVTON_E_LAUNCH = -4,
       IDMVTON_E_ARG = -5 };
enum { IDMVTON_F16 = 0, IDMVTON_BF16 = 1, IDMVTON_F32 = 2, IDMVTON_F8E4M3 = 3  };

const char* idmvton_last_error(void);
int idmvton_abi_version(void);
int idmvton_sizeof(const char* struct_name);

#define IDMVTON_MAX_SEG 24
typedef struct {
    const void* ptr;
    uint32_t bytes;
    int32_t pitch;
    int32_t coff;
    int32_t len;
    int32_t dy, dx;
} idmvton_seg;

enum { IDMVTON_EPI_NONE = 0, IDMVTON_EPI_GEGLU = 1, IDMVTON_EPI_GELU = 2 ,
       IDMVTON_EPI_QUICKGELU = 3 ,
       IDMVTON_EPI_XATTN = 4  };
typedef struct {
    int32_t nseg;
    const void* k[2]; int32_t ldk[2]; int32_t k_rows[2];
    const void* vt[2]; int32_t ldvt[2];
    int32_t nk[2];
    int32_t tokens; float ip_scale;
} idmvton_xattn;
enum { IDMVTON_IO_RES_F32 = 1, IDMVTON_IO_OUT_F32 = 2, IDMVTON_IO_BIAS_F32 = 4, IDMVTON_IO_OUT_F8 = 8 };
typedef struct {
    int32_t dtype;
    const void* w; int32_t N; int32_t Ktot;
    int32_t nseg; idmvton_seg seg[IDMVTON_MAX_SEG];
    int32_t M, Ho, Wo, Hi, Wi, stride, ups;
    void* out; int32_t ldo;
    const void* bias;
    const void* rowbias; int32_t rowbias_ld; int32_t rows_per_group;
    const void* res; int32_t ldr;
    int32_t mode;
    void* vt; int32_t vt_n0; int32_t vt_tokens;
    int32_t tile_hint;
    int32_t vt_perm;
    int32_t io_flags;
    const idmvton_xattn* xattn;
    int32_t colscale_n; float colscale;
    float f8_out_scale, f8_vt_scale;
} idmvton_gemm_conv_args;
int idmvton_gemm_conv(const idmvton_gemm_conv_args* a, void* stream);

enum { IDMVTON_ATTN_SELF = 0, IDMVTON_ATTN_CROSS = 1 };
typedef struct {
    int32_t dtype; int32_t mode;
    int32_t B, heads, Nq;
    const void* q; int32_t ldq;
    void* out; int32_t ldo;
    int32_t nseg;
    const void* k[2]; int32_t ldk[2];
    const void* vt[2]; int32_t ldvt[2];
    int32_t nk[2];
    int32_t k_rows[2];
    int32_t seg_b0[2];
    float ip_scale;
    int32_t tune;
    int32_t q_prescaled;
} idmvton_attn_args;
int idmvton_attn_fwd(const idmvton_attn_args* a, void* stream);
int idmvton_attn_fwd_shared(const idmvton_attn_args* a, const int32_t seg_nb[2], void* stream);
int idmvton_attn_fwd_indexed(const idmvton_attn_args* a, const int32_t seg_nb[2], const int32_t* const seg_index[2], void* stream);
int idmvton_attn_fwd_ragged(const idmvton_attn_args* a, const int32_t seg_nb[2], const int32_t* const seg_index[2],
                            const int32_t* const seg_nk[2], void* stream);

typedef struct {
    int32_t out_dtype; int32_t B, heads, Nq;
    const void* q8; int32_t ldq;
    void* out; int32_t ldo;
    int32_t nseg;
    const void* k8[2]; int32_t ldk[2];
    const void* vt8[2]; int32_t ldvt[2];
    int32_t nk[2]; int32_t k_rows[2]; int32_t seg_b0[2];
    int32_t qk_scale_exp; int32_t v_scale_exp;
} idmvton_attn_f8_args;
int idmvton_attn_f8(const idmvton_attn_f8_args* a, void* stream);
int idmvton_attn_f8_shared(const idmvton_attn_f8_args* a, const int32_t seg_nb[2], void* stream);
int idmvton_attn_f8_indexed(const idmvton_attn_f8_args* a, const int32_t seg_nb[2], const int32_t* const seg_index[2], void* stream);
int idmvton_attn_f8_ragged(const idmvton_attn_f8_args* a, const int32_t seg_nb[2], const int32_t* const seg_index[2],
                           const int32_t* const seg_nk[2], void* stream);
typedef struct {
    int32_t dtype; int32_t mode; int32_t rows, cols;
    const void* src; int32_t lds;
    void* dst; int32_t ldd;
    float scale;
} idmvton_quant_f8_args;
int idmvton_quant_f8(const idmvton_quant_f8_args* a, void* stream);

typedef struct {
    const void* src;
    void* dst;
    const int32_t* exp;
    int32_t rows, cols, lds, ldd;
} idmvton_kv_unpack_desc;
typedef struct {
    int32_t dtype; int32_t n;
    const idmvton_kv_unpack_desc* desc;
    int32_t max_chunks;
} idmvton_kv_unpack_args;
int idmvton_kv_unpack(const idmvton_kv_unpack_args* a, const idmvton_kv_unpack_desc* host_desc, void* stream);

enum { IDMVTON_KVS_WIDEN_E4M3 = 0, IDMVTON_KVS_COPY = 1 };
#define IDMVTON_KVS_MAX_N (1 << 20)
typedef idmvton_kv_unpack_desc idmvton_kv_stream_desc;
typedef struct {
    int32_t dtype; int32_t mode; int32_t n; int32_t workgroups;
    const idmvton_kv_stream_desc* desc;
    const int32_t* first;
} idmvton_kv_stream_args;
int idmvton_kv_stream(const idmvton_kv_stream_args* a, const idmvton_kv_stream_desc* host_desc, const int32_t* host_first, void* stream);
int idmvton_host_device_ptr(const void* host, void** dev);

int idmvton_kv_fill(const idmvton_kv_stream_args* a, const idmvton_kv_stream_desc* host_desc, const int32_t* host_first, void* stream);

typedef struct {
    int32_t dtype; int32_t B, heads, Lq, Lk, d;
    const void* q; int32_t ldq;
    const void* k; int32_t ldk;
    const void* v; int32_t ldv;
    void* out; int32_t ldo;
    float scale; int32_t causal;
} idmvton_attn_small_args;
int idmvton_attn_small(const idmvton_attn_small_args* a, void* stream);

typedef struct {
    int32_t dtype; int32_t rows, C;
    const void* x; int32_t ldx;
    const void* gamma; const void* beta; float eps;
    void* y; int32_t ldy;
    void* y2; int32_t ldy2;
    int32_t x_f32;
} idmvton_layernorm_args;
int idmvton_layernorm(const idmvton_layernorm_args* a, void* stream);

enum { IDMVTON_GN_X_F32 = 1 , IDMVTON_GN_Y_SPLIT = 2 ,
       IDMVTON_GN_AFFINE_F32 = 4  };
typedef struct {
    int32_t dtype; int32_t B, HW, C, groups;
    const void* x; int32_t C1;
    const void* x2;
    const void* gamma; const void* beta; float eps; int32_t silu;
    void* y;
    double* stats; int32_t stats_doubles;
    int32_t flags;
} idmvton_groupnorm_args;
int idmvton_groupnorm(const idmvton_groupnorm_args* a, void* stream);
int idmvton_groupnorm_stats_doubles(int B, int HW, int C, int groups);

typedef struct {
    int32_t dtype; int32_t B, hw, cpad;
    const float* latents; const void* cond; void* out;
} idmvton_pack_input_args;
int idmvton_pack_input(const idmvton_pack_input_args* a, void* stream);

typedef struct {
    int32_t dtype; int32_t B, hw, ldc;
    const void* eps_nhwc; float* latents; const float* noise; const float* coef;
} idmvton_cfg_step_args;
int idmvton_cfg_step(const idmvton_cfg_step_args* a, void* stream);

enum { IDMVTON_LAYOUT_SPLIT = 1 , IDMVTON_LAYOUT_NHWC_F32 = 2  };
typedef struct {
    int32_t dtype; int32_t B, C, HW, cpad; int32_t to_nhwc;
    const void* src; void* dst; float scale; float shift;
    int32_t flags;
} idmvton_layout_args;
int idmvton_layout(const idmvton_layout_args* a, void* stream);

typedef struct {
    int32_t dtype; int32_t B, hw, ldm;
    const void* moments; const float* noise; float* z; float scale;
} idmvton_vae_sample_args;
int idmvton_vae_sample(const idmvton_vae_sample_args* a, void* stream);

typedef struct {
    int32_t dtype; int32_t rows, n, ld;
    void* x; float scale;
    void* y_split; int32_t ldy;
    int32_t n_valid;
} idmvton_softmax_args;
int idmvton_softmax_rows(const idmvton_softmax_args* a, void* stream);

enum { IDMVTON_SPLIT_ACT = 0, IDMVTON_SPLIT_W3 = 1, IDMVTON_SPLIT_W3T = 2 };
typedef struct {
    int32_t dtype; int32_t mode; int32_t rows, cols;
    const float* src; int32_t lds;
    void* dst; int32_t ldd;
} idmvton_split_args;
int idmvton_split(const idmvton_split_args* a, void* stream);

int idmvton_rccl_unique_id(void* id128);
int idmvton_rccl_comm_init(const void* id128, int rank, int world, void** comm_out);
int idmvton_rccl_bcast_arena(void* comm, void* buf, uint64_t bytes, int root, uint64_t chunk_bytes, void* stream);
int idmvton_rccl_comm_destroy(void* comm);

int idmvton_probe_mfma(int which, const void* a, const void* b, float* c, void* stream);

#ifdef __cplusplus
}
#endif
#endif
```

Baseline: 1.609 images/s.

## Fuse GarmentNet QKV projection with TryonNet garment K/V projection into one GEMM

```diff
diff --git a/idm-vton_amd/csrc/gemm_body.cuh b/idm-vton_amd/csrc/gemm_body.cuh
--- a/idm-vton_amd/csrc/gemm_body.cuh
+++ b/idm-vton_amd/csrc/gemm_body.cuh
@@ -6,8 +6,8 @@
 #include "common.cuh"
 #include "gemm_common.cuh"
 
-template <typename T, int BN, int BM, int WN, int WM, int ST, bool V1, bool LIN, bool PF, bool TR, bool XA = false>
-__device__ __forceinline__ void gemm_body(const GemmParams& p, char* smem, const int m0, const int n0) {
+template <typename T, int BN, int BM, int WN, int WM, int ST, bool V1, bool LIN, bool PF, bool TR, bool XA = false, bool SP = false>
+__device__ __forceinline__ void gemm_body(const typename GemmParamsOf<SP>::type& p, char* smem, const int m0, const int n0) {
     typedef typename VT<T>::v8 v8;
     typedef typename VT<T>::v4 v4;
     constexpr int NW = WN * WM;
@@ -229,11 +229,12 @@
         xattn_load_v<T>(p.xa, xa_b, xa_h, lane, xvf);
         xattn_compute<T, MI>(p.xa, p.M, acc, m0 + wm * SM, lane, xkf, xvf);
     }
-    gemm_epilogue<T, NI, MI, SN, SM, TR>(p, acc, m0, n0, wn, wm, lane);
-}
-
-template <typename T, int BN, int BM, int WN, int WM, int ST, bool V1, bool LIN, int OCC, bool PFX = false>
-__global__ __launch_bounds__(WN * WM * 64, OCC) void gemm_conv_kernel(const GemmParams p) {
+    if constexpr (SP) gemm_epilogue_split<T, NI, MI, SN, SM, TR>(p, acc, m0, n0, wn, wm, lane);
+    else gemm_epilogue<T, NI, MI, SN, SM, TR>(p, acc, m0, n0, wn, wm, lane);
+}
+
+template <typename T, int BN, int BM, int WN, int WM, int ST, bool V1, bool LIN, int OCC, bool PFX = false, bool SP = false>
+__global__ __launch_bounds__(WN * WM * 64, OCC) void gemm_conv_kernel(const typename GemmParamsOf<SP>::type p) {
     __shared__ __attribute__((aligned(1024))) char smem[ST * (BN + BM) * 128];
     const int wg = xcd_remap(blockIdx.x, p.tiles_m * p.tiles_n);
     int tm, tn;
@@ -250,8 +251,13 @@
     if constexpr (BN == 320) {
         gemm_body<T, BN, BM, WN, WM, ST, V1, LIN, OCC == 1 || PFX, false>(p, smem, m0, n0);
     } else {
-        if (p.vt != nullptr && n0 >= p.vt_n0) gemm_body<T, BN, BM, WN, WM, ST, V1, LIN, OCC == 1 || PFX, true>(p, smem, m0, n0);
-        else gemm_body<T, BN, BM, WN, WM, ST, V1, LIN, OCC == 1 || PFX, false>(p, smem, m0, n0);
+        if constexpr (SP) {
+            if (gemm_tile_tr(p, n0)) gemm_body<T, BN, BM, WN, WM, ST, V1, LIN, OCC == 1 || PFX, true, false, true>(p, smem, m0, n0);
+            else gemm_body<T, BN, BM, WN, WM, ST, V1, LIN, OCC == 1 || PFX, false, false, true>(p, smem, m0, n0);
+        } else {
+            if (p.vt != nullptr && n0 >= p.vt_n0) gemm_body<T, BN, BM, WN, WM, ST, V1, LIN, OCC == 1 || PFX, true>(p, smem, m0, n0);
+            else gemm_body<T, BN, BM, WN, WM, ST, V1, LIN, OCC == 1 || PFX, false>(p, smem, m0, n0);
+        }
     }
 }
 
@@ -268,11 +274,16 @@
     gemm_body<T, BN, BM, WN, WM, ST, true, true, OCC == 1, false, true>(p, smem, tm * BM, tn * BN);
 }
 
-template <typename T, int BN, int BM, int WN, int WM, int ST, bool V1, int OCC, bool PFX = false>
-static void launch_cfg(const GemmParams& p0, bool lin, hipStream_t st) {
-    GemmParams p = p0;
+template <typename T, int BN, int BM, int WN, int WM, int ST, bool V1, int OCC, bool PFX = false, bool SP = false>
+static void launch_cfg(const typename GemmParamsOf<SP>::type& p0, bool lin, hipStream_t st) {
+    typename GemmParamsOf<SP>::type p = p0;
     p.gm = V1 ? idmvton_choose_gm(p.tiles_m, p.tiles_n, BM, BN, p.Ktot) : 0;
     const dim3 grid(p.tiles_n * p.tiles_m), block(WN * WM * 64);
+    if constexpr (SP) {
+        static_assert(V1 && BN != 320, "second output group: the variant-1 ring tiles");
+        hipLaunchKernelGGL((gemm_conv_kernel<T, BN, BM, WN, WM, ST, true, true, OCC, PFX, true>), grid, block, 0, st, p);
+        return;
+    }
     if constexpr (V1) {
         if (lin) { hipLaunchKernelGGL((gemm_conv_kernel<T, BN, BM, WN, WM, ST, true, true, OCC, PFX>), grid, block, 0, st, p); return; }
     }
@@ -281,8 +292,8 @@
 
 
 int gemm_tiles_v0(const GemmParams& p, bool bf16, int bn, int bm, bool lin, hipStream_t st);
-int gemm_tiles_v1(const GemmParams& p, bool bf16, int bn, int bm, bool lin, hipStream_t st);
+int gemm_tiles_v1(const GemmParamsX& p, bool bf16, int bn, int bm, bool lin, hipStream_t st);
 int gemm_tiles_v2(const GemmParams& p, bool bf16, int bn, int bm, bool lin, hipStream_t st);
 int gemm_tiles_w8(const GemmParams& p, bool bf16, int bn, int bm, int form, bool lin, hipStream_t st);
 int gemm_tiles_xattn(const GemmParams& p, bool bf16, int bn, int bm, int w8, hipStream_t st);
-int launch_gemm_lin(const GemmParams& p, bool bf16, int bm, int form, int grid_cap, hipStream_t st);
+int launch_gemm_lin(const GemmParamsX& p, bool bf16, int bm, int form, int grid_cap, hipStream_t st);
diff --git a/idm-vton_amd/csrc/gemm_common.cuh b/idm-vton_amd/csrc/gemm_common.cuh
--- a/idm-vton_amd/csrc/gemm_common.cuh
+++ b/idm-vton_amd/csrc/gemm_common.cuh
@@ -20,6 +20,17 @@
     int out8; float o8_scale, vt8_scale;
     XAttnParams xa;
 };
+struct GemmParamsX : GemmParams {
+    int n_split;
+    void* out2; int ldo2;
+    void* vt2; int vt2_n0; int vt2_tokens;
+};
+template <bool SP> struct GemmParamsOf { typedef GemmParams type; };
+template <> struct GemmParamsOf<true> { typedef GemmParamsX type; };
+
+__device__ __forceinline__ bool gemm_tile_tr(const GemmParamsX& p, const int n0) {
+    return (p.vt != nullptr && n0 >= p.vt_n0 && n0 < p.n_split) || (p.vt2 != nullptr && n0 >= p.vt2_n0);
+}
 
 int idmvton_choose_gm(int tiles_m, int tiles_n, int bm, int bn, int K);
 
@@ -290,3 +301,91 @@
             }
     }
 }
+
+template <typename T, int NI, int MI, int SN, int SM, bool TR>
+__device__ __forceinline__ void gemm_epilogue_split(const GemmParamsX& p, f32x16 (&acc)[NI][MI], const int m0, const int n0, const int wn, const int wm,
+                                                    const int lane) {
+    typedef typename VT<T>::v8 v8;
+    const int u = lane >> 5, l31 = lane & 31;
+    auto dest = [&](const int c, T*& base, int& col, int& ld, int& cv) -> int {
+        cv = 0;
+        if (c >= p.N) return 0;
+        if (c < p.n_split) {
+            if (p.vt != nullptr && c >= p.vt_n0) { base = (T*)p.vt; col = c - p.vt_n0; ld = p.vt_tokens; cv = p.n_split - p.vt_n0; return 2; }
+            base = (T*)p.out; col = c; ld = p.ldo;
+            return 1;
+        }
+        if (p.vt2 != nullptr && c >= p.vt2_n0) { base = (T*)p.vt2; col = c - p.vt2_n0; ld = p.vt2_tokens; cv = p.N - p.vt2_n0; return 2; }
+        base = (T*)p.out2; col = c - p.n_split; ld = p.ldo2;
+        return 1;
+    };
+    if constexpr (TR) {
+#pragma unroll
+        for (int ni = 0; ni < NI; ++ni) {
+            const int n = n0 + wn * SN + ni * 32 + l31;
+            T* base; int col, ld, cv;
+            const int kind = dest(n & ~15, base, col, ld, cv);
+            col += n & 15;
+            if (kind == 2) {
+#pragma unroll
+                for (int mi = 0; mi < MI; ++mi)
+#pragma unroll
+                    for (int gp = 0; gp < 2; ++gp) {
+                        const int m = m0 + wm * SM + mi * 32 + 16 * gp;
+                        if (m >= p.M) continue;
+                        const int b = m / ld;
+                        const int tok = m - b * ld + 8 * u;
+                        v8 o;
+#pragma unroll
+                        for (int j = 0; j < 8; ++j) o[j] = (T)(acc[ni][mi][8 * gp + j] + 0.f);
+                        *(v8*)(base + ((size_t)(b * cv + col) * ld + tok)) = o;
+                    }
+            } else if (kind == 1) {
+                const bool scaled = n < p.colscale_n;
+#pragma unroll
+                for (int mi = 0; mi < MI; ++mi)
+#pragma unroll
+                    for (int r = 0; r < 16; ++r) {
+                        const int m = m0 + wm * SM + mi * 32 + 8 * (r >> 2) + 4 * u + (r & 3);
+                        if (m >= p.M) continue;
+                        const float v = acc[ni][mi][r];
+                        base[(size_t)m * ld + col] = (T)(scaled ? v * p.colscale : v);
+                    }
+            }
+        }
+        return;
+    }
+#pragma unroll
+    for (int mi = 0; mi < MI; ++mi) {
+        const int m = m0 + wm * SM + mi * 32 + l31;
+        if (m >= p.M) continue;
+#pragma unroll
+        for (int ni = 0; ni < NI; ++ni)
+#pragma unroll
+            for (int gp = 0; gp < 2; ++gp) {
+                const int c = n0 + wn * SN + ni * 32 + 16 * gp;
+                T* base; int col, ld, cv;
+                const int kind = dest(c, base, col, ld, cv);
+                if (kind == 0) continue;
+                float v[8];
+                swap_cols8(acc[ni][mi], gp, v);
+                if (c + 8 * u < p.colscale_n) {
+#pragma unroll
+                    for (int j = 0; j < 8; ++j) v[j] *= p.colscale;
+                }
+                if (kind == 1) {
+                    v8 o;
+#pragma unroll
+                    for (int j = 0; j < 8; ++j) o[j] = (T)v[j];
+                    *(v8*)(base + (size_t)m * ld + col + 8 * u) = o;
+                } else {
+                    const int b = m / ld;
+                    int tok = m - b * ld;
+                    tok = (tok & ~12) | ((tok & 4) << 1) | ((tok & 8) >> 1);
+                    T* q = base + ((size_t)(b * cv + col + 8 * u) * ld + tok);
+#pragma unroll
+                    for (int j = 0; j < 8; ++j) q[(size_t)j * ld] = (T)v[j];
+                }
+            }
+    }
+}
diff --git a/idm-vton_amd/csrc/gemm_conv.hip b/idm-vton_amd/csrc/gemm_conv.hip
--- a/idm-vton_amd/csrc/gemm_conv.hip
+++ b/idm-vton_amd/csrc/gemm_conv.hip
@@ -3,7 +3,7 @@
 #include <vector>
 #include "gemm_body.cuh"
 
-int launch_gemm_lin(const GemmParams& p, bool bf16, int bm, int form, int grid_cap, hipStream_t st);
+int launch_gemm_lin(const GemmParamsX& p, bool bf16, int bm, int form, int grid_cap, hipStream_t st);
 
 #include <map>
 #include <mutex>
@@ -46,8 +46,8 @@
     return best_gm;
 }
 
-static int launch_gemm(const GemmParams& p0, bool bf16, int variant, int bn, int bm, bool lin, hipStream_t st) {
-    GemmParams p = p0;
+static int launch_gemm(const GemmParamsX& p0, bool bf16, int variant, int bn, int bm, bool lin, hipStream_t st) {
+    GemmParamsX p = p0;
     int form = 0;
     int grid_cap = 0;
     if (variant == 5) { form = bm & 15; grid_cap = (bm & 0x4000) ? 5 : 0; bm &= ~(15 | 0x4000); }
@@ -63,6 +63,12 @@
             return idmvton_set_error(IDMVTON_E_ARG, "gemm_conv: IDMVTON_EPI_XATTN runs on the 128x64, 128x128 and 128x256 tiles (got %dx%d)", bn, bm);
         CHECK_LAUNCH("gemm_conv");
         return IDMVTON_OK;
+    }
+    if (p.n_split && variant != 1 && variant != 5) {
+        if (variant == 6) bm &= ~15;
+        if (bn == 320) { bn = 128; bm = 256; }
+        p.tiles_n = (p.N + bn - 1) / bn; p.tiles_m = (p.M + bm - 1) / bm;
+        variant = 1;
     }
     if (variant == 0) rc = gemm_tiles_v0(p, bf16, bn, bm, lin, st);
     else if (variant == 1) rc = gemm_tiles_v1(p, bf16, bn, bm, lin, st);
@@ -131,7 +137,7 @@
                          a->vt_n0 >= 0 && a->vt_n0 < a->N && ((uintptr_t)a->vt & 7) == 0,
                          IDMVTON_E_ARG, "gemm_conv: vt_tokens=%d vt_n0=%d", a->vt_tokens, a->vt_n0);
 
-    GemmParams p;
+    GemmParamsX p;
     memset(&p.xa, 0, sizeof(p.xa));
     if (xattn) {
         const idmvton_xattn* x = a->xattn;
@@ -158,6 +164,8 @@
     p.vt = a->vt; p.vt_n0 = a->vt_n0; p.vt_tokens = a->vt_tokens > 0 ? a->vt_tokens : 4; p.vt_perm = a->vt_perm ? 1 : 0;
     p.colscale_n = a->colscale_n; p.colscale = a->colscale;
     p.tiles_m = p.tiles_n = 0; p.gm = 0;
+    p.n_split = a->n_split;
+    p.out2 = a->out2; p.ldo2 = a->ldo2; p.vt2 = a->vt2; p.vt2_n0 = a->vt2_n0; p.vt2_tokens = a->vt2_tokens > 0 ? a->vt2_tokens : 16;
     {
         auto a16 = [](const void* q) { return ((uintptr_t)q & 15) == 0; };
         const int n_out = geglu ? a->N / 2 : a->N;
@@ -206,11 +214,28 @@
     const idmvton_seg& s0 = a->seg[0];
     const bool lin = a->nseg == 1 && a->Ho == 1 && a->Hi == 1 && a->Wo == a->M && a->Wi == a->M && a->stride == 1 &&
                      !a->ups && s0.dy == 0 && s0.dx == 0 && (uint64_t)a->M * s0.pitch * 2 < 0x80000000ull;
+    if (a->n_split) {
+        CHECK_ARG(a->n_split > 0 && a->n_split < a->N && a->n_split % 16 == 0 && a->N % 16 == 0, IDMVTON_E_ARG,
+                  "gemm_conv: n_split=%d must be a multiple of 16 inside (0, N=%d), N a multiple of 16", a->n_split, a->N);
+        CHECK_ARG(a->out2 != nullptr, IDMVTON_E_ARG, "gemm_conv: n_split=%d with a null out2", a->n_split);
+        CHECK_ARG(lin && a->mode == IDMVTON_EPI_NONE && !a->bias && !a->rowbias && !a->res && !a->io_flags, IDMVTON_E_ARG,
+                  "gemm_conv: a second output group needs a plain Linear (one K segment, mode NONE) without bias / rowbias / residual / io_flags");
+        CHECK_ARG(a->colscale_n <= (a->vt ? a->vt_n0 : a->n_split), IDMVTON_E_ARG, "gemm_conv: colscale_n=%d reaches beyond the first group's row-major columns", a->colscale_n);
+        CHECK_ARG(!a->vt || (a->vt_perm && a->vt_n0 < a->n_split), IDMVTON_E_ARG,
+                  "gemm_conv: with a second output group vt needs vt_perm = 1 and vt_n0=%d < n_split=%d", a->vt_n0, a->n_split);
+        CHECK_ARG(((uintptr_t)a->out2 & 15) == 0 && a->ldo2 % 8 == 0 && ((uintptr_t)a->vt2 & 15) == 0, IDMVTON_E_ALIGN,
+                  "gemm_conv: out2 / vt2 must be 16-byte aligned and ldo2=%d a multiple of 8", a->ldo2);
+        CHECK_ARG(a->ldo2 >= (a->vt2 ? a->vt2_n0 : a->N) - a->n_split, IDMVTON_E_ARG, "gemm_conv: ldo2=%d is narrower than the second group's row-major columns", a->ldo2);
+        if (a->vt2) CHECK_ARG(a->vt_perm && a->vt2_n0 >= a->n_split && a->vt2_n0 < a->N && a->vt2_n0 % 16 == 0 && a->vt2_tokens > 0 &&
+                              a->vt2_tokens % 16 == 0 && a->M % a->vt2_tokens == 0, IDMVTON_E_ARG,
+                              "gemm_conv: vt2 needs vt_perm = 1, vt2_n0=%d a multiple of 16 in [n_split, N), vt2_tokens=%d a multiple of 16 dividing M", a->vt2_n0, a->vt2_tokens);
+        CHECK_ARG(p.wide, IDMVTON_E_ALIGN, "gemm_conv: a second output group needs the 16-byte epilogue (16-byte aligned out / vt, ldo and colscale_n multiples of 8)");
+    } else CHECK_ARG(!a->out2 && !a->vt2 && !a->ldo2 && !a->vt2_n0 && !a->vt2_tokens, IDMVTON_E_ARG, "gemm_conv: out2 / vt2 fields set without n_split");
     if (!a->tile_hint && bn == 256 && bm == 256 && lin) { variant = 5; bm = 257; }
     else if (!a->tile_hint && !xattn) {
         if (bn == 256 && bm == 256) variant = 6;
         else if (bn == 128 && bm == 128) variant = 6;
-        if (a->N > 256 && a->N <= 320 && p.wide && !a->vt && !geglu && !p.out8 && (a->M + 191) / 192 >= 200) { variant = 6; bn = 320; bm = 192; }
+        if (a->N > 256 && a->N <= 320 && p.wide && !a->vt && !geglu && !p.out8 && !a->n_split && (a->M + 191) / 192 >= 200) { variant = 6; bn = 320; bm = 192; }
     }
     hipStream_t st = (hipStream_t)stream;
     return launch_gemm(p, a->dtype == IDMVTON_BF16, variant, bn, bm, lin, st);
diff --git a/idm-vton_amd/csrc/gemm_lin.hip b/idm-vton_amd/csrc/gemm_lin.hip
--- a/idm-vton_amd/csrc/gemm_lin.hip
+++ b/idm-vton_amd/csrc/gemm_lin.hip
@@ -1,8 +1,8 @@
 #include "gemm_common.cuh"
 #include <type_traits>
 
-template <typename T, int BM, int WN, int WM, int DMA_SPLIT, int WAIT_AT>
-__device__ __forceinline__ void gemm_lin_persistent(const GemmParams& p, char* smem) {
+template <typename T, int BM, int WN, int WM, int DMA_SPLIT, int WAIT_AT, bool SP>
+__device__ __forceinline__ void gemm_lin_persistent(const typename GemmParamsOf<SP>::type& p, char* smem) {
     typedef typename VT<T>::v8 v8;
     constexpr int BN = 256, NW = WN * WM;
     constexpr int SN = BN / WN, SM = BM / WM, NI = SN / 32, MI = SM / 32;
@@ -173,7 +173,8 @@
         __builtin_amdgcn_sched_barrier(0);
         mfma_range(1, 0, NMF);
         if (has_next) asm volatile("s_waitcnt vmcnt(0)" ::: "memory");
-        gemm_epilogue<T, NI, MI, SN, SM, TR>(p, acc, m0, n0, wn, wm, lane);
+        if constexpr (SP) gemm_epilogue_split<T, NI, MI, SN, SM, TR>(p, acc, m0, n0, wn, wm, lane);
+        else gemm_epilogue<T, NI, MI, SN, SM, TR>(p, acc, m0, n0, wn, wm, lane);
     };
 
     coords(idx, m0, n0);
@@ -184,17 +185,22 @@
         const int nidx = idx + G;
         has_next = nidx < ntiles;
         if (has_next) coords(nidx, nm0, nn0);
-        if (p.vt != nullptr && n0 >= p.vt_n0) run_tile(std::true_type{});
-        else run_tile(std::false_type{});
+        if constexpr (SP) {
+            if (gemm_tile_tr(p, n0)) run_tile(std::true_type{});
+            else run_tile(std::false_type{});
+        } else {
+            if (p.vt != nullptr && n0 >= p.vt_n0) run_tile(std::true_type{});
+            else run_tile(std::false_type{});
+        }
         if (!has_next) break;
         cur ^= BUF; idx = nidx; m0 = nm0; n0 = nn0;
     }
 }
 
-template <typename T, int BM, int WN, int WM, int DMA_SPLIT, int WAIT_AT>
-__global__ __launch_bounds__(512, 2) void gemm_lin_kernel(const GemmParams p) {
+template <typename T, int BM, int WN, int WM, int DMA_SPLIT, int WAIT_AT, bool SP = false>
+__global__ __launch_bounds__(512, 2) void gemm_lin_kernel(const typename GemmParamsOf<SP>::type p) {
     __shared__ __attribute__((aligned(1024))) char smem[2 * (256 + BM) * 128];
-    gemm_lin_persistent<T, BM, WN, WM, DMA_SPLIT, WAIT_AT>(p, smem);
+    gemm_lin_persistent<T, BM, WN, WM, DMA_SPLIT, WAIT_AT, SP>(p, smem);
 }
 
 static int persistent_grid(int ntiles, int grid_cap) {
@@ -208,15 +214,24 @@
     return ntiles < cap ? ntiles : cap;
 }
 template <typename T>
-static int launch_lin(const GemmParams& p0, int bm, int form, int grid_cap, hipStream_t st) {
+static int launch_lin(const GemmParamsX& p0, int bm, int form, int grid_cap, hipStream_t st) {
+    const int gm = idmvton_choose_gm(p0.tiles_m, p0.tiles_n, bm, 256, p0.Ktot);
+    const dim3 grid(persistent_grid(p0.tiles_n * p0.tiles_m, grid_cap)), block(512);
+    if (p0.n_split) {
+        GemmParamsX p = p0;
+        p.gm = gm;
+        if (bm == 192) hipLaunchKernelGGL((gemm_lin_kernel<T, 192, 4, 2, 0, 2, true>), grid, block, 0, st, p);
+        else if (form == 0) hipLaunchKernelGGL((gemm_lin_kernel<T, 256, 2, 4, 0, 2, true>), grid, block, 0, st, p);
+        else hipLaunchKernelGGL((gemm_lin_kernel<T, 256, 2, 4, 1, 2, true>), grid, block, 0, st, p);
+        return 0;
+    }
     GemmParams p = p0;
-    p.gm = idmvton_choose_gm(p.tiles_m, p.tiles_n, bm, 256, p.Ktot);
-    const dim3 grid(persistent_grid(p.tiles_n * p.tiles_m, grid_cap)), block(512);
+    p.gm = gm;
     if (bm == 192) hipLaunchKernelGGL((gemm_lin_kernel<T, 192, 4, 2, 0, 2>), grid, block, 0, st, p);
     else if (form == 0) hipLaunchKernelGGL((gemm_lin_kernel<T, 256, 2, 4, 0, 2>), grid, block, 0, st, p);
     else hipLaunchKernelGGL((gemm_lin_kernel<T, 256, 2, 4, 1, 2>), grid, block, 0, st, p);
     return 0;
 }
-int launch_gemm_lin(const GemmParams& p, bool bf16, int bm, int form, int grid_cap, hipStream_t st) {
+int launch_gemm_lin(const GemmParamsX& p, bool bf16, int bm, int form, int grid_cap, hipStream_t st) {
     return bf16 ? launch_lin<bf16_t>(p, bm, form, grid_cap, st) : launch_lin<f16_t>(p, bm, form, grid_cap, st);
 }
diff --git a/idm-vton_amd/csrc/gemm_tiles_v1.hip b/idm-vton_amd/csrc/gemm_tiles_v1.hip
--- a/idm-vton_amd/csrc/gemm_tiles_v1.hip
+++ b/idm-vton_amd/csrc/gemm_tiles_v1.hip
@@ -1,7 +1,16 @@
 #include "gemm_body.cuh"
 
 template <typename T>
-static int run(const GemmParams& p, int bn, int bm, bool lin, hipStream_t st) {
+static int run(const GemmParamsX& p, int bn, int bm, bool lin, hipStream_t st) {
+    if (p.n_split) {
+        if (bn == 256 && bm == 256) launch_cfg<T, 256, 256, 2, 4, 2, true, 2, false, true>(p, lin, st);
+        else if (bn == 128 && bm == 256) launch_cfg<T, 128, 256, 2, 4, 3, true, 2, false, true>(p, lin, st);
+        else if (bn == 128 && bm == 128) launch_cfg<T, 128, 128, 2, 2, 3, true, 1, false, true>(p, lin, st);
+        else if (bn == 128 && bm == 64) launch_cfg<T, 128, 64, 2, 2, 3, true, 2, false, true>(p, lin, st);
+        else if (bn == 64 && bm == 64) launch_cfg<T, 64, 64, 2, 2, 4, true, 2, false, true>(p, lin, st);
+        else return 1;
+        return 0;
+    }
     if (bn == 256 && bm == 256) launch_cfg<T, 256, 256, 2, 4, 2, true, 2>(p, lin, st);
     else if (bn == 128 && bm == 256) launch_cfg<T, 128, 256, 2, 4, 3, true, 2>(p, lin, st);
     else if (bn == 128 && bm == 128) launch_cfg<T, 128, 128, 2, 2, 3, true, 1>(p, lin, st);
@@ -10,6 +19,6 @@
     else return 1;
     return 0;
 }
-int gemm_tiles_v1(const GemmParams& p, bool bf16, int bn, int bm, bool lin, hipStream_t st) {
+int gemm_tiles_v1(const GemmParamsX& p, bool bf16, int bn, int bm, bool lin, hipStream_t st) {
     return bf16 ? run<bf16_t>(p, bn, bm, lin, st) : run<f16_t>(p, bn, bm, lin, st);
 }
diff --git a/idm-vton_amd/ffi.py b/idm-vton_amd/ffi.py
--- a/idm-vton_amd/ffi.py
+++ b/idm-vton_amd/ffi.py
@@ -33,7 +33,8 @@
                 ("out", vp), ("ldo", i32), ("bias", vp), ("rowbias", vp), ("rowbias_ld", i32),
                 ("rows_per_group", i32), ("res", vp), ("ldr", i32), ("mode", i32), ("vt", vp), ("vt_n0", i32),
                 ("vt_tokens", i32), ("tile_hint", i32), ("vt_perm", i32), ("io_flags", i32), ("xattn", C.POINTER(XAttn)),
-                ("colscale_n", i32), ("colscale", f32), ("f8_out_scale", f32), ("f8_vt_scale", f32)]
+                ("colscale_n", i32), ("colscale", f32), ("f8_out_scale", f32), ("f8_vt_scale", f32),
+                ("n_split", i32), ("out2", vp), ("ldo2", i32), ("vt2", vp), ("vt2_n0", i32), ("vt2_tokens", i32)]
 
 
 class AttnArgs(C.Structure):
diff --git a/idm-vton_amd/ops.py b/idm-vton_amd/ops.py
--- a/idm-vton_amd/ops.py
+++ b/idm-vton_amd/ops.py
@@ -90,7 +90,8 @@
 
 def gemm_conv(segs, w, M, *, Ho=1, Wo=None, Hi=1, Wi=None, stride=1, ups=False, out=None, ldo=None, bias=None,
               rowbias=None, rowbias_ld=0, rows_per_group=1, res=None, ldr=None, geglu=False, gelu=False, quick_gelu=False, vt=None,
-              vt_n0=0, vt_tokens=0, vt_perm=True, colscale_n=0, colscale=1.0, tile_hint=0, out_f32=False, xattn=None, f8=None):
+              vt_n0=0, vt_tokens=0, vt_perm=True, colscale_n=0, colscale=1.0, tile_hint=0, out_f32=False, xattn=None, f8=None,
+              n_split=0, out2=None, ldo2=None, vt2=None, vt2_n0=0, vt2_tokens=0):
     if f8 is not None:
         if res is not None or rowbias is not None or geglu or gelu or quick_gelu or (bias is not None and bias.dtype == torch.float32):
             raise ValueError("gemm_conv(f8=...): no residual / rowbias / activation, and the bias in the storage dtype (not fp32)")
@@ -115,7 +116,7 @@
     Wo = M if Wo is None else Wo
     Wi = M if Wi is None else Wi
     a.M, a.Ho, a.Wo, a.Hi, a.Wi, a.stride, a.ups = M, Ho, Wo, Hi, Wi, stride, int(bool(ups))
-    n_out = N // 2 if geglu else (vt_n0 if vt is not None else N)
+    n_out = N // 2 if geglu else (vt_n0 if vt is not None else (n_split or N))
     if out is None and n_out > 0:
         out = torch.empty((M, n_out), dtype=torch.uint8 if f8 is not None else (torch.float32 if out_f32 else w.dtype), device=w.device)
     if f8 is not None:
@@ -142,11 +143,13 @@
             xflops += 4.0 * M * N * sg["nk"]
         a.mode, a.xattn = ffi.EPI_XATTN, C.pointer(xa)
     a.vt, a.vt_n0, a.vt_tokens = _ptr(vt), vt_n0, vt_tokens
-    a.vt_perm = int(bool(vt_perm)) if vt is not None else 0
+    a.vt_perm = int(bool(vt_perm)) if vt is not None or vt2 is not None else 0
     a.colscale_n, a.colscale = colscale_n, colscale
+    a.n_split, a.out2, a.vt2, a.vt2_n0, a.vt2_tokens = n_split, _ptr(out2), _ptr(vt2), vt2_n0, vt2_tokens
+    a.ldo2 = ldo2 if ldo2 is not None else (out2.stride(-2) if out2 is not None else 0)
     a.tile_hint = tile_hint if tile_hint else _TUNE["gemm"].get(gemm_key(a), 0)
     if RECORD is not None:
-        RECORD.append(("gemm", gemm_key(a), type(a).from_buffer_copy(a), (segs, w, out, bias, rowbias, res, vt, xa, xattn)))
+        RECORD.append(("gemm", gemm_key(a), type(a).from_buffer_copy(a), (segs, w, out, bias, rowbias, res, vt, xa, xattn, out2, vt2)))
     seen, xbytes = set(), 0
     for sg in segs:
         if sg.t.data_ptr() not in seen:
diff --git a/idm-vton_amd/pipeline.py b/idm-vton_amd/pipeline.py
--- a/idm-vton_amd/pipeline.py
+++ b/idm-vton_amd/pipeline.py
@@ -46,9 +46,10 @@
 
 
 class TryonEngine:
-    def __init__(self, unet, unet_encoder, vae, resampler=None, dtype=torch.bfloat16, device="cuda"):
+    def __init__(self, unet, unet_encoder, vae, resampler=None, dtype=torch.bfloat16, device="cuda", merge_garment_kv=True):
         self.unet, self.unet_encoder, self.vae, self.resampler = unet, unet_encoder, vae, resampler
         self.dtype, self.device = dtype, torch.device(device)
+        self._merged_qkv = self._merge_qkv_weights() if merge_garment_kv else None
         self._graphs = {}
         self._set_shapes = {}
         self._side = None
@@ -112,6 +113,21 @@
             return (st["B"], st["h"], st["w"], st["gh"], st["gw"], st["k"], st["steps_noise"] is not None)
         return (st["B"], st["h"], st["w"], st["gh"], st["gw"], st["k"], st["steps_noise"] is not None, "cached",
                 "indexed" if st.get("gindex") is not None else st["gcache"].G) + (("ragged",) if st.get("gnk") is not None else ())
+
+    def _merge_qkv_weights(self):
+        t, g = self.unet, self.unet_encoder
+        if t is None or g is None or not hasattr(t, "block_order") or not hasattr(g, "block_order"):
+            return None
+        tb, gb = t.block_order, g.block_order
+        if t.attn_fp8 or g.attn_fp8 or t.dtype != g.dtype or len(tb) != len(gb) or any(a["qkv"].shape != b["qkv"].shape for a, b in zip(gb, tb)):
+            return None
+        ws = []
+        for a, b in zip(gb[:-1], tb[:-1]):
+            C = a["qkv"].shape[1]
+            w = torch.cat([a["qkv"], b["qkv"][C:]]).contiguous()
+            a["qkv"] = w[:3 * C]
+            ws.append(w)
+        return ws
 
     def weights_identity(self):
         if self._weights_id is None:
@@ -296,8 +312,10 @@
         B, h, w = st["B"], st["gh"], st["gw"]
         c = st["k"] if c is None else c
         self.stats["garment_batches"] += 1
-        _, feats = self.unet_encoder.forward(st["cloth_k"][:c * B], temb_gk[:c * B], st["ctx_gk"], c * B, h, w, feats_buf=fset["feats"])
-        self.unet.project_garment_kv(feats, out=fset["kv"])
+        mq = self._merged_qkv
+        _, feats = self.unet_encoder.forward(st["cloth_k"][:c * B], temb_gk[:c * B], st["ctx_gk"], c * B, h, w, feats_buf=fset["feats"],
+                                             merged_kv=(mq, fset["kv"]) if mq is not None else None)
+        self.unet.project_garment_kv(feats, out=fset["kv"], only=(len(feats) - 1,) if mq is not None else None)
 
     def _tryon_main(self, st, temb_t, coef, noise, kv_j):
         B, h, w = st["B"], st["h"], st["w"]
diff --git a/idm-vton_amd/unet.py b/idm-vton_amd/unet.py
--- a/idm-vton_amd/unet.py
+++ b/idm-vton_amd/unet.py
@@ -199,7 +199,10 @@
         M = B * N
         nk = N if nk is None else nk
         feat = None
-        if not self.tryon:
+        merged = garment.get("merged") if garment and not self.tryon else None
+        if merged is not None and len(feats_out) >= len(merged[0]):
+            merged = None
+        if not self.tryon and merged is None:
             fb = garment.get("feats_buf") if garment else None
             feat = fb[len(feats_out)][:B].view(M, C) if fb is not None else torch.empty(M, C, dtype=dt, device=dev)
         f8 = self._f8_fused(N)
@@ -213,7 +216,14 @@
             feats_out.append(feat.view(B, N, C))
             if stop is not None and len(feats_out) >= stop:
                 return None
-        ops.linear(n1, blk["qkv"], out=qk, vt=vt, vt_n0=2 * C, vt_tokens=N, colscale_n=C, colscale=qcs, **f8kw)
+        if merged is not None:
+            i = len(feats_out)
+            feats_out.append(None)
+            kg, vtg = merged[1][i][0][:M], merged[1][i][1][:B]
+            ops.linear(n1, merged[0][i], out=qk, vt=vt, vt_n0=2 * C, vt_tokens=N, colscale_n=C, colscale=qcs,
+                       n_split=3 * C, out2=kg, vt2=vtg, vt2_n0=4 * C, vt2_tokens=N)
+        else:
+            ops.linear(n1, blk["qkv"], out=qk, vt=vt, vt_n0=2 * C, vt_tokens=N, colscale_n=C, colscale=qcs, **f8kw)
         segs = [dict(k=qk[:, C:], vt=vt, nk=nk, ldk=2 * C, ldvt=N, k_rows=N)]
         if self.tryon:
             gnk = garment["nk"][garment["idx"]] if garment.get("nk") is not None else None
@@ -328,10 +338,13 @@
     def _f8_fused(self, N):
         return self.attn_fp8 and self.f8_fused and N % 64 == 0
 
-    def project_garment_kv(self, feats, out=None):
+    def project_garment_kv(self, feats, out=None, only=None):
         assert self.tryon and len(feats) == len(self.block_order)
         res = []
         for i, (blk, g) in enumerate(zip(self.block_order, feats)):
+            if only is not None and i not in only:
+                res.append(None)
+                continue
             Bg, N, C = g.shape
             f8 = self._f8_fused(N)
             if out is not None:
@@ -353,9 +366,10 @@
         return ids[key]
 
     def forward(self, x, temb, ctx, B, H, W, garment_feats=None, garment_kv=None, feats_buf=None, garment_persons=None, garment_hw=None,
-                garment_index=None, garment_nk=None):
+                garment_index=None, garment_nk=None, merged_kv=None):
         topo = self.topo
         garment = dict(feats=garment_feats, kv=garment_kv, feats_buf=feats_buf, idx=0, persons=garment_persons, index=garment_index, nk_table=garment_nk,
+                       merged=merged_kv,
                        nk=self.feature_tokens(*garment_hw) if garment_hw is not None and self.tryon else None)
         feats = []
         stop = None if self.tryon else self.num_features()
diff --git a/include/idmvton_hip.h b/include/idmvton_hip.h
--- a/include/idmvton_hip.h
+++ b/include/idmvton_hip.h
@@ -53,6 +53,9 @@
     const idmvton_xattn* xattn;
     int32_t colscale_n; float colscale;
     float f8_out_scale, f8_vt_scale;
+    int32_t n_split;
+    void* out2; int32_t ldo2;
+    void* vt2; int32_t vt2_n0; int32_t vt2_tokens;
 } idmvton_gemm_conv_args;
 int idmvton_gemm_conv(const idmvton_gemm_conv_args* a, void* stream);
 
```

Result: no change. 1.619 images/s (median of 6 runs) (+0.6%).
